# ChristophReich1996/Multi-StyleGAN

Hardware: AMD Instinct MI355X
Metric: training images/sec (G+D step, 256^2, seq=3x2ch) (higher is better)
Workload: dtype bf16

## Files before the change

include/msg_hip.h:

```cpp
#ifndef MSG_HIP_H
#define MSG_HIP_H

#ifdef __cplusplus
extern "C" {
#endif

enum { MSG_OK = 0, MSG_EINVAL = -1, MSG_EUNSUPPORTED = -2, MSG_ELAUNCH = -3 };
enum { MSG_F32 = 0, MSG_BF16 = 1, MSG_F16 = 2, MSG_F64 = 3, MSG_F32_SPLIT = 4 };

#define MSG_ABI_VERSION 5
int msg_abi_version(void);
const char* msg_build_arch(void);
const char* msg_strerror(int code);

int msg_upfirdn2d(const void* x, const float* fir, void* y, int dtype,
                  int major, int in_h, int in_w, int minor, int kh, int kw,
                  int up_x, int up_y, int down_x, int down_y,
                  int pad_x0, int pad_x1, int pad_y0, int pad_y1, void* stream);

int msg_upfirdn2d_pitched(const void* x, const float* fir, void* y, int dtype,
                          int major, int in_h, int in_w, int minor, int in_pitch, int kh, int kw,
                          int up_x, int up_y, int down_x, int down_y,
                          int pad_x0, int pad_x1, int pad_y0, int pad_y1, void* stream);

int msg_upfirdn2d_pitched2(const void* x, const float* fir, void* y, int dtype,
                           int major, int in_h, int in_w, int minor, int in_pitch, int out_pitch, int kh, int kw,
                           int up_x, int up_y, int down_x, int down_y,
                           int pad_x0, int pad_x1, int pad_y0, int pad_y1, void* stream);

int msg_upfirdn2d_separable(const void* x, const float* fir_y, const float* fir_x, void* y, int dtype,
                            int major, int in_h, int in_w, int minor, int kh, int kw,
                            int pad_x0, int pad_x1, int pad_y0, int pad_y1, void* stream);

int msg_upfirdn2d_separable_act(const void* x, const float* fir_y, const float* fir_x, void* y, int dtype,
                                int major, int in_h, int in_w, int minor, int kh, int kw,
                                int pad_x0, int pad_x1, int pad_y0, int pad_y1,
                                const float* act_bias, const float* noise, const float* noise_weight,
                                int noise_batch, float alpha, float scale, void* stream);
int msg_upfirdn2d_separable_act_mask(const void* x, const float* fir_y, const float* fir_x, void* y, int dtype,
                                     int major, int in_h, int in_w, int minor, int kh, int kw,
                                     int pad_x0, int pad_x1, int pad_y0, int pad_y1,
                                     const float* act_bias, const float* noise, const float* noise_weight,
                                     int noise_batch, float alpha, float scale, unsigned char* mask, void* stream);

int msg_fused_bias_act(const void* x, const float* bias, const void* ref, void* y, int dtype,
                       long long size_x, int step_b, int size_b,
                       const float* noise, const float* noise_weight, int noise_batch, int pix,
                       int act, int grad, float alpha, float scale, void* stream);

long long msg_bias_act_backward_workspace(long long size_x, int step_b, int size_b, int has_noise);
int msg_bias_act_backward(const void* gy, const void* out, void* gx, int dtype,
                          long long size_x, int step_b, int size_b,
                          float* grad_bias, const float* noise, float* grad_noise_weight,
                          int noise_batch, int pix, float alpha, float scale,
                          float* ws, long long ws_floats, void* stream);
int msg_channel_sums(const void* x, float* sums, int dtype, long long size_x, int C, float* ws, long long ws_floats,
                     void* stream);
int msg_bias_act_backward_mask(const void* gy, const unsigned char* mask, int tile_m, int tile_n, void* gx, int dtype,
                               long long size_x, int size_b,
                               float* grad_bias, const float* noise, float* grad_noise_weight,
                               int noise_batch, int pix, float alpha, float scale,
                               float* ws, long long ws_floats, void* stream);
int msg_sum_rows(const float* part, float* out, long long rows, int cols, void* stream);
int msg_bias_act_backward_mask_head(const void* gy, const void* ghead, const float* whead, const float* style,
                                    float wscale, int n_head, const unsigned char* mask, int tile_m, int tile_n,
                                    void* gx, int dtype, long long size_x, int size_b,
                                    float* grad_bias, const float* noise, float* grad_noise_weight,
                                    int noise_batch, int pix, float alpha, float scale,
                                    float* ws, long long ws_floats, void* stream);

int msg_conv2d_fprop(const void* x, const void* w, const float* bias, void* y, int dtype,
                     int B, int IH, int IW, int Cx, int Ck, int OH, int OW, int N, int ldy,
                     int kh, int kw, int stride, int pad, int in_up, int pixel_shuffle,
                     long long w_batch_stride, void* stream);
enum { MSG_WGRAD_K_AUTO = -1 };
int msg_conv2d_wgrad(const void* gy, const void* x, float* gw, int dtype,
                     int B, int IH, int IW, int Cx, int I, int OH, int OW, int ldgy, int O, int ldgw,
                     int kh, int kw, int stride, int pad, int pixel_shuffle,
                     int per_sample, int k_chunks, int oi_major, float gain,
                     float* ws, long long ws_floats, void* stream);
long long msg_conv2d_wgrad_workspace(int dtype, int B, int IH, int IW, int Cx, int I, int OH, int OW, int ldgy,
                                     int O, int ldgw, int kh, int kw, int stride, int pad, int pixel_shuffle,
                                     int per_sample, int k_chunks);

int msg_demod_coeff(const float* W, const float* s, float* d, int B, int O, int I, int taps,
                    float scale, float eps, void* stream);
int msg_scale_rows_cols(const float* base, const float* rowscale, const float* colscale, void* out,
                        int dtype, int B, int R, int T, int C, int Ck, float gain, void* stream);
int msg_modulate_weights(const float* base, const float* wsq, const float* style, void* out, float* d_out,
                         int dtype, int B, int R, int O, int T, int C, int Ck, float scale, float eps, void* stream);
int msg_modulate_backward(const float* gwk, const float* W, const float* s, const float* d, float* gW,
                          float* gs_part, int B, int O, int I, int taps, int ldg, int o_group,
                          float scale, void* stream);
int msg_scale_rows_cols2(const float* base, const float* row1, const float* col1, const float* row2, const float* col2,
                         void* out, int dtype, int B, int R, int T, int C, int Ck, float gain, void* stream);
int msg_modulate_backward2(const float* gwk, const float* W, const float* s, const float* d, const float* v,
                           float* gW, float* gs_part, int B, int O, int I, int taps, int ldg, int o_group,
                           float scale, void* stream);

int msg_relayout_weight(const float* w, void* fwd, void* dgrad, float* wsq, int dtype,
                        int O, int I, int T, int Ck, int Ok, int flip, int t_major, float gain, void* stream);

int msg_gather_taps(const void* x, void* y, int dtype, int B, int H, int W, int Cx, int C, int kh, int kw,
                    int pad, int Ko, void* stream);
int msg_fold_taps(const void* g, const void* add, void* gx, int dtype, int B, int H, int W, int Ko, int C, int kh, int kw,
                  int pad, int ldx, int ld_add, void* stream);

int msg_scaled_add(const void* a, const void* b, void* y, int dtype, long long n, float beta, float gain, void* stream);
int msg_rgb_skip_merge(const void* conv, int dtype, int ld, const float* bias, const float* skip, const float* fir,
                       float* out, int B, int C, int H, int W, void* stream);
int msg_rgb_skip_merge_backward(const float* g, void* g_conv, int dtype, int ld, float* g_skip, const float* fir,
                                int B, int C, int H, int W, void* stream);
int msg_gamma_merge(const void* a, const void* b, const float* gamma, void* y, int dtype, long long n, float gain, void* stream);
long long msg_gamma_merge_backward_workspace(void);
int msg_gamma_merge_backward(const void* gy, const void* a, const float* gamma, void* ga, void* gb, float* g_gamma, int dtype,
                             long long n, float gain, float* ws, void* stream);
int msg_scaled_add_rows(const void* a, const void* b, void* y, int dtype, long long rows, int cols,
                        long long lda, long long ldb, long long ldy, float beta, float gain, void* stream);

int msg_softmax_rows(const void* x, void* y, int dtype, long long rows, int cols, void* stream);
int msg_softmax_rows_backward(const void* y, const void* gy, void* gx, int dtype, long long rows, int cols,
                              void* stream);
int msg_softmax_rows_backward2(const void* y, const void* gy, const void* v, void* d_y, void* d_gy, int dtype,
                               long long rows, int cols, void* stream);

int msg_nonlocal_attention_supported(int B, int Nq, int Nk, int dk, int dv);
int msg_nonlocal_attention_fwd(const void* q, const void* k, const void* vt, void* o, float* lse, int dtype,
                               int B, int Nq, int Nk, int dk, int dv, void* stream);
int msg_maxpool2x2_fwd(const void* x, void* y, unsigned short* idx, int dtype, int B, int H, int W, int C, long long ldx,
                       void* stream);
int msg_maxpool2x2_bwd(const void* gy, const unsigned short* idx, void* gx, int dtype, int B, int H, int W, int C,
                       void* stream);
int msg_maxpool2x2_gather(const void* v, const unsigned short* idx, void* out, int dtype, int B, int H, int W, int C,
                          long long ldv, void* stream);

int msg_nonlocal_attention_bwd_splits(int B, int Nq, int Nk);
int msg_nonlocal_attention_bwd(const void* q, const void* qt, const void* k, const void* kt, const void* v,
                               const void* dO, const void* dOt, const void* o, const float* lse, float* delta,
                               void* dq, void* dk_out, void* dv_out, float* workspace, int dtype,
                               int B, int Nq, int Nk, int dk, int dv, void* stream);

int msg_affine_warp(const float* x, float* y, const float* angle_deg, float angle_const, const float* scale_xy,
                    const float* select_u, const float* p, int rot_prob, float cx, float cy, int padding,
                    int align_corners, int B, int C, int H, int W, int backward, void* workspace, void* stream);

long long msg_minibatch_stddev_workspace(int C, int H, int W, int groups, int dtype);
int msg_minibatch_stddev(const void* x, void* y, float* stat, float* workspace, int dtype,
                         int B, int C, int H, int W, int ldx, int ldy, int groups, float alpha, void* stream);
int msg_minibatch_stddev_backward(const void* x, const void* gy, const float* gstat, void* gx, int dtype,
                                  int B, int C, int H, int W, int ldx, int ldgy, int ldgx, int groups,
                                  float alpha, void* stream);

int msg_conv2d_fprop_act(const void* x, const void* w, void* y, int dtype,
                         int B, int IH, int IW, int Cx, int Ck, int OH, int OW, int N, int ldy,
                         int kh, int kw, int stride, int pad, long long w_batch_stride,
                         const float* act_bias, const float* noise, const float* noise_weight,
                         int noise_batch, float alpha, float scale, void* stream);
int msg_conv2d_fprop_act_mask(const void* x, const void* w, void* y, int dtype,
                              int B, int IH, int IW, int Cx, int Ck, int OH, int OW, int N, int ldy,
                              int kh, int kw, int stride, int pad, long long w_batch_stride,
                              const float* act_bias, const float* noise, const float* noise_weight,
                              int noise_batch, float alpha, float scale, unsigned char* mask, void* stream);

int msg_conv2d_fprop_residual(const void* x, const void* w, void* y, int dtype,
                              int B, int IH, int IW, int Cx, int Ck, int OH, int OW, int N, int ldy,
                              int kh, int kw, int stride, int pad, long long w_batch_stride,
                              const void* residual, int res_ld, float gain, void* stream);

int msg_conv2d_fprop_act_backward(const void* x, const void* w, void* y, int dtype,
                                  int B, int IH, int IW, int Cx, int Ck, int OH, int OW, int N, int ldy,
                                  int kh, int kw, int stride, int pad, long long w_batch_stride,
                                  const void* residual, int res_ld,
                                  const unsigned char* sign_mask, int mask_tile_m, int mask_tile_n,
                                  const void* sign_map, int sign_ld, float alpha, float scale,
                                  float* grad_bias, const float* noise, int noise_batch, float* grad_noise_weight,
                                  float* ws, long long ws_floats, void* stream);

int msg_act_pointwise_head(const void* x, const float* bias, const float* w, float* y, int dtype,
                           long long npix, int C, float wscale, float alpha, float scale, void* stream);
long long msg_act_pointwise_head_backward_workspace(long long npix, int C);
int msg_act_pointwise_head_backward(const void* x, const float* bias, const float* w, const float* gy, void* gx,
                                    float* grad_bias_and_w, int dtype, long long npix, int C, float wscale,
                                    float alpha, float scale, float* ws, long long ws_floats, void* stream);

int msg_linear_fprop(const float* x, const float* w, const float* bias, float* y, int M, int N, int K,
                     float gain, float bias_gain, void* stream);
int msg_linear_dgrad(const float* gy, const float* w, float* gx, int M, int N, int K, float gain, void* stream);
int msg_linear_wgrad(const float* gy, const float* x, float* gw, float* gb, int M, int N, int K,
                     float gain, float bias_gain, void* stream);

int msg_linear_grouped_fprop(const float* x, const int* slot, const float* const* w, const float* const* bias, float* y,
                             int G, int M, int N, int K, int L, float gain, float bias_gain, void* stream);
int msg_linear_grouped_dgrad(const float* gy, const float* const* w, float* gx, int G, int M, int N, int K, float gain,
                             void* stream);
int msg_linear_grouped_wgrad(const float* gy, const float* x, const int* slot, float* gw, float* gb, int G, int M, int N,
                             int K, int L, float gain, float bias_gain, void* stream);
int msg_linear_grouped_wgrad_ptrs(const float* gy, const float* x, const int* slot, float* const* gw, float* const* gb, int G,
                                  int M, int N, int K, int L, float gain, float bias_gain, void* stream);

enum {
    MSG_PLAN_REG = 0,
    MSG_PLAN_DMA = 1,
    MSG_PLAN_PP = 2,
    MSG_PLAN_ROW3 = 3,
    MSG_PLAN_ROW3N = 4,
    MSG_PLAN_THIN = 5,
    MSG_PLAN_UPCONV = 6,
    MSG_FPLAN_FIELDS = 5
};
int msg_conv2d_fprop_launch_plan(int dtype, int B, int IH, int IW, int Cx, int Ck, int OH, int OW, int N, int ldy,
                                 int kh, int kw, int stride, int pad, int in_up, int pixel_shuffle,
                                 long long w_batch_stride, int has_bias, int epilogue, long long* out, int n_out_fields);
enum {
    MSG_WPLAN_GENERIC = 0,
    MSG_WPLAN_DMA = 1,
    MSG_WPLAN_UNI = 2,
    MSG_WPLAN_ROW3 = 3,
    MSG_WPLAN_ROW3_W32 = 4,
    MSG_WPLAN_FIELDS = 11
};
int msg_conv2d_wgrad_plan(int dtype, int B, int IH, int IW, int Cx, int I, int OH, int OW, int ldgy,
                          int O, int ldgw, int kh, int kw, int stride, int pad, int pixel_shuffle,
                          int per_sample, int k_chunks, long long* out, int n_out_fields);
int msg_conv2d_fprop_plan(int dtype, int B, int IH, int IW, int Cx, int Ck, int OH, int OW, int N,
                          int kh, int kw, long long w_batch_stride);
long long msg_conv2d_fprop_act_backward_workspace(int dtype, int B, int IH, int IW, int Cx, int Ck, int OH, int OW,
                                                  int N, int kh, int kw, long long w_batch_stride, int has_noise);
int msg_conv2d_fprop_upconv_eligible(int B, int IH, int IW, int Cx, int Ck, int OH, int OW, int N, int kh, int kw,
                                     int stride, int pad, int in_up, int pixel_shuffle, long long w_batch_stride);
int msg_conv2d_fprop_thin_eligible(int B, int IH, int IW, int Cx, int Ck, int OH, int OW, int N, int ldy, int kh, int kw,
                                   int stride, int pad, int in_up, int pixel_shuffle, int act_mode);

int msg_flat_adam(float* param, const float* grad, float* exp_avg, float* exp_avg_sq, float* ema, long long n,
                  const float* coef, float lr, float beta1, float beta2, float eps, int step, float ema_decay,
                  void* stream);
int msg_flat_ema(float* ema, const float* param, long long n, float decay, void* stream);

long long msg_tlfm_prepare_workspace(int B, int T);
int msg_tlfm_prepare(const unsigned short* raw, const unsigned char* hflip, void* out, int dtype,
                     int B, int C, int T, int H, int W, int vflip,
                     float lo1, float div1, float lo2, float div2,
                     unsigned int* ws, void* stream);

int msg_tlfm_frame_range(const unsigned short* frames, long long N, int H, int W,
                         unsigned int* range, void* stream);
int msg_tlfm_gather(const unsigned short* frames, const unsigned int* range, long long N,
                    const int* index, const unsigned char* hflip, void* out, int dtype,
                    int B, int C, int T, int H, int W, int vflip,
                    float lo1, float div1, float lo2, float div2, void* stream);

int msg_sample_sheet(const void* seq, unsigned char* out, int dtype,
                     int B, int C, int T, int H, int W, int tints, void* stream);

enum { MSG_GAN_LOGISTIC = 0, MSG_GAN_WASSERSTEIN = 1, MSG_GAN_HINGE = 2 };
enum { MSG_GAN_AUX_NONE = 0, MSG_GAN_AUX_WEIGHT = 1, MSG_GAN_AUX_LABEL = 2 };
long long msg_gan_loss_workspace(long long n_real, long long n_fake);
int msg_gan_loss(const void* pred_real, const void* pred_fake, const float* aux, float* out, int dtype, int kind,
                 int aux_mode, long long n_real, long long n_fake, long long P, float* ws, long long ws_floats,
                 void* stream);
int msg_gan_loss_backward(const void* pred_real, const void* pred_fake, const float* aux, const float* grad_out,
                          void* grad_real, void* grad_fake, int dtype, int kind, int aux_mode,
                          long long n_real, long long n_fake, long long P, void* stream);

#define MSG_ELASTIC_MAX_SIGMA 32
long long msg_elastic_workspace(int B, int H, int W);
int msg_elastic_deform(const void* in, const float* noise, float* field, void* out, int dtype,
                       int B, int F, int H, int W, int sigma, float alpha, void* ws, void* stream);

#define MSG_JPEG_MAX_WIDTH 16384
long long msg_jpeg_workspace(int N, int H, int W);
int msg_jpeg_scan_capacity(int N, int H, int W, long long* bytes);
int msg_jpeg_encode(const unsigned char* rgb, const unsigned short* qtables, short* coef, unsigned char* scan,
                    long long* offsets, int N, int H, int W, void* ws, void* stream);

#ifdef __cplusplus
}
#endif
#endif
```

multi_stylegan_amd/conv_ops.py:

```python
import ctypes
import functools
import math
import os
from typing import Optional, Tuple

import torch
from torch.autograd import Function

from . import _lib
from ._autograd import _derive


def _vec(dtype) -> int:
    return 8 if dtype == torch.bfloat16 else 4


def _round_up(n: int, m: int) -> int:
    return (n + m - 1) // m * m


def _padded_nhwc(b, c, h, w, dtype, device):
    cx = _round_up(c, _vec(dtype))
    buf = torch.empty((b, h, w, cx), dtype=dtype, device=device)
    if cx != c:
        buf[..., c:].zero_()
    return buf.permute(0, 3, 1, 2)[:, :c]


class _CatChannels(Function):

    @staticmethod
    def forward(ctx, *tensors):
        t0 = tensors[0]
        ctx.splits = [t.shape[1] for t in tensors]
        out = _padded_nhwc(t0.shape[0], sum(ctx.splits), t0.shape[2], t0.shape[3], t0.dtype, t0.device)
        off = 0
        for t in tensors:
            out[:, off:off + t.shape[1]].copy_(t)
            off += t.shape[1]
        return out

    @staticmethod
    def backward(ctx, g):
        if torch.is_grad_enabled():
            pieces = _SplitChannels.apply(g, *ctx.splits)
            return tuple(p if need else None for p, need in zip(pieces, ctx.needs_input_grad))
        outs, off = [], 0
        for i, c in enumerate(ctx.splits):
            outs.append(g[:, off:off + c] if ctx.needs_input_grad[i] else None)
            off += c
        return tuple(outs)


class _SplitChannels(Function):

    @staticmethod
    def forward(ctx, g, *splits):
        ctx.splits = splits
        ctx.meta = (g.shape[0], g.shape[2], g.shape[3], g.dtype, g.device)
        outs, off = [], 0
        for c in splits:
            outs.append(g[:, off:off + c])
            off += c
        return tuple(outs)

    @staticmethod
    def backward(ctx, *gg):
        b, h, w, dtype, dev = ctx.meta
        pieces = [x if x is not None else torch.zeros((b, c, h, w), dtype=dtype, device=dev)
                  for x, c in zip(gg, ctx.splits)]
        return (_CatChannels.apply(*pieces),) + (None,) * len(ctx.splits)


def to_compute_layout(x: torch.Tensor, dtype=None) -> torch.Tensor:
    if dtype is not None and x.dtype != dtype:
        x = x.to(dtype)
    if x.ndim == 4 and x.shape[1] > 1:
        if x.is_cuda and x.shape[1] % _vec(x.dtype):
            return _CatChannels.apply(x)
        return x.contiguous(memory_format=torch.channels_last)
    return x.contiguous()


class _CatAliased(Function):

    @staticmethod
    def forward(ctx, buffer, *pieces):
        ctx.splits = [t.shape[1] for t in pieces]
        off = 0
        for t in pieces:
            want = buffer[:, off:off + t.shape[1]]
            if t.shape != want.shape or t.dtype != buffer.dtype:
                raise _lib.MsgHipError(f"cat_in_place: piece {tuple(t.shape)} for slice {tuple(want.shape)}")
            same = t.data_ptr() == want.data_ptr() and \
                all(a == b for a, b, n in zip(t.stride(), want.stride(), t.shape) if n != 1)
            if not same:
                if t.untyped_storage().data_ptr() == buffer.untyped_storage().data_ptr():
                    raise _lib.MsgHipError("cat_in_place: a piece lives in the destination buffer, but not in its slice")
                want.copy_(t)
            off += t.shape[1]
        if off != buffer.shape[1]:
            raise _lib.MsgHipError("cat_in_place: the pieces do not fill the destination buffer")
        return buffer.view_as(buffer)

    @staticmethod
    def backward(ctx, g):
        needs = ctx.needs_input_grad[1:]
        if torch.is_grad_enabled():
            pieces = _SplitChannels.apply(g, *ctx.splits)
            return (None, *(p if need else None for p, need in zip(pieces, needs)))
        out, off = [], 0
        for c, need in zip(ctx.splits, needs):
            out.append(g[:, off:off + c] if need else None)
            off += c
        return (None, *out)


def cat_destination(b: int, channels, h: int, w: int, dtype, device):
    if any(c % _vec(dtype) for c in channels) or not torch.device(device).type == "cuda":
        return None
    buf = _padded_nhwc(b, sum(channels), h, w, dtype, device)
    if any(c % (128 // buf.element_size()) for c in channels):
        buf.zero_()
    views, off = [], 0
    for c in channels:
        views.append(buf[:, off:off + c])
        off += c
    return buf, views


def cat_in_place(buffer, pieces) -> torch.Tensor:
    return _CatAliased.apply(buffer, *pieces)


def cat_channels(tensors) -> torch.Tensor:
    tensors = list(tensors)
    if tensors[0].is_cuda and all(t.dtype == tensors[0].dtype for t in tensors):
        return _CatChannels.apply(*tensors)
    return to_compute_layout(torch.cat(tensors, dim=1))


def _nhwc_view(x: torch.Tensor) -> Tuple[torch.Tensor, int]:
    b, c, h, w = x.shape
    vec = _vec(x.dtype)
    sb, sc, sh, sw = x.stride()
    cx = sw
    if (sc == 1 or c == 1) and cx >= c and cx % vec == 0 and sh == w * cx and (sb == h * w * cx or b == 1) \
            and x.data_ptr() % 16 == 0:
        return x, cx
    cx = _round_up(c, vec)
    buf = torch.empty((b, h, w, cx), dtype=x.dtype, device=x.device).permute(0, 3, 1, 2)
    if cx == c:
        buf.copy_(x)
        return buf, cx
    buf[:, :c].copy_(x)
    buf[:, c:].zero_()
    return buf[:, :c], cx


def _alloc_out(b: int, n: int, h: int, w: int, dtype, device) -> Tuple[torch.Tensor, int]:
    ld = _round_up(n, _vec(dtype))
    if ld == n:
        return torch.empty((b, n, h, w), dtype=dtype, device=device, memory_format=torch.channels_last), ld
    buf = torch.empty((b, h, w, ld), dtype=dtype, device=device)
    return buf.permute(0, 3, 1, 2)[:, :n], ld


def _relayout_kernel_ok(w, dtype, taps) -> bool:
    return w.is_cuda and w.dtype == torch.float32 and dtype in (torch.bfloat16, torch.float32) and \
        taps <= 16 and w.ndim >= 4


def _relay_fwd(w: torch.Tensor, dtype) -> Tuple[torch.Tensor, int]:
    if w.ndim == 2:
        w = w[:, :, None, None]
    *lead, o, i, kh, kw = w.shape
    ck = _round_up(i, 128 // (2 if dtype == torch.bfloat16 else 4))
    if _relayout_kernel_ok(w, dtype, kh * kw):
        rows = w.numel() // (i * kh * kw)
        out = torch.empty((*lead, o, kh * kw, ck), dtype=dtype, device=w.device)
        with _lib.on_device(w.device):
            code = _lib.lib().msg_relayout_weight(w.detach().contiguous().data_ptr(), out.data_ptr(), None, None,
                                                  _lib.dtype_code(out), rows, i, kh * kw, ck, ck, 0, 0, 1.0,
                                                  _lib.stream_of(w.device))
        _lib.check(code, "msg_relayout_weight")
        return out, ck
    out = torch.zeros((*lead, o, kh * kw, ck), dtype=dtype, device=w.device)
    out[..., :i] = w.reshape(*lead, o, i, kh * kw).transpose(-1, -2)
    return out, ck


def _relay_dgrad(w: torch.Tensor, dtype, flip: bool) -> Tuple[torch.Tensor, int]:
    if w.ndim == 2:
        w = w[:, :, None, None]
    *lead, o, i, kh, kw = w.shape
    ok = _round_up(o, 128 // (2 if dtype == torch.bfloat16 else 4))
    if _relayout_kernel_ok(w, dtype, kh * kw) and len(lead) <= 1:
        n = lead[0] if lead else 1
        out = torch.empty((*lead, i, kh * kw, ok), dtype=dtype, device=w.device)
        w3 = w.detach().contiguous().view(n, o, i, kh * kw)
        ov = out.view(n, i, kh * kw, ok)
        with _lib.on_device(w.device):
            for k in range(n):
                code = _lib.lib().msg_relayout_weight(w3[k].data_ptr(), None, ov[k].data_ptr(), None, _lib.dtype_code(out),
                                                      o, i, kh * kw, ok, ok, int(flip), 0, 1.0, _lib.stream_of(w.device))
                _lib.check(code, "msg_relayout_weight")
        return out, ok
    src = w.reshape(*lead, o, i, kh * kw)
    if flip:
        src = src.flip(-1)
    out = torch.zeros((*lead, i, kh * kw, ok), dtype=dtype, device=w.device)
    out[..., :o] = src.permute(*range(len(lead)), len(lead) + 1, len(lead) + 2, len(lead))
    return out, ok


def _s2_plan(k: int, pad: int):
    offs = {}
    for ph in (0, 1):
        t0 = (ph + pad) % 2
        e = (ph + pad - t0) // 2
        for u in range((k - t0 + 1) // 2):
            offs[(ph, e - u)] = t0 + 2 * u
    dmin = min(d for _, d in offs)
    dmax = max(d for _, d in offs)
    taps = dmax - dmin + 1
    table = [[offs.get((ph, tau + dmin), -1) for tau in range(taps)] for ph in (0, 1)]
    return taps, -dmin, table


def _relay_dgrad_s2(w: torch.Tensor, dtype, pad: int) -> Tuple[torch.Tensor, int, int, int]:
    *lead, o, i, kh, kw = w.shape
    assert kh == kw
    taps, pad2, table = _s2_plan(kh, pad)
    ok = _round_up(o, 128 // (2 if dtype == torch.bfloat16 else 4))
    src = [[(table[ph][th] * kw + table[pw][tw]) if table[ph][th] >= 0 and table[pw][tw] >= 0 else kh * kw
            for th in range(taps) for tw in range(taps)] for ph in (0, 1) for pw in (0, 1)]
    idx = torch.tensor(src, dtype=torch.long, device=w.device)
    wt = w.transpose(-4, -3).reshape(*lead, i, o, kh * kw)
    wz = torch.cat([wt, wt.new_zeros((*lead, i, o, 1))], dim=-1)
    picked = wz[..., idx]
    n = len(lead)
    picked = picked.permute(*range(n), n + 2, n, n + 3, n + 1)
    out = torch.zeros((*lead, 4, i, taps * taps, ok), dtype=dtype, device=w.device)
    out[..., :o] = picked
    return out.reshape(*lead, 4 * i, taps * taps, ok), ok, taps, pad2


_WEIGHT_GENERATION = [0]


def invalidate_weight_cache(params=None) -> None:
    if params is None:
        _WEIGHT_GENERATION[0] += 1
        return
    for p in params:
        p.__dict__["_msg_gen"] = p.__dict__.get("_msg_gen", 0) + 1


def _after_optimizer_step(optimizer, *_args, **_kwargs) -> None:
    for group in optimizer.param_groups:
        invalidate_weight_cache(group["params"])


def _stamp(w):
    return (w._version, _WEIGHT_GENERATION[0], w.__dict__.get("_msg_gen", 0), w.data_ptr())


from torch.optim.optimizer import register_optimizer_step_post_hook as _register_step_hook

_register_step_hook(_after_optimizer_step)


def _cached(w, tag, dtype, wscale, build):
    if not isinstance(w, torch.nn.Parameter):
        out = build()
        return (out[0] * wscale, *out[1:]) if wscale != 1.0 else out
    store = w.__dict__.setdefault("_msg_relay", {})
    key = (tag, dtype, wscale)
    stamp = _stamp(w)
    hit = store.get(key)
    if hit is not None and hit[0] == stamp:
        return hit[1]
    with torch.no_grad():
        out = build()
        if wscale != 1.0:
            out = (out[0] * wscale, *out[1:])
    store[key] = (stamp, out)
    return out


def _param_images(w, dtype, gain, kind, modulation=False):
    key = ("img", dtype, gain, kind, modulation)
    store = w.__dict__.get("_msg_relay")
    if store is not None:
        hit = store.get(key)
        if hit is not None and hit[0] == (w._version, _WEIGHT_GENERATION[0], w.__dict__.get("_msg_gen", 0), w.data_ptr()):
            return hit[1]
    if not (isinstance(w, torch.nn.Parameter) and w.is_cuda and w.dtype == torch.float32):
        return None
    o, i = _oi(w)
    t = w.numel() // (o * i)
    if t > 16 or w.numel() != o * i * t:
        return None
    store = w.__dict__.setdefault("_msg_relay", {})
    stamp = _stamp(w)
    dev = w.device
    unit = 1 if modulation else 128 // (2 if dtype == torch.bfloat16 else 4)
    ck, ok = _round_up(i, unit), _round_up(o, unit)
    up2 = kind == "up2"
    with torch.no_grad():
        w3 = w.detach().reshape(o, i, t).contiguous()
        fwd = torch.empty((t * o, 1, ck) if up2 else (o, t, ck), dtype=dtype, device=dev)
        dgr = torch.empty((i, t, ok), dtype=dtype, device=dev)
        wsq = torch.empty((o, i), dtype=torch.float32, device=dev) if modulation else None
        with _lib.on_device(dev):
            code = _lib.lib().msg_relayout_weight(w3.data_ptr(), fwd.data_ptr(), dgr.data_ptr(), _lib.ptr(wsq),
                                                  _lib.dtype_code(fwd), o, i, t, ck, ok, int(not up2), int(up2),
                                                  float(gain), _lib.stream_of(dev))
        _lib.check(code, "msg_relayout_weight")
    out = {"f": (fwd, ck), "d": (dgr, ok), "wsq": wsq}
    store[key] = (stamp, out)
    return out


_CLOCK_SHAPES = bool(int(os.environ.get("MSG_CLOCK_SHAPES", "0")))

FP32_CONTRACTION = "exact"
MSG_F32_SPLIT = _lib.MSG_F32_SPLIT
_SPLIT_CODES = {"split_bf16x3": MSG_F32_SPLIT}


class fp32_contraction:

    def __init__(self, mode: str):
        if mode not in ("exact", "split_bf16x3"):
            raise ValueError(f"fp32 contraction mode {mode!r}: 'exact' or 'split_bf16x3'")
        self.mode, self.prev = mode, None

    def __enter__(self):
        global FP32_CONTRACTION
        self.prev, FP32_CONTRACTION = FP32_CONTRACTION, self.mode
        return self

    def __exit__(self, *exc):
        global FP32_CONTRACTION
        FP32_CONTRACTION = self.prev
        return False

    @staticmethod
    def set(mode: str) -> None:
        fp32_contraction(mode).__enter__()


def _contraction_code(t: torch.Tensor, mode: Optional[str] = None) -> int:
    code = _lib.dtype_code(t)
    mode = FP32_CONTRACTION if mode is None else mode
    return _SPLIT_CODES[mode] if (code == _lib.MSG_F32 and mode != "exact") else code


_PLANS = {_lib.MSG_PLAN_REG: ("conv_fprop_reg", None), _lib.MSG_PLAN_DMA: ("conv_fprop_dma", None),
          _lib.MSG_PLAN_PP: ("conv_fprop_pp", None), _lib.MSG_PLAN_ROW3: ("conv_fprop_row3", 256),
          _lib.MSG_PLAN_ROW3N: ("conv_fprop_row3n", 128), _lib.MSG_PLAN_THIN: ("conv_fprop_thin", None),
          _lib.MSG_PLAN_UPCONV: ("conv_fprop_upconv", None)}


@functools.lru_cache(maxsize=None)
def _fprop_plan(*args):
    out = (ctypes.c_longlong * _lib.MSG_FPLAN_FIELDS)()
    ok = _lib.lib().msg_conv2d_fprop_launch_plan(*args, ctypes.addressof(out), len(out)) == _lib.MSG_OK
    kernel = out[0] if ok else None
    return (kernel,) + _PLANS.get(kernel, ("conv_fprop", None)) + (out[3] * args[8], out[4])


@functools.lru_cache(maxsize=None)
def _wgrad_plan(*geom):
    out = (ctypes.c_longlong * _lib.MSG_WPLAN_FIELDS)()
    _lib.check(_lib.lib().msg_conv2d_wgrad_plan(*geom, _lib.MSG_WGRAD_K_AUTO, ctypes.addressof(out), len(out)),
               "msg_conv2d_wgrad_plan")
    return out[10], out[1]


def _launch_fprop(x, wk, ck, bias, n, out_hw, kh, kw, stride, pad, in_up, pixel_shuffle, per_sample, c_real,
                  flops=None, act=None, residual=None, out=None, mode=None):
    dev = _lib.require_gpu(x, wk, bias)
    xv, cx = _nhwc_view(x)
    b, _, ih, iw = xv.shape
    oh, ow = out_hw
    if out is not None:
        y, ldy = _nhwc_view(out)
        if y is not out or pixel_shuffle or out.shape != (b, n, oh, ow) or out.dtype != x.dtype or n % _vec(x.dtype):
            raise _lib.MsgHipError(f"conv fprop: destination {tuple(out.shape)} / {out.stride()} for a {(b, n, oh, ow)} result")
    elif pixel_shuffle:
        y, ldy = _alloc_out(b, n // 4, 2 * oh, 2 * ow, x.dtype, dev)
    else:
        y, ldy = _alloc_out(b, n, oh, ow, x.dtype, dev)
    rows_needed = n * (1 if pixel_shuffle else kh * kw) * ck
    if per_sample:
        ws_ = wk.stride() if wk.ndim == 4 else None
        if ws_ is None or wk.shape[0] != b or ws_[0] < rows_needed or ws_[3] != 1 or \
                (wk.shape[2] > 1 and ws_[2] != wk.shape[3]) or (wk.shape[1] > 1 and ws_[1] != wk.shape[2] * wk.shape[3]):
            raise _lib.MsgHipError(f"conv fprop: per-sample weight image {tuple(wk.shape)} for batch {b}, {n} x {kh * kw} x {ck}")
    elif wk.numel() < rows_needed or not wk.is_contiguous():
        raise _lib.MsgHipError(f"conv fprop: weight image {tuple(wk.shape)} smaller than {n} x {kh * kw} x {ck}")
    wstride = wk.stride(0) if per_sample else 0
    if flops is None:
        flops = 2.0 * b * oh * ow * n * kh * kw * c_real / (in_up * in_up)
    key, sign_tile = "conv_fprop", None
    sign_holder = act[5] if act is not None and len(act) > 5 else None
    if _lib.kernel_clock.enabled or sign_holder is not None:
        _, key, sign_tile, _, _ = _fprop_plan(_lib.dtype_code(x), b, ih, iw, cx, ck, oh, ow, n, ldy, kh, kw, stride, pad, in_up,
                                              int(pixel_shuffle), wstride, int(bias is not None),
                                              2 if residual is not None else int(act is not None))
    if _lib.kernel_clock.enabled and _CLOCK_SHAPES:
        key += f"|B{b} {ih}x{iw}->{oh}x{ow} {c_real}->{n} {kh}x{kw} s{stride} up{in_up}" \
               f"{' ps' if pixel_shuffle else ''}{' per-sample' if per_sample else ''}|"
    with _lib.on_device(dev), _lib.kernel_clock.span((key, 'bf16' if x.dtype == torch.bfloat16 else 'f32'), flops):
        if residual is not None:
            assert bias is None and act is None and in_up == 1 and not pixel_shuffle
            rv, res_ld = _nhwc_view(residual[0])
            assert rv.shape == (b, n, oh, ow) and rv.dtype == x.dtype
            code = _lib.lib().msg_conv2d_fprop_residual(
                xv.data_ptr(), wk.data_ptr(), y.data_ptr(), _contraction_code(x, mode), b, ih, iw, cx, ck, oh, ow, n, ldy, kh, kw,
                stride, pad, wstride, rv.data_ptr(), res_ld, float(residual[1]), _lib.stream_of(dev))
        elif act is None:
            code = _lib.lib().msg_conv2d_fprop(
                xv.data_ptr(), wk.data_ptr(), _lib.ptr(bias), y.data_ptr(), _contraction_code(x, mode), b, ih, iw, cx, ck, oh,
                ow, n, ldy, kh, kw, stride, pad, in_up, int(pixel_shuffle), wstride, _lib.stream_of(dev))
        else:
            assert bias is None and in_up == 1 and not pixel_shuffle
            act_bias, noise, noise_w, alpha, scale = act[:5]
            _lib.require_gpu(x, act_bias, noise, noise_w)
            mask = None
            if sign_holder is not None and sign_tile:
                from .op_static.fused_act import sign_mask_for
                mask = sign_mask_for(b, n, oh, ow, x.dtype, dev)
                if mask is not None:
                    sign_holder.append((mask, sign_tile, sign_tile))
            code = _lib.lib().msg_conv2d_fprop_act_mask(
                xv.data_ptr(), wk.data_ptr(), y.data_ptr(), _contraction_code(x, mode), b, ih, iw, cx, ck, oh, ow, n, ldy, kh, kw,
                stride, pad, wstride, _lib.ptr(act_bias), _lib.ptr(noise), _lib.ptr(noise_w),
                1 if noise is None else noise.shape[0], float(alpha), float(scale), _lib.ptr(mask), _lib.stream_of(dev))
    _lib.check(code, "msg_conv2d_fprop")
    return y


def _grad_dest(param):
    if param is None or "_msg_grad_slot" not in getattr(param, "__dict__", ()):
        return None
    from .dist import grad_destination
    return grad_destination(param)


def _launch_wgrad(gy, x, o, i, kh, kw, stride, pad, pixel_shuffle, per_sample, low_hw, raw=False, gain=1.0, out=None,
                  mode=None):
    dev = _lib.require_gpu(gy, x)
    gv, ldgy = _nhwc_view(gy)
    xv, cx = _nhwc_view(x)
    b, _, ih, iw = xv.shape
    oh, ow = low_hw if pixel_shuffle else gv.shape[2:]
    taps = kh * kw
    ldgw = _round_up(i, 4)
    geom = (_contraction_code(x, mode), b, ih, iw, cx, i, oh, ow, ldgy, o, ldgw, kh, kw, stride, pad, int(pixel_shuffle),
            int(per_sample))
    need, nz = _wgrad_plan(*geom)
    ws = _lib.scratch_ptr(need, dev) if need else None
    if per_sample or raw:
        out = None
    oi_major = (bool(need) or out is not None) and not per_sample and not raw
    if oi_major:
        gw = out.view(o, i, kh, kw) if out is not None else torch.empty((o, i, kh, kw), dtype=torch.float32, device=dev)
    elif per_sample:
        gw = torch.empty((b, o, taps, ldgw), dtype=torch.float32, device=dev)
    else:
        gw = torch.empty((o, taps, ldgw), dtype=torch.float32, device=dev)
    flops = 2.0 * b * oh * ow * o * i * taps
    key = "conv_wgrad"
    if _CLOCK_SHAPES and _lib.kernel_clock.enabled:
        key += f"|B{b} {ih}x{iw}->{oh}x{ow} {i}->{o} {kh}x{kw} s{stride}{' ps' if pixel_shuffle else ''}" \
               f"{' per-sample' if per_sample else ' shared'}{f' slabs{nz}' if need else ''}|"
    with _lib.on_device(dev), _lib.kernel_clock.span((key, 'bf16' if x.dtype == torch.bfloat16 else 'f32'), flops):
        code = _lib.lib().msg_conv2d_wgrad(
            gv.data_ptr(), xv.data_ptr(), gw.data_ptr(), *geom, _lib.MSG_WGRAD_K_AUTO, int(oi_major), float(gain), ws, need,
            _lib.stream_of(dev))
    _lib.check(code, "msg_conv2d_wgrad")
    if raw:
        return gw, ldgw
    if oi_major:
        return gw
    lead = gw.shape[:-2]
    return gw.view(*lead, kh, kw, ldgw)[..., :i].permute(*range(len(lead)), len(lead) + 2, len(lead), len(lead) + 1)


class Geometry:
    __slots__ = ("kind", "kh", "kw", "stride", "pad", "x_hw", "y_hw", "per_sample", "wscale", "mode")

    def __init__(self, kind, kh, kw, stride, pad, x_hw, per_sample, wscale=1.0, mode=None):
        self.kind, self.kh, self.kw, self.stride, self.pad = kind, kh, kw, stride, pad
        self.x_hw, self.per_sample, self.wscale = tuple(x_hw), per_sample, float(wscale)
        self.mode = FP32_CONTRACTION if mode is None else mode
        if kind == "up2":
            self.y_hw = (2 * x_hw[0], 2 * x_hw[1])
        else:
            self.y_hw = ((x_hw[0] + 2 * pad - kh) // stride + 1, (x_hw[1] + 2 * pad - kw) // stride + 1)


def _oi(w):
    return (w.shape[0], w.shape[1]) if w.ndim == 2 else (w.shape[-4], w.shape[-3])


def _relay_fwd_kind(w, dtype, kind):
    wk, ck = _relay_fwd(w, dtype)
    if kind == "up2":
        o = _oi(w)[0]
        wk = wk.transpose(-3, -2).reshape(*wk.shape[:-3], 4 * o, 1, ck).contiguous()
    return wk, ck


def _thin_ok(dtype, i, g: Geometry) -> bool:
    taps = g.kh * g.kw
    return g.kind == "conv" and g.stride == 1 and not g.per_sample and taps > 1 and \
        2 * g.pad + 1 == g.kh and g.kh == g.kw and i * taps <= 128 // (2 if dtype == torch.bfloat16 else 4)


def _gather_taps(x, i, g: Geometry):
    dev = _lib.require_gpu(x)
    xv, cx = _nhwc_view(x)
    b, _, h, w = xv.shape
    ko = 128 // x.element_size()
    out = torch.empty((b, h, w, ko), dtype=x.dtype, device=dev)
    with _lib.on_device(dev):
        code = _lib.lib().msg_gather_taps(xv.data_ptr(), out.data_ptr(), _lib.dtype_code(x), b, h, w, cx, i, g.kh, g.kw,
                                          g.pad, ko, _lib.stream_of(dev))
    _lib.check(code, "msg_gather_taps")
    return out.permute(0, 3, 1, 2), ko


def _relay_thin(w, dtype):
    o, i, kh, kw = w.shape
    ko = 128 // (2 if dtype == torch.bfloat16 else 4)
    out = torch.zeros((o, 1, ko), dtype=dtype, device=w.device)
    out[:, 0, :kh * kw * i] = w.permute(0, 2, 3, 1).reshape(o, kh * kw * i)
    return out, ko


def _f_raw(x, w, bias, g: Geometry, act=None, residual=None, out=None):
    if w.ndim == 4 and _thin_ok(x.dtype, w.shape[1], g):
        xc, ko = _gather_taps(x, w.shape[1], g)
        wk, _ = _cached(w, "thin", x.dtype, g.wscale, lambda: _relay_thin(w, x.dtype))
        return _launch_fprop(xc, wk, ko, bias, w.shape[0], g.y_hw, 1, 1, 1, 0, 1, False, False,
                             w.shape[1] * g.kh * g.kw, act=act, residual=residual, out=out, mode=g.mode)
    if g.kind == "up2" and _oi(w)[0] % _vec(x.dtype):
        o_real = _oi(w)[0]
        wp = torch.zeros((*w.shape[:-4], _round_up(o_real, _vec(x.dtype)), *w.shape[-3:]), dtype=w.dtype, device=w.device)
        wp[..., :o_real, :, :, :] = w.detach()
        assert out is None
        return _f_raw(x, wp, bias, g, act=act, residual=residual)[:, :o_real]
    img = _param_images(w, x.dtype, g.wscale, g.kind) if not g.per_sample else None
    wk, ck = img["f"] if img is not None else \
        _cached(w, "f" + g.kind, x.dtype, g.wscale, lambda: _relay_fwd_kind(w, x.dtype, g.kind))
    o, _ = _oi(w)
    if g.kind == "up2":
        assert out is None
        return _launch_fprop(x, wk, ck, None, 4 * o, g.x_hw, 1, 1, 1, 0, 1, True, g.per_sample, _oi(w)[1], mode=g.mode)
    return _launch_fprop(x, wk, ck, bias, o, g.y_hw, g.kh, g.kw, g.stride, g.pad, 1, False, g.per_sample, _oi(w)[1],
                         act=act, residual=residual, out=out, mode=g.mode)


def _act_operands(bias, noise, noise_w, y_shape):
    b32 = None if bias is None else bias.detach().to(torch.float32).contiguous()
    nz = nw = None
    if noise is not None:
        if noise.shape[0] not in (1, y_shape[0]) or noise.shape[1] != 1 or tuple(noise.shape[2:]) != tuple(y_shape[2:]):
            raise _lib.MsgHipError(f"noise shape {tuple(noise.shape)} does not match output {tuple(y_shape)}")
        nz = noise.detach().to(torch.float32).contiguous()
        nw = noise_w.detach().to(torch.float32).contiguous()
    return b32, nz, nw


ACT_BACKWARD_IN_DGRAD = bool(int(os.environ.get("MSG_ACT_BACKWARD_IN_DGRAD", "1")))


class ActHandle:
    __slots__ = ("armed", "sign", "alpha", "scale", "bias_param", "has_bias", "noise", "done")

    def __init__(self):
        self.armed, self.sign, self.done = False, None, None
        self.alpha = self.scale = 0.0
        self.bias_param, self.has_bias, self.noise = None, False, None

    def arm(self, y, mask, alpha, scale, bias_param, has_bias, noise):
        if not ACT_BACKWARD_IN_DGRAD or y.dtype != torch.bfloat16 or not y.is_cuda:
            return
        self.sign = ("mask",) + tuple(mask) if mask is not None else ("map",)
        self.alpha, self.scale = float(alpha), float(scale)
        self.bias_param, self.has_bias, self.noise = bias_param, bool(has_bias), noise
        self.armed, self.done = True, None


def _launch_dgrad_act_backward(gy, wk, ck, n, kh, kw, per_sample, c_real, handle: ActHandle, residual=None, mode=None,
                               sign_map=None):
    if torch.is_grad_enabled() or gy.dtype != torch.bfloat16:
        return None
    if mode is not None and _contraction_code(gy, mode) != _lib.MSG_BF16:
        return None
    dev = gy.device
    xv, cx = _nhwc_view(gy)
    b, _, h, w_ = xv.shape
    wstride = wk.stride(0) if per_sample else 0
    noise = handle.noise
    ldy = _round_up(n, _vec(gy.dtype))
    _, label, _, bias_floats, noise_floats = _fprop_plan(_lib.MSG_BF16, b, h, w_, cx, ck, h, w_, n, ldy, kh, kw, 1, 1, 1, 0, wstride, 0, 3)
    if not bias_floats:
        return None
    need = bias_floats + (noise_floats if noise is not None else 0)
    sign = handle.sign
    smask = smap = None
    tm = tn = sld = 0
    if sign[0] == "mask":
        smask, tm, tn = sign[1], int(sign[2]), int(sign[3])
        if smask.numel() * 8 != b * n * h * w_ or (tm != 1 and tm % 64):
            return None
    else:
        if sign_map is None or sign_map.dtype != torch.bfloat16:
            return None
        smap, sld = _nhwc_view(sign_map)
        if smap is not sign_map or tuple(smap.shape) != (b, n, h, w_):
            return None
    rv, res_ld = (None, 0)
    if residual is not None:
        assert residual[1] == 1.0
        rv, res_ld = _nhwc_view(residual[0])
        if rv.shape != (b, n, h, w_) or rv.dtype != gy.dtype:
            return None
    y, ldy = _alloc_out(b, n, h, w_, gy.dtype, dev)
    gb = None
    if handle.has_bias:
        bp = handle.bias_param
        if bp is not None and bp.dtype == torch.float32 and bp.shape == (n,):
            gb = _grad_dest(bp)
        if gb is None:
            gb = torch.empty(n, dtype=torch.float32, device=dev)
    nz = gnw = None
    nb = 1
    if noise is not None:
        if noise.shape[0] not in (1, b) or tuple(noise.shape[1:]) != (1, h, w_):
            return None
        nz, nb = noise.detach().to(torch.float32).contiguous(), noise.shape[0]
        gnw = torch.empty(1, dtype=torch.float32, device=dev)
    ws = _lib.scratch_ptr(need, dev)
    flops = 2.0 * b * h * w_ * n * kh * kw * c_real
    key = label + "_actbwd"
    if _lib.kernel_clock.enabled and _CLOCK_SHAPES:
        key += f"|B{b} {h}x{w_}->{h}x{w_} {c_real}->{n} 3x3 s1 up1{' per-sample' if per_sample else ''}|"
    with _lib.on_device(dev), _lib.kernel_clock.span((key, 'bf16'), flops):
        code = _lib.lib().msg_conv2d_fprop_act_backward(
            xv.data_ptr(), wk.data_ptr(), y.data_ptr(), _lib.MSG_BF16, b, h, w_, cx, ck, h, w_, n, ldy, kh, kw, 1, 1, wstride,
            _lib.ptr(rv), res_ld, _lib.ptr(smask), tm, tn, _lib.ptr(smap), sld, handle.alpha, handle.scale,
            _lib.ptr(gb), _lib.ptr(nz), nb, _lib.ptr(gnw), ws, need, _lib.stream_of(dev))
    _lib.check(code, "msg_conv2d_fprop_act_backward")
    handle.done = (gb, gnw)
    return y


def _d_raw(gy, w, g: Geometry, residual=None, act_bwd: Optional["ActHandle"] = None, sign_map=None):
    if act_bwd is not None and act_bwd.armed and not g.per_sample and g.kind == "conv" and g.stride == 1 and g.kh == 3 and \
            g.kw == 3 and g.pad == 1 and w.ndim == 4:
        i = _oi(w)[1]
        img = _param_images(w, gy.dtype, g.wscale, g.kind)
        wk, ok = img["d"] if img is not None else \
            _cached(w, "d" + g.kind, gy.dtype, g.wscale, lambda: _relay_dgrad(w, gy.dtype, flip=True))
        out = _launch_dgrad_act_backward(gy, wk, ok, i, 3, 3, False, _oi(w)[0], act_bwd, residual=residual, mode=g.mode,
                                         sign_map=sign_map)
        if out is not None:
            return out
    return _d_raw_plain(gy, w, g, residual)


def _d_raw_plain(gy, w, g: Geometry, residual=None):
    assert residual is None or (g.kind == "conv" and g.stride == 1)
    if g.kind == "conv" and g.stride == 2 and _oi(w)[1] % _vec(gy.dtype) == 0:
        return _d_raw_s2(gy, w, g)
    i = _oi(w)[1]
    if w.ndim == 4 and _thin_ok(gy.dtype, i, g) and i <= 8 and gy.shape[1] >= 64:
        return _d_raw_thin(gy, w, g, residual)
    img = _param_images(w, gy.dtype, g.wscale, g.kind) if not g.per_sample else None
    wk, ok = img["d"] if img is not None else \
        _cached(w, "d" + g.kind, gy.dtype, g.wscale, lambda: _relay_dgrad(w, gy.dtype, flip=g.kind != "up2"))
    if g.kind == "up2":
        return _launch_fprop(gy, wk, ok, None, i, g.x_hw, 2, 2, 2, 0, 1, False, g.per_sample, _oi(w)[0], mode=g.mode)
    pad = g.kh - 1 - g.pad
    assert g.kh == g.kw
    return _launch_fprop(gy, wk, ok, None, i, g.x_hw, g.kh, g.kw, 1, pad, g.stride, False, g.per_sample, _oi(w)[0],
                         residual=residual, mode=g.mode)


def _relay_thin_dgrad(w, dtype):
    o, i, kh, kw = w.shape
    esz = 2 if dtype == torch.bfloat16 else 4
    ko, ok = 128 // esz, _round_up(o, 128 // esz)
    out = torch.zeros((ko, 1, ok), dtype=dtype, device=w.device)
    out[:kh * kw * i, 0, :o] = w.permute(2, 3, 1, 0).reshape(kh * kw * i, o)
    return out, ok


def _d_raw_thin(gy, w, g: Geometry, residual=None):
    o, i = w.shape[0], w.shape[1]
    dev = gy.device
    wd, ok = _cached(w, "dthin", gy.dtype, g.wscale, lambda: _relay_thin_dgrad(w, gy.dtype))
    ko = 128 // gy.element_size()
    flops = 2.0 * gy.shape[0] * g.x_hw[0] * g.x_hw[1] * o * i * g.kh * g.kw
    gk = _launch_fprop(gy, wd, ok, None, ko, g.x_hw, 1, 1, 1, 0, 1, False, False, o, flops=flops, mode=g.mode)
    gkv, ldk = _nhwc_view(gk)
    b, _, h, w_ = gkv.shape
    gx, ldx = _alloc_out(b, i, h, w_, gy.dtype, dev)
    add = ld_add = None
    if residual is not None:
        assert residual[1] == 1.0
        add, ld_add = _nhwc_view(residual[0])
        assert add.shape == gx.shape and add.dtype == gx.dtype
    with _lib.on_device(dev), _lib.kernel_clock.span(("fold_taps", gy.dtype), (gkv.numel() + b * h * w_ * ldx) * gy.element_size()):
        code = _lib.lib().msg_fold_taps(gkv.data_ptr(), _lib.ptr(add), gx.data_ptr(), _lib.dtype_code(gy), b, h, w_, ldk, i,
                                        g.kh, g.kw, g.pad, ldx, ld_add or 0, _lib.stream_of(dev))
    _lib.check(code, "msg_fold_taps")
    return gx


def _d_raw_s2(gy, w, g: Geometry):
    o, i = _oi(w)
    wk, ok, taps, pad2 = _cached(w, "ds2", gy.dtype, g.wscale, lambda: _relay_dgrad_s2(w, gy.dtype, g.pad))
    hc, wc = (g.x_hw[0] + 1) // 2, (g.x_hw[1] + 1) // 2
    flops = 2.0 * gy.shape[0] * gy.shape[2] * gy.shape[3] * o * i * g.kh * g.kw
    gx = _launch_fprop(gy, wk, ok, None, 4 * i, (hc, wc), taps, taps, 1, pad2, 1, True, g.per_sample, o, flops=flops, mode=g.mode)
    return gx[:, :, :g.x_hw[0], :g.x_hw[1]]


def _g_raw(gy, x, o, i, g: Geometry, out=None):
    if _thin_ok(x.dtype, i, g):
        xc, ko = _gather_taps(x, i, g)
        gwp = _launch_wgrad(gy, xc, o, ko, 1, 1, 1, 0, False, False, None, gain=g.wscale, mode=g.mode)
        taps = g.kh * g.kw
        return gwp[:, :taps * i, 0, 0].reshape(o, taps, i).permute(0, 2, 1).reshape(o, i, g.kh, g.kw)
    if g.kind == "up2":
        return _launch_wgrad(gy, x, o, i, 2, 2, 1, 0, True, g.per_sample, g.x_hw, gain=g.wscale, out=out, mode=g.mode)
    return _launch_wgrad(gy, x, o, i, g.kh, g.kw, g.stride, g.pad, False, g.per_sample, None, gain=g.wscale, out=out, mode=g.mode)


def _consumed(ctx, arg_index: int, tensor_ordinal: int) -> bool:
    if not ctx.needs_input_grad[arg_index]:
        return False
    try:
        node = ctx.next_functions[tensor_ordinal][0]
        return node is None or bool(torch._C._will_engine_execute_node(node))
    except Exception:
        return True


class _ConvF(Function):
    @staticmethod
    def forward(ctx, x, w, bias, g):
        ctx.g = g
        ctx.has_bias = bias is not None
        ctx.save_for_backward(x, w)
        return _f_raw(x, w, bias, g)

    @staticmethod
    def backward(ctx, gy):
        x, w = ctx.saved_tensors
        g = ctx.g
        gx = _derive(_ConvD, gy, w, g) if ctx.needs_input_grad[0] else None
        gw = _derive(_ConvG, gy, x, _oi(w), w.ndim, g, w) if _consumed(ctx, 1, 1) else None
        gb = _channel_sums(gy) if ctx.has_bias and _consumed(ctx, 2, 2) else None
        return gx, gw, gb, None


def _channel_sums(gy):
    c = gy.shape[1]
    vec = _vec(gy.dtype)
    if torch.is_grad_enabled() or not gy.is_cuda or gy.dtype not in (torch.float32, torch.bfloat16) or c % vec or \
            not gy.is_contiguous(memory_format=torch.channels_last) or gy.data_ptr() % 16 or gy.numel() == 0:
        return gy.sum(dim=(0, 2, 3), dtype=torch.float32)
    dev = gy.device
    need = _lib.lib().msg_bias_act_backward_workspace(gy.numel(), 1, c, 0)
    ws = torch.empty(max(need, 1), dtype=torch.float32, device=dev)
    out = torch.empty(c, dtype=torch.float32, device=dev)
    with _lib.on_device(dev):
        code = _lib.lib().msg_channel_sums(gy.data_ptr(), out.data_ptr(), _lib.dtype_code(gy), gy.numel(), c, ws.data_ptr(),
                                           need, _lib.stream_of(dev))
    _lib.check(code, "msg_channel_sums")
    return out


def _dgrad_add_ok(add, x_shape, dtype, g) -> bool:
    return add is not None and g.kind == "conv" and g.stride == 1 and tuple(add.shape) == tuple(x_shape) and add.dtype == dtype


class _ConvD(Function):

    @staticmethod
    def forward(ctx, gy, w, g, add=None):
        ctx.g = g
        ctx.save_for_backward(gy, w)
        return _d_raw(gy, w, g, residual=None if add is None else (add, 1.0))

    @staticmethod
    def backward(ctx, v):
        gy, w = ctx.saved_tensors
        g = ctx.g
        ggy = _derive(_ConvF, v, w, None, g) if ctx.needs_input_grad[0] else None
        gw = _derive(_ConvG, gy, v, _oi(w), w.ndim, g) if ctx.needs_input_grad[1] else None
        return ggy, gw, None, (v if len(ctx.needs_input_grad) > 3 and ctx.needs_input_grad[3] else None)


RESIDUAL_FORK_NODE = True


class _ConvDFork(Function):

    @staticmethod
    def forward(ctx, gy, w, g):
        ctx.g = g
        ctx.save_for_backward(gy, w)
        return _d_raw(gy, w, g), gy.view_as(gy)

    @staticmethod
    @torch.autograd.function.once_differentiable
    def backward(ctx, v, c):
        gy, w = ctx.saved_tensors
        g = ctx.g
        ggy = gw = None
        if v is None:
            return c, None, None
        if ctx.needs_input_grad[0]:
            if c is not None and g.kind == "conv" and g.stride == 1 and c.shape == gy.shape and c.dtype == v.dtype:
                ggy = _f_raw(v, w, None, g, residual=(c, 1.0))
            else:
                ggy = _f_raw(v, w, None, g)
                ggy = ggy if c is None else ggy + c
        if ctx.needs_input_grad[1]:
            gw = _derive(_ConvG, gy, v, _oi(w), w.ndim, g)
        return ggy, gw, None


class _ConvG(Function):
    @staticmethod
    def forward(ctx, gy, x, oi, w_ndim, g, dest=None):
        ctx.g = g
        ctx.save_for_backward(gy, x)
        out = None if (g.per_sample or _thin_ok(x.dtype, oi[1], g)) else _grad_dest(dest)
        gw = _g_raw(gy, x, oi[0], oi[1], g, out=out)
        if out is not None:
            return out
        if w_ndim == 5 and not g.per_sample:
            return gw.unsqueeze(0)
        return gw.reshape(oi) if w_ndim == 2 else gw

    @staticmethod
    def backward(ctx, u):
        gy, x = ctx.saved_tensors
        g = ctx.g
        ggy = _derive(_ConvF, x, u, None, g) if ctx.needs_input_grad[0] else None
        gx = _derive(_ConvD, gy, u, g) if ctx.needs_input_grad[1] else None
        return ggy, gx, None, None, None, None


class _ConvActF(Function):

    @staticmethod
    def forward(ctx, x, w, act_bias, noise, noise_w, g, alpha, scale, slot=None, out_scale=None, act_handle=None,
                input_act=None):
        o = _oi(w)[0]
        b32, nz, nw = _act_operands(act_bias, noise, noise_w, (x.shape[0], o, *g.y_hw))
        holder = [] if any(ctx.needs_input_grad) else None
        y = _f_raw(x, w, None, g, act=(b32, nz, nw, alpha, scale, holder))
        ctx.mask = holder[0] if holder else None
        ctx.slot, ctx.out_scale = slot, out_scale
        ctx.act_handle = ctx.input_act = None
        if act_handle is not None and out_scale is None and noise is None and holder is not None:
            act_handle.arm(y, ctx.mask, alpha, scale, act_bias, act_bias is not None, None)
            ctx.act_handle = act_handle if act_handle.armed else None
        if input_act is not None and input_act.armed:
            ctx.input_act = input_act
        ctx.bias_param = act_bias
        ctx.g, ctx.cfg = g, (alpha, scale, act_bias is not None, noise is not None)
        ctx.nw_shape = None if noise_w is None else noise_w.shape
        ctx.save_for_backward(x, w, y, noise)
        return y

    @staticmethod
    def backward(ctx, gy):
        from .op_static.fused_act import FusedLeakyReLUFunctionBackward
        x, w, y, noise = ctx.saved_tensors
        alpha, scale, has_bias, has_noise = ctx.cfg
        g = ctx.g
        owed = 1.0
        if ctx.out_scale is not None and ctx.out_scale.pending is not None:
            owed, ctx.out_scale.pending = ctx.out_scale.pending, None
        handed = ctx.act_handle.done if ctx.act_handle is not None else None
        if handed is not None:
            ctx.act_handle.done = None
            gpre, (gb, gnw) = gy, handed
        else:
            gpre, gb, gnw = _derive(FusedLeakyReLUFunctionBackward, gy, y, noise if has_noise else None,
                                    ctx.bias_param if has_bias else False, alpha, scale * owed, ctx.mask)
        gx = None
        if ctx.needs_input_grad[0]:
            other = ctx.slot.g if ctx.slot is not None else None
            pre = ctx.input_act if not torch.is_grad_enabled() else None
            if _dgrad_add_ok(other, x.shape, gpre.dtype, g):
                gx = _derive(_ConvD, gpre, w, g, other) if torch.is_grad_enabled() else \
                    _d_raw(gpre, w, g, residual=(other, 1.0), act_bwd=pre, sign_map=x)
                ctx.slot.merged = True
            elif pre is not None:
                gx = _d_raw(gpre, w, g, act_bwd=pre, sign_map=x)
            else:
                gx = _derive(_ConvD, gpre, w, g)
        gw = _derive(_ConvG, gpre, x, _oi(w), w.ndim, g, w) if _consumed(ctx, 1, 1) else None
        return gx, gw, (gb if has_bias and ctx.needs_input_grad[2] else None), None, \
            (gnw.reshape(ctx.nw_shape) if has_noise and ctx.needs_input_grad[4] else None), None, None, None, None, None, None, None


class _ConvResidualF(Function):

    @staticmethod
    def forward(ctx, x, w, main, g, gain, fork, slot=None, main_scale=None, out=None):
        y = _f_raw(x, w, None, g, residual=(main, gain), out=out)
        if out is not None:
            y = out.view_as(out)
        ctx.slot, ctx.main_scale = slot, main_scale
        ctx.g, ctx.gain, ctx.fork = g, float(gain), fork
        ctx.save_for_backward(x, w)
        return (y, y.view_as(y)) if fork else y

    @staticmethod
    def backward(ctx, *grads):
        from .op_static.fused_act import _ScaledAddRows, _rows_ok
        x, w = ctx.saved_tensors
        g1 = grads[0]
        g2 = grads[1] if ctx.fork else None
        if (g1 is None or g2 is None) and ctx.main_scale is not None and ctx.needs_input_grad[2]:
            gs = g1 if g1 is not None else g2
            ctx.main_scale.pending = ctx.gain
            gg = Geometry(ctx.g.kind, ctx.g.kh, ctx.g.kw, ctx.g.stride, ctx.g.pad, ctx.g.x_hw, ctx.g.per_sample,
                          ctx.g.wscale * ctx.gain, mode=ctx.g.mode)
            gs_main = gs
            if torch.is_grad_enabled() and ctx.needs_input_grad[0] and RESIDUAL_FORK_NODE:
                gx, gs_main = _ConvDFork.apply(gs, w, gg)
            else:
                gx = _derive(_ConvD, gs, w, gg) if ctx.needs_input_grad[0] else None
            if ctx.slot is not None and gx is not None:
                ctx.slot.g = gx
            gw = _derive(_ConvG, gs, x, _oi(w), w.ndim, gg, w) if _consumed(ctx, 1, 1) else None
            return gx, gw, gs_main, None, None, None, None, None, None
        if g1 is None or g2 is None:
            gs = (g1 if g1 is not None else g2) * ctx.gain
        elif _rows_ok(g1, g2):
            gs = _derive(_ScaledAddRows, g1, g2, ctx.gain)
        else:
            gs = (g1 + g2) * ctx.gain
        gx = _derive(_ConvD, gs, w, ctx.g) if ctx.needs_input_grad[0] else None
        if ctx.slot is not None and gx is not None:
            ctx.slot.g = gx
        gw = _derive(_ConvG, gs, x, _oi(w), w.ndim, ctx.g, w) if _consumed(ctx, 1, 1) else None
        return gx, gw, (gs if ctx.needs_input_grad[2] else None), None, None, None, None, None, None


class _MultiConvF(Function):

    @staticmethod
    def forward(ctx, x, geoms, *weights):
        ctx.geoms = geoms
        ctx.save_for_backward(x, *weights)
        return tuple(_f_raw(x, w, None, g) for w, g in zip(weights, geoms))

    @staticmethod
    def backward(ctx, *grads):
        x, *weights = ctx.saved_tensors
        second_order = torch.is_grad_enabled()
        gx, gws = None, []
        for k, (gy, w, g) in enumerate(zip(grads, weights, ctx.geoms)):
            if gy is None:
                gws.append(None)
                continue
            if ctx.needs_input_grad[0]:
                if gx is None or not _dgrad_add_ok(gx, x.shape, gy.dtype, g):
                    part = _derive(_ConvD, gy, w, g)
                    gx = part if gx is None else gx + part
                elif second_order:
                    gx = _derive(_ConvD, gy, w, g, gx)
                else:
                    gx = _d_raw(gy, w, g, residual=(gx, 1.0))
            gws.append(_derive(_ConvG, gy, x, _oi(w), w.ndim, g, w) if _consumed(ctx, 2 + k, 1 + k) else None)
        return (gx, None, *gws)


def conv2d_shared_input(x, weights_and_scales, padding=0):
    p = _square(padding, "padding")
    geoms = tuple(Geometry("conv", w.shape[2], w.shape[3], 1, p, x.shape[2:], False, ws) for w, ws in weights_and_scales)
    return _MultiConvF.apply(x, geoms, *[w for w, _ in weights_and_scales])


class GradScale:
    __slots__ = ("pending",)

    def __init__(self):
        self.pending = None


class GradSlot:
    __slots__ = ("g", "merged")

    def __init__(self):
        self.g, self.merged = None, False


class HeadGradSlot:
    __slots__ = ("head", "dgrad", "armed")

    def __init__(self):
        self.head = None
        self.dgrad = None
        self.armed = False

    def take(self):
        head, dgrad, self.head, self.dgrad = self.head, self.dgrad, None, None
        return head, dgrad


class _ForkInput(Function):

    @staticmethod
    def forward(ctx, x, slot):
        ctx.slot = slot
        return x.view_as(x), x.view_as(x)

    @staticmethod
    def backward(ctx, g_main, g_res):
        slot = ctx.slot
        merged, slot.g, slot.merged = slot.merged, None, False
        if merged or g_res is None:
            return g_main, None
        if g_main is None:
            return g_res, None
        return g_main + g_res, None


def _square(value, what: str) -> int:
    if isinstance(value, int):
        return value
    value = tuple(value)
    if len(value) != 2 or value[0] != value[1]:
        raise _lib.MsgHipError(f"conv2d: only square {what} is implemented, got {value}")
    return int(value[0])


def fork_input(x, slot: GradSlot):
    return _ForkInput.apply(x, slot)


def conv2d_add_residual(x, weight, main, gain, stride=1, padding=0, wscale=1.0, fork=False, grad_slot=None,
                        main_grad_scale=None, out=None):
    s, p = _square(stride, "stride"), _square(padding, "padding")
    g = Geometry("conv", weight.shape[2], weight.shape[3], s, p, x.shape[2:], False, wscale)
    return _ConvResidualF.apply(x, weight, main, g, float(gain), bool(fork), grad_slot, main_grad_scale, out)


def conv2d_bias_act(x, weight, act_bias, stride=1, padding=0, wscale=1.0, negative_slope=0.2, scale=1.0,
                    grad_slot=None, out_grad_scale=None, act_handle=None, input_act=None):
    s, p = _square(stride, "stride"), _square(padding, "padding")
    g = Geometry("conv", weight.shape[2], weight.shape[3], s, p, x.shape[2:], False, wscale)
    return _ConvActF.apply(x, weight, act_bias, None, None, g, float(negative_slope), float(scale), grad_slot,
                           out_grad_scale, act_handle, input_act)


def conv2d(x, weight, bias=None, stride=1, padding=0, wscale=1.0):
    s, p = _square(stride, "stride"), _square(padding, "padding")
    g = Geometry("conv", weight.shape[2], weight.shape[3], s, p, x.shape[2:], False, wscale)
    return _ConvF.apply(x, weight, None if bias is None else bias.float(), g)


def conv_transpose2d_2x2(x, weight, bias=None, wscale=1.0):
    if tuple(weight.shape[2:]) != (2, 2):
        raise _lib.MsgHipError("conv_transpose2d_2x2: 2x2 kernel, stride 2, padding 0 only")
    g = Geometry("up2", 2, 2, 1, 1, x.shape[2:], False, wscale)
    y = _ConvF.apply(x, weight.transpose(0, 1), None, g)
    return y if bias is None else y + bias.view(1, -1, 1, 1).to(y.dtype)


_LINEAR_MAX_ROWS = 256


def _lin_call(name, flops, *args):
    dev = args[0].device
    with _lib.on_device(dev), _lib.kernel_clock.span((name, "f32"), flops):
        code = getattr(_lib.lib(), f"msg_{name}")(*[a.data_ptr() if isinstance(a, torch.Tensor) else
                                                   (0 if a is None else a) for a in args], _lib.stream_of(dev))
    _lib.check(code, f"msg_{name}")


def _dense32(*ts):
    for t in ts:
        if t is not None and t.dtype != torch.float32:
            raise _lib.MsgHipError("the few-row linear kernels are fp32 (mapping network / style affines / heads)")
    return [None if t is None else t.contiguous() for t in ts]


class _LinF(Function):

    @staticmethod
    def forward(ctx, x, w, bias, gain, bias_gain=1.0):
        _lib.require_gpu(x, w, bias)
        x, w, bias = _dense32(x, w, bias)
        (m, k), n = x.shape, w.shape[0]
        y = torch.empty((m, n), dtype=torch.float32, device=x.device)
        _lin_call("linear_fprop", 2.0 * m * n * k, x, w, bias, y, m, n, k, float(gain), float(bias_gain))
        ctx.save_for_backward(x, w)
        ctx.gain, ctx.has_bias, ctx.bias_gain = float(gain), bias is not None, float(bias_gain)
        ctx.bias_param = bias
        return y

    @staticmethod
    def backward(ctx, gy):
        x, w = ctx.saved_tensors
        need_x, need_w, need_b = ctx.needs_input_grad[:3]
        gx = _derive(_LinD, gy, w, ctx.gain) if need_x else None
        gw = gb = None
        if need_w and need_b and ctx.has_bias and not torch.is_grad_enabled():
            (gy_,) = _dense32(gy)
            (m, n), k = gy_.shape, x.shape[1]
            gw, gb = _grad_dest(w), _grad_dest(ctx.bias_param)
            gw = gw if gw is not None else torch.empty((n, k), dtype=torch.float32, device=x.device)
            gb = gb if gb is not None else torch.empty((n,), dtype=torch.float32, device=x.device)
            _lin_call("linear_wgrad", 2.0 * m * n * k, gy_, x, gw, gb, m, n, k, ctx.gain, ctx.bias_gain)
        else:
            if need_w:
                gw = _derive(_LinG, gy, x, ctx.gain)
            if need_b and ctx.has_bias:
                gb = gy.sum(dim=0) if ctx.bias_gain == 1.0 else gy.sum(dim=0) * ctx.bias_gain
        return gx, gw, gb, None, None


class _LinD(Function):

    @staticmethod
    def forward(ctx, gy, w, gain):
        _lib.require_gpu(gy, w)
        gy, w = _dense32(gy, w)
        (m, n), k = gy.shape, w.shape[1]
        gx = torch.empty((m, k), dtype=torch.float32, device=gy.device)
        _lin_call("linear_dgrad", 2.0 * m * n * k, gy, w, gx, m, n, k, float(gain))
        ctx.save_for_backward(gy, w)
        ctx.gain = float(gain)
        return gx

    @staticmethod
    def backward(ctx, g):
        gy, w = ctx.saved_tensors
        d_gy = _derive(_LinF, g, w, None, ctx.gain) if ctx.needs_input_grad[0] else None
        d_w = _derive(_LinG, gy, g, ctx.gain) if ctx.needs_input_grad[1] else None
        return d_gy, d_w, None


class _LinG(Function):

    @staticmethod
    def forward(ctx, gy, x, gain):
        _lib.require_gpu(gy, x)
        gy, x = _dense32(gy, x)
        (m, n), k = gy.shape, x.shape[1]
        gw = torch.empty((n, k), dtype=torch.float32, device=gy.device)
        _lin_call("linear_wgrad", 2.0 * m * n * k, gy, x, gw, None, m, n, k, float(gain), 1.0)
        ctx.save_for_backward(gy, x)
        ctx.gain = float(gain)
        return gw

    @staticmethod
    def backward(ctx, g):
        gy, x = ctx.saved_tensors
        d_gy = _derive(_LinF, x, g, None, ctx.gain) if ctx.needs_input_grad[0] else None
        d_x = _derive(_LinD, gy, g, ctx.gain) if ctx.needs_input_grad[1] else None
        return d_gy, d_x, None


def linear(x, weight, bias=None, wscale=1.0, bias_scale=1.0):
    b, i = x.shape
    o = weight.shape[0]
    if x.dtype == torch.float32 and weight.dtype == torch.float32 and b <= _LINEAR_MAX_ROWS:
        return _LinF.apply(x, weight, None if bias is None else bias.float(), float(wscale), float(bias_scale))
    if bias is not None and bias_scale != 1.0:
        bias = bias * bias_scale
    g = Geometry("conv", 1, 1, 1, 0, (b, 1), False, wscale)
    y = _ConvF.apply(x.reshape(1, b, 1, i).permute(0, 3, 1, 2), weight, None if bias is None else bias.float(), g)
    return y.permute(0, 2, 3, 1).reshape(b, o)


_PTR_TABLES: dict = {}


def _ptr_table(tensors, dev):
    key = (dev.index, tuple(t.data_ptr() for t in tensors))
    hit = _PTR_TABLES.get(key)
    if hit is None:
        if len(_PTR_TABLES) > 64:
            _PTR_TABLES.clear()
        hit = _PTR_TABLES[key] = torch.tensor(key[1], dtype=torch.int64, device=dev)
    return hit


class _GroupedLinear(Function):

    @staticmethod
    def forward(ctx, latent, slot, wscale, bias_scale, *wb):
        g = len(slot)
        ws, bs = wb[:g], wb[g:]
        dev = _lib.require_gpu(latent, *ws, *bs)
        (lat,) = _dense32(latent)
        b, l, k = lat.shape
        n = ws[0].shape[0]
        for w, bb in zip(ws, bs):
            if w.shape != (n, k) or bb.shape != (n,) or w.dtype != torch.float32 or bb.dtype != torch.float32 \
                    or not w.is_contiguous():
                raise _lib.MsgHipError("grouped linear: layers must be fp32, contiguous and of one shape")
        slot_t = _ptr_table_ints(slot, dev)
        y = torch.empty((g, b, n), dtype=torch.float32, device=dev)
        with _lib.on_device(dev), _lib.kernel_clock.span("linear_grouped_fprop/f32", 2.0 * g * b * n * k):
            code = _lib.lib().msg_linear_grouped_fprop(lat.data_ptr(), slot_t.data_ptr(), _ptr_table(ws, dev).data_ptr(),
                                                       _ptr_table(bs, dev).data_ptr(), y.data_ptr(), g, b, n, k, l,
                                                       float(wscale), float(bias_scale), _lib.stream_of(dev))
        _lib.check(code, "msg_linear_grouped_fprop")
        ctx.save_for_backward(latent, *ws, *bs)
        ctx.cfg = (tuple(slot), float(wscale), float(bias_scale))
        return y

    @staticmethod
    def backward(ctx, gy):
        slot, wscale, bias_scale = ctx.cfg
        g = len(slot)
        lat, ws, bs = ctx.saved_tensors[0], ctx.saved_tensors[1:1 + g], ctx.saved_tensors[1 + g:]
        need = ctx.needs_input_grad
        if torch.is_grad_enabled() and need[0] and not any(_consumed(ctx, 4 + j, 1 + j) for j in range(2 * g) if need[4 + j]):
            glat = _GroupedLinD.apply(gy, slot, wscale, lat.shape[1], *ws)
            return (glat, None, None, None, *([None] * (2 * g)))
        if torch.is_grad_enabled():
            with torch.enable_grad():
                ins = [t for t, nd in zip((lat, *ws, *bs), (need[0], *need[4:])) if nd]
                out = torch.stack([linear(lat[:, slot[j]], ws[j], bs[j], wscale, bias_scale) for j in range(g)])
                grads = list(torch.autograd.grad(out, ins, gy, create_graph=True, allow_unused=True))
            res = [grads.pop(0) if nd else None for nd in (need[0], *need[4:])]
            return (res[0], None, None, None, *res[1:])
        dev = lat.device
        gy, lat = _dense32(gy, lat)
        b, l, k = lat.shape
        n = ws[0].shape[0]
        slot_t = _ptr_table_ints(slot, dev)
        glat = _grouped_dgrad(gy, ws, slot, wscale, l) if need[0] else None
        grads_w, grads_b = [None] * g, [None] * g
        if any(need[4:]):
            gw = gb = None
            dw, db, direct = [], [], 0
            for j in range(g):
                tw = _grad_dest(ws[j]) if need[4 + j] else None
                tb = _grad_dest(bs[j]) if need[4 + g + j] else None
                direct += (tw is not None) + (tb is not None)
                if tw is None:
                    if gw is None:
                        gw = torch.empty((g, n, k), dtype=torch.float32, device=dev)
                    tw = gw[j]
                if tb is None:
                    if gb is None:
                        gb = torch.empty((g, n), dtype=torch.float32, device=dev)
                    tb = gb[j]
                dw.append(tw)
                db.append(tb)
            if direct == 0:
                with _lib.on_device(dev):
                    code = _lib.lib().msg_linear_grouped_wgrad(gy.data_ptr(), lat.data_ptr(), slot_t.data_ptr(), gw.data_ptr(),
                                                               gb.data_ptr(), g, b, n, k, l, wscale, bias_scale,
                                                               _lib.stream_of(dev))
                _lib.check(code, "msg_linear_grouped_wgrad")
            else:
                if gw is None and gb is None:
                    tbl = _ptr_table(dw + db, dev).view(2, g)
                else:
                    tbl = torch.tensor([[t.data_ptr() for t in dw], [t.data_ptr() for t in db]], dtype=torch.int64).to(dev)
                with _lib.on_device(dev):
                    code = _lib.lib().msg_linear_grouped_wgrad_ptrs(gy.data_ptr(), lat.data_ptr(), slot_t.data_ptr(),
                                                                    tbl[0].data_ptr(), tbl[1].data_ptr(), g, b, n, k, l,
                                                                    wscale, bias_scale, _lib.stream_of(dev))
                _lib.check(code, "msg_linear_grouped_wgrad_ptrs")
            grads_w = [dw[j] if need[4 + j] else None for j in range(g)]
            grads_b = [db[j] if need[4 + g + j] else None for j in range(g)]
        return (glat, None, None, None, *grads_w, *grads_b)


def _grouped_dgrad(gy, ws, slot, wscale, n_slots):
    dev = gy.device
    g = len(slot)
    (gy,) = _dense32(gy)
    b, n, k = gy.shape[1], ws[0].shape[0], ws[0].shape[1]
    gx = torch.empty((g + 1, b, k), dtype=torch.float32, device=dev)
    gx[g].zero_()
    with _lib.on_device(dev):
        code = _lib.lib().msg_linear_grouped_dgrad(gy.data_ptr(), _ptr_table(ws, dev).data_ptr(), gx.data_ptr(),
                                                   g, b, n, k, wscale, _lib.stream_of(dev))
    _lib.check(code, "msg_linear_grouped_dgrad")
    return gx[_slot_gather_table(slot, n_slots, dev)].sum(dim=1).transpose(0, 1)


class _GroupedLinD(Function):

    @staticmethod
    def forward(ctx, gy, slot, wscale, n_slots, *ws):
        _lib.require_gpu(gy, *ws)
        ctx.save_for_backward(gy, *ws)
        ctx.cfg = (tuple(slot), float(wscale), int(n_slots))
        return _grouped_dgrad(gy, ws, slot, wscale, n_slots)

    @staticmethod
    @torch.autograd.function.once_differentiable
    def backward(ctx, v):
        gy, *ws = ctx.saved_tensors
        slot, wscale, l = ctx.cfg
        g, dev = len(slot), gy.device
        gy, v = _dense32(gy, v)
        b, n, k = gy.shape[1], ws[0].shape[0], ws[0].shape[1]
        slot_t = _ptr_table_ints(slot, dev)
        d_gy, d_ws = None, [None] * g
        with _lib.on_device(dev):
            if ctx.needs_input_grad[0]:
                d_gy = torch.empty((g, b, n), dtype=torch.float32, device=dev)
                code = _lib.lib().msg_linear_grouped_fprop(v.data_ptr(), slot_t.data_ptr(), _ptr_table(ws, dev).data_ptr(), None,
                                                           d_gy.data_ptr(), g, b, n, k, l, wscale, 1.0, _lib.stream_of(dev))
                _lib.check(code, "msg_linear_grouped_fprop")
            if any(ctx.needs_input_grad[4:]):
                gw = torch.empty((g, n, k), dtype=torch.float32, device=dev)
                code = _lib.lib().msg_linear_grouped_wgrad(gy.data_ptr(), v.data_ptr(), slot_t.data_ptr(), gw.data_ptr(), None, g, b,
                                                           n, k, l, wscale, 1.0, _lib.stream_of(dev))
                _lib.check(code, "msg_linear_grouped_wgrad")
                d_ws = [gw[j] if ctx.needs_input_grad[4 + j] else None for j in range(g)]
        return (d_gy, None, None, None, *d_ws)


_INT_TABLES: dict = {}
_GATHER_TABLES: dict = {}


def _slot_gather_table(slot, n_slots, dev):
    key = (dev.index, tuple(int(v) for v in slot), n_slots)
    hit = _GATHER_TABLES.get(key)
    if hit is None:
        if len(_GATHER_TABLES) > 64:
            _GATHER_TABLES.clear()
        rows = [[j for j, v in enumerate(key[1]) if v == l] for l in range(n_slots)]
        width = max(1, max(len(r) for r in rows))
        hit = _GATHER_TABLES[key] = torch.tensor([r + [len(slot)] * (width - len(r)) for r in rows], dtype=torch.int64,
                                                 device=dev)
    return hit


def _ptr_table_ints(values, dev):
    key = (dev.index, tuple(int(v) for v in values))
    hit = _INT_TABLES.get(key)
    if hit is None:
        if len(_INT_TABLES) > 64:
            _INT_TABLES.clear()
        hit = _INT_TABLES[key] = torch.tensor(key[1], dtype=torch.int32, device=dev)
    return hit


def grouped_linear(latent, slots, weights, biases, wscale, bias_scale):
    return _GroupedLinear.apply(latent, tuple(int(v) for v in slots), float(wscale), float(bias_scale), *weights, *biases)


def demod_coefficients(weight, style, scale):
    wsq = weight[0].square().sum(dim=(2, 3))
    return torch.rsqrt((scale * scale) * (style.square() @ wsq.t()) + 1e-8)


def _modulated_composite(x, weight, style, demodulate, upsample):
    _, out_c, in_c, kh, kw = weight.shape
    scale = math.sqrt(2.0) / math.sqrt(in_c * kh * kw)
    coef = style[:, None, :] * scale
    if demodulate:
        coef = coef * demod_coefficients(weight, style, scale)[:, :, None]
    wmod = weight * coef[:, :, :, None, None]
    g = Geometry("up2" if upsample else "conv", kh, kw, 1, kh // 2, x.shape[2:], True)
    return _ConvF.apply(x, wmod, None, g)


def _scale_rows_cols(base, rowscale, colscale, out, gain):
    b, r, t, ck = out.shape
    c = base.shape[-1]
    dev = base.device
    with _lib.on_device(dev):
        code = _lib.lib().msg_scale_rows_cols(base.data_ptr(), _lib.ptr(rowscale), _lib.ptr(colscale), out.data_ptr(),
                                              _lib.dtype_code(out), b, r, t, c, ck, float(gain), _lib.stream_of(dev))
    _lib.check(code, "msg_scale_rows_cols")
    return out


_MODCONV_BWD_BATCH = 16


def _dgrad_image_base(weight, w3, upsample, kind):
    img = _param_images(weight, torch.float32, 1.0, kind, modulation=True)
    return img["d"][0] if img is not None else _cached(weight, "md" + kind, torch.float32, 1.0, lambda: (
        (w3 if upsample else w3.flip(-1)).permute(1, 2, 0).contiguous(), 0))[0]


def _fwd_image_base(weight, w3, upsample, kind):
    o, i, t = w3.shape
    img = _param_images(weight, torch.float32, 1.0, kind, modulation=True)
    return img["f"][0] if img is not None else _cached(weight, "mb" + kind, torch.float32, 1.0, lambda: (
        (w3.permute(2, 0, 1).reshape(t * o, 1, i) if upsample else w3.transpose(1, 2)).contiguous(), 0))[0]


def _tap_square_sums(weight, w3, kind):
    img = _param_images(weight, torch.float32, 1.0, kind, modulation=True)
    return img["wsq"] if img is not None else \
        _cached(weight, "wsq", torch.float32, 1.0, lambda: (w3.square().sum(dim=2).contiguous(), 0))[0]


def _dgrad_modconv(gy, wd, okp, o, i, kh, kw, upsample, g, act_bwd=None, sign_map=None):
    if act_bwd is not None and act_bwd.armed and not upsample and kh == 3 and kw == 3:
        out = _launch_dgrad_act_backward(gy, wd, okp, i, kh, kw, True, o, act_bwd, mode=g.mode, sign_map=sign_map)
        if out is not None:
            return out
    if upsample:
        return _launch_fprop(gy, wd, okp, None, i, g.x_hw, 2, 2, 2, 0, 1, False, True, o, mode=g.mode)
    return _launch_fprop(gy, wd, okp, None, i, g.x_hw, kh, kw, 1, kh - 1 - kh // 2, 1, False, True, o, mode=g.mode)


def _fprop_modconv(x, wk, ck, o, i, kh, kw, upsample, g, add_to=None):
    if upsample:
        y = _launch_fprop(x, wk, ck, None, 4 * o, g.x_hw, 1, 1, 1, 0, 1, True, True, i, mode=g.mode)
        return y if add_to is None else y + add_to
    return _launch_fprop(x, wk, ck, None, o, g.y_hw, kh, kw, 1, kh // 2, 1, False, True, i,
                         residual=None if add_to is None else (add_to, 1.0), mode=g.mode)


def _wgrad_modconv(gy, x, o, i, kh, kw, upsample, g):
    if upsample:
        return _launch_wgrad(gy, x, o, i, 2, 2, 1, 0, True, True, g.x_hw, raw=True, mode=g.mode)
    return _launch_wgrad(gy, x, o, i, kh, kw, 1, kh // 2, False, True, None, raw=True, mode=g.mode)


def _fold_weight_gradient(gwk, ldg, w3, s, dd, scale, style_dtype, cotangent=None, dest=None):
    b = gwk.shape[0]
    o, i, t = w3.shape
    dev = gwk.device
    og = 2 if o >= 512 or o < 256 else 1
    groups = (o + og - 1) // og
    out = _grad_dest(dest) if cotangent is None else None
    gw3 = out.view(o, i, t) if out is not None else torch.empty((o, i, t), dtype=torch.float32, device=dev)
    gs_part = _lib.scratch_ptr(groups * b * i, dev)
    gs = torch.empty((b, i), dtype=torch.float32, device=dev)
    with _lib.on_device(dev):
        st = _lib.stream_of(dev)
        if cotangent is None:
            code = _lib.lib().msg_modulate_backward(gwk.data_ptr(), w3.data_ptr(), s.data_ptr(), _lib.ptr(dd),
                                                    gw3.data_ptr(), gs_part, b, o, i, t, ldg, og, scale, st)
        else:
            code = _lib.lib().msg_modulate_backward2(gwk.data_ptr(), w3.data_ptr(), s.data_ptr(), _lib.ptr(dd),
                                                     cotangent.data_ptr(), gw3.data_ptr(), gs_part, b, o, i, t,
                                                     ldg, og, scale, st)
        _lib.check(code, "msg_modulate_backward" + ("2" if cotangent is not None else ""))
        code = _lib.lib().msg_sum_rows(gs_part, gs.data_ptr(), groups, b * i, st)
    _lib.check(code, "msg_sum_rows")
    return (out if out is not None else gw3), (gs if style_dtype == torch.float32 else gs.to(style_dtype))


def _modconv_backward(x, weight, style, d, gy, demodulate, upsample, g, scale, need, keep_gwk=False, direct=False,
                      act_bwd=None):
    _, o, i, kh, kw = weight.shape
    b, t = x.shape[0], kh * kw
    dev = x.device
    w3 = weight.detach().reshape(o, i, t)
    s = style.detach().float().contiguous()
    dd = d if demodulate else None
    esz = 2 if gy.dtype == torch.bfloat16 else 4
    gx = None
    if need[0]:
        okp = _round_up(o, 128 // esz)
        wd = torch.empty((b, i, t, okp), dtype=gy.dtype, device=dev)
        _scale_rows_cols(_dgrad_image_base(weight, w3, upsample, g.kind), s, dd, wd, scale)
        gx = _dgrad_modconv(gy, wd, okp, o, i, kh, kw, upsample, g, act_bwd=act_bwd, sign_map=x)
    gw = gs = gwk = None
    if need[1] or need[2]:
        gwk, ldg = _wgrad_modconv(gy, x, o, i, kh, kw, upsample, g)
        gw3, gs = _fold_weight_gradient(gwk, ldg, w3, s, dd, scale, style.dtype, dest=weight if direct else None)
        gw = gw3.reshape(1, o, i, kh, kw)
    return (gx, gw, gs, gwk) if keep_gwk else (gx, gw, gs)


_NATIVE_SECOND_ORDER = True


def _modconv_second_order_composite(gy, x, weight, style, demodulate, upsample, a, cot_w, cot_s, want):
    with torch.enable_grad():
        leaves = [t.detach().requires_grad_(True) for t in (gy, x, weight, style)]
        y2 = _modulated_composite(leaves[1], leaves[2], leaves[3], demodulate, upsample)
        first = torch.autograd.grad(y2, leaves[1:], leaves[0], create_graph=True, allow_unused=True)
        terms = [(c.to(f.dtype) * f).sum() for c, f in zip((a, cot_w, cot_s), first) if c is not None and f is not None]
        if not terms:
            return (None, None, None, None)
        grads = torch.autograd.grad(sum(terms), leaves, allow_unused=True)
    return tuple(gr if w else None for gr, w in zip(grads, want))


class _ModConvGrad(Function):

    @staticmethod
    def forward(ctx, gy, x, weight, style, d, demodulate, upsample, g, scale, need):
        gx, gw, gs, gwk = _modconv_backward(x, weight, style, d, gy, demodulate, upsample, g, scale, need, keep_gwk=True)
        ctx.set_materialize_grads(False)
        ctx.save_for_backward(gy, x, weight, style, d, gwk)
        ctx.cfg = (demodulate, upsample, g, scale)
        return gx, gw, gs

    @staticmethod
    @torch.autograd.function.once_differentiable
    def backward(ctx, a, cot_w, cot_s):
        gy, x, weight, style, d, gwk = ctx.saved_tensors
        demodulate, upsample, g, scale = ctx.cfg
        want = ctx.needs_input_grad[:4]
        _, o, i, kh, kw = weight.shape
        b, t = x.shape[0], kh * kw
        tail = (None,) * 6
        if a is None and cot_w is None and cot_s is None:
            return (None, None, None, None) + tail
        if cot_w is not None or i % 4 or i > 512 or t not in (1, 4, 9) or b > _MODCONV_BWD_BATCH or \
                (cot_s is not None and gwk is None):
            return _modconv_second_order_composite(gy, x, weight, style, demodulate, upsample, a, cot_w, cot_s, want) + tail
        dev = x.device
        w3 = weight.detach().reshape(o, i, t)
        s = style.detach().float().contiguous()
        dd = d if demodulate else None
        esz = 2 if gy.dtype == torch.bfloat16 else 4
        ck, okp = _round_up(i, 128 // esz), _round_up(o, 128 // esz)
        rows = t * o if upsample else o
        ggy = gx2 = gw3 = gs2 = None
        if a is not None:
            a = a.to(x.dtype)
            if want[0]:
                wk = torch.empty((b, rows, 1 if upsample else t, ck), dtype=x.dtype, device=dev)
                base = _fwd_image_base(weight, w3, upsample, g.kind)
                if demodulate:
                    _scale_rows_cols(base, d.repeat(1, t) if upsample else d, s, wk, scale)
                else:
                    _scale_rows_cols(base, None, s, wk, scale)
                ggy = _fprop_modconv(a, wk, ck, o, i, kh, kw, upsample, g)
            if want[2] or want[3]:
                gwk_a, ldg = _wgrad_modconv(gy, a, o, i, kh, kw, upsample, g)
                gw3, gs2 = _fold_weight_gradient(gwk_a, ldg, w3, s, dd, scale, style.dtype)
        if cot_s is not None:
            v = cot_s.detach().float().contiguous()
            if want[0] or want[1]:
                hf = torch.empty((b, rows, 1 if upsample else t, ck), dtype=x.dtype, device=dev)
                hd = torch.empty((b, i, t, okp), dtype=gy.dtype, device=dev)
                base_f = _fwd_image_base(weight, w3, upsample, g.kind)
                base_d = _dgrad_image_base(weight, w3, upsample, g.kind)
                if demodulate:
                    wsq = _tap_square_sums(weight, w3, g.kind)
                    ddir = -(scale * scale) * d.pow(3) * linear(s * v, wsq)
                    rows_d, rows_dd = (d.repeat(1, t), ddir.repeat(1, t)) if upsample else (d, ddir)
                    with _lib.on_device(dev):
                        lib, st = _lib.lib(), _lib.stream_of(dev)
                        code = lib.msg_scale_rows_cols2(base_f.data_ptr(), rows_d.contiguous().data_ptr(), v.data_ptr(),
                                                        rows_dd.contiguous().data_ptr(), s.data_ptr(), hf.data_ptr(),
                                                        _lib.dtype_code(hf), b, rows, 1 if upsample else t, i, ck, scale, st)
                        _lib.check(code, "msg_scale_rows_cols2")
                        code = lib.msg_scale_rows_cols2(base_d.data_ptr(), v.data_ptr(), d.data_ptr(), s.data_ptr(),
                                                        ddir.contiguous().data_ptr(), hd.data_ptr(), _lib.dtype_code(hd), b, i, t,
                                                        o, okp, scale, st)
                        _lib.check(code, "msg_scale_rows_cols2")
                else:
                    _scale_rows_cols(base_f, None, v, hf, scale)
                    _scale_rows_cols(base_d, v, None, hd, scale)
                if want[0]:
                    ggy = _fprop_modconv(x, hf, ck, o, i, kh, kw, upsample, g, add_to=ggy)
                if want[1]:
                    gx2 = _dgrad_modconv(gy, hd, okp, o, i, kh, kw, upsample, g)
            if want[2] or want[3]:
                gw3b, gs2b = _fold_weight_gradient(gwk, gwk.shape[-1], w3, s, dd, scale, style.dtype, cotangent=v)
                gw3 = gw3b if gw3 is None else gw3 + gw3b
                gs2 = gs2b if gs2 is None else gs2 + gs2b
        gw = gw3.reshape(1, o, i, kh, kw) if (gw3 is not None and want[2]) else None
        return (ggy, gx2, gw, gs2 if want[3] else None) + tail


class _ModulatedConv(Function):

    @staticmethod
    def forward(ctx, x, weight, style, demodulate, upsample, act_bias=None, noise=None, noise_w=None, alpha=0.2,
                act_scale=1.0, fuse_act=False, head_slot=None, input_act=None):
        dev = _lib.require_gpu(x, weight, style)
        ctx.input_act = input_act if input_act is not None and input_act.armed else None
        ctx.head_slot = head_slot
        if head_slot is not None and fuse_act:
            ctx.set_materialize_grads(False)
            head_slot.armed = True
        _, o, i, kh, kw = weight.shape
        b, t = x.shape[0], kh * kw
        scale = math.sqrt(2.0) / math.sqrt(i * t)
        w3 = weight.detach().reshape(o, i, t)
        s = style.detach().float().contiguous()
        d = None
        esz = 2 if x.dtype == torch.bfloat16 else 4
        ck = _round_up(i, 128 // esz)
        kind = "up2" if upsample else "conv"
        img = _param_images(weight, torch.float32, 1.0, kind, modulation=True)
        base = img["f"][0] if img is not None else _cached(weight, "mb" + kind, torch.float32, 1.0, lambda: (
            (w3.permute(2, 0, 1).reshape(t * o, 1, i) if upsample else w3.transpose(1, 2)).contiguous(), 0))[0]
        rows = t * o if upsample else o
        wk = torch.empty((b, rows, 1 if upsample else t, ck), dtype=x.dtype, device=dev)
        if demodulate:
            wsq = img["wsq"] if img is not None else \
                _cached(weight, "wsq", torch.float32, 1.0, lambda: (w3.square().sum(dim=2).contiguous(), 0))[0]
            d = torch.empty((b, o), dtype=torch.float32, device=dev)
            with _lib.on_device(dev):
                code = _lib.lib().msg_modulate_weights(base.data_ptr(), wsq.data_ptr(), s.data_ptr(), wk.data_ptr(),
                                                       d.data_ptr(), _lib.dtype_code(wk), b, rows, o,
                                                       1 if upsample else t, i, ck, scale, 1e-8, _lib.stream_of(dev))
            _lib.check(code, "msg_modulate_weights")
        else:
            _scale_rows_cols(base, None, s, wk, scale)
        g = Geometry(kind, kh, kw, 1, kh // 2, x.shape[2:], True)
        act = None
        holder = [] if any(ctx.needs_input_grad) else None
        if fuse_act:
            assert not upsample, "the upsampling layers blur before their activation"
            act = (*_act_operands(act_bias, noise, noise_w, (b, o, *g.y_hw)), alpha, act_scale, holder)
        if upsample:
            y = _launch_fprop(x, wk, ck, None, 4 * o, g.x_hw, 1, 1, 1, 0, 1, True, True, i, mode=g.mode)
        else:
            y = _launch_fprop(x, wk, ck, None, o, g.y_hw, kh, kw, 1, kh // 2, 1, False, True, i, act=act, mode=g.mode)
        ctx.save_for_backward(x, weight, style, d if d is not None else torch.empty(0, device=dev),
                              y if fuse_act else None, noise if fuse_act else None)
        ctx.cfg = (demodulate, upsample, g, scale)
        ctx.act = (alpha, act_scale, act_bias is not None, noise is not None,
                   None if noise_w is None else noise_w.shape) if fuse_act else None
        ctx.bias_param = act_bias
        ctx.mask = holder[0] if holder else None
        return y

    @staticmethod
    def backward(ctx, gy):
        x, weight, style, d, y_act, noise = ctx.saved_tensors
        demodulate, upsample, g, scale = ctx.cfg
        _, o, i, kh, kw = weight.shape
        b, t = x.shape[0], kh * kw
        need = list(ctx.needs_input_grad)
        need[1], need[2] = _consumed(ctx, 1, 1), _consumed(ctx, 2, 2)
        gb = gnw = None
        slot = ctx.head_slot
        if ctx.act is not None:
            from .op_static.fused_act import FusedLeakyReLUFunctionBackward, act_backward_with_head
            alpha, act_scale, has_bias, has_noise, nw_shape = ctx.act
            head, head_dgrad = slot.take() if slot is not None else (None, None)
            fused = None
            if head is not None:
                fused = act_backward_with_head(gy, head, y_act.shape, noise if has_noise else None,
                                               ctx.bias_param if has_bias else None, has_bias, alpha, act_scale, ctx.mask)
                if fused is None:
                    gh = head_dgrad()
                    gy = gh if gy is None else gy + gh
            if fused is not None:
                gy, gb, gnw = fused
            elif gy is None:
                return (None,) * 13
            else:
                gy, gb, gnw = _derive(FusedLeakyReLUFunctionBackward, gy, y_act, noise if has_noise else None,
                                      ctx.bias_param if has_bias else False, alpha, act_scale, ctx.mask)
            gb = gb if has_bias and need[5] else None
            gnw = gnw.reshape(nw_shape) if has_noise and need[7] else None
        tail = (None, None, gb, None, gnw, None, None, None, None, None)
        if ctx.act is None and slot is not None and slot.armed and need[0] and not torch.is_grad_enabled() and \
                fused_head_ok(gy, weight, b, demodulate, upsample):
            gyc, wt, st = gy, weight, style
            slot.head = (gyc, weight.detach().reshape(o, i).float().contiguous(), style.detach().float().contiguous(), scale)
            slot.dgrad = lambda: _modconv_backward(x, wt, st, d, gyc, demodulate, upsample, g, scale,
                                                   [True, False, False])[0]
            need[0] = False
        fused_ok = i <= 512 and t <= 9
        if torch.is_grad_enabled() and fused_ok and _NATIVE_SECOND_ORDER and b <= _MODCONV_BWD_BATCH and x.is_cuda:
            gx, gw, gs = _derive(_ModConvGrad, gy, x, weight, style, d if demodulate else None, demodulate, upsample, g, scale,
                                            tuple(need[:3]))
            return (gx, gw, gs) + tail
        if torch.is_grad_enabled() or not fused_ok:
            with torch.enable_grad():
                ins = [v for v, n in zip((x, weight, style), need[:3]) if n]
                y2 = _modulated_composite(x, weight, style, demodulate, upsample)
                grads = list(torch.autograd.grad(y2, ins, gy, create_graph=torch.is_grad_enabled(), allow_unused=True))
            out = [grads.pop(0) if n else None for n in need[:3]]
            return (out[0], out[1], out[2]) + tail
        if b > _MODCONV_BWD_BATCH:
            gxs, gws, gss = [], [], []
            for lo in range(0, b, _MODCONV_BWD_BATCH):
                hi = min(b, lo + _MODCONV_BWD_BATCH)
                cgx, cgw, cgs = _modconv_backward(x[lo:hi], weight, style[lo:hi], d[lo:hi] if demodulate else d,
                                                  gy[lo:hi], demodulate, upsample, g, scale, need)
                gxs.append(cgx); gws.append(cgw); gss.append(cgs)
            gx = torch.cat(gxs) if need[0] else None
            gw = torch.stack(gws).sum(dim=0) if gws[0] is not None else None
            gs = torch.cat(gss) if gss[0] is not None else None
            return (gx, gw, gs) + tail
        gx, gw, gs = _modconv_backward(x, weight, style, d, gy, demodulate, upsample, g, scale, need, direct=True,
                                       act_bwd=ctx.input_act)
        return (gx, gw, gs) + tail


def fused_head_ok(gy, weight, b, demodulate, upsample) -> bool:
    _, o, _, kh, kw = weight.shape
    return gy is not None and gy.is_cuda and gy.dtype == torch.bfloat16 and kh == 1 and kw == 1 and o <= 8 and \
        not demodulate and not upsample and b <= _MODCONV_BWD_BATCH and HEAD_GRAD_FUSION


HEAD_GRAD_FUSION = bool(int(os.environ.get("MSG_HEAD_GRAD_FUSION", "1")))


def modulated_conv2d_bias_act(x, weight, style, demodulate, act_bias, noise, noise_weight, negative_slope=0.2,
                              scale=1.0, head_slot=None, input_act=None):
    return _ModulatedConv.apply(x, weight, style, bool(demodulate), False, act_bias, noise, noise_weight,
                                float(negative_slope), float(scale), True, head_slot, input_act)


def modulated_conv2d(x, weight, style, demodulate, upsample, head_slot=None):
    if head_slot is None:
        return _ModulatedConv.apply(x, weight, style, bool(demodulate), bool(upsample))
    return _ModulatedConv.apply(x, weight, style, bool(demodulate), bool(upsample), None, None, None, 0.2, 1.0, False,
                                head_slot)
```

multi_stylegan_amd/csrc/conv_fprop.hip:

```cpp
#include "conv_dispatch.h"
#include <stdlib.h>

typedef __bf16 bf16v8 __attribute__((ext_vector_type(8)));
typedef const __attribute__((address_space(1))) char* gptr_t;
typedef const __attribute__((address_space(1))) u32x4* gvec_t;
typedef __attribute__((address_space(3))) char* lds_t;

struct ConvParams {
    int B, IH, IW, Cx, Ck, OH, OW, N, ldy;
    int kh, kw, stride, pad, in_up, pixel_shuffle, per_sample;
    long long x_bstride, w_bstride, y_bstride;
    int Mtot, n_chunks, n_iters, m_tiles, n_tiles;
    ActEpilogue act;
};

constexpr int BM = 128, BN = 128, ROWB = 128;
constexpr int STAGE_BYTES = (BM + BN) * ROWB;
__device__ __attribute__((aligned(256))) unsigned int g_zero_page[16384];

__device__ __forceinline__ int swz(int row, int slot) { return row * ROWB + ((slot ^ ((row >> 1) & 7)) << 4); }

template <int SPLIT>
__device__ __forceinline__ void split_park(const u32x4& raw, char* dst) {
    uint2 pl[3];
#pragma unroll
    for (int h = 0; h < 2; ++h) {
        const float x0 = __uint_as_float(raw[2 * h]), x1 = __uint_as_float(raw[2 * h + 1]);
        const unsigned hp = (unsigned)f2bf(x0) | ((unsigned)f2bf(x1) << 16);
        const float r0 = x0 - __uint_as_float(hp << 16), r1 = x1 - __uint_as_float(hp & 0xffff0000u);
        const unsigned mp = (unsigned)f2bf(r0) | ((unsigned)f2bf(r1) << 16);
        (h ? pl[0].y : pl[0].x) = hp;
        (h ? pl[1].y : pl[1].x) = mp;
        if constexpr (SPLIT == 3) {
            const float q0 = r0 - __uint_as_float(mp << 16), q1 = r1 - __uint_as_float(mp & 0xffff0000u);
            (h ? pl[2].y : pl[2].x) = (unsigned)f2bf(q0) | ((unsigned)f2bf(q1) << 16);
        }
    }
#pragma unroll
    for (int p = 0; p < SPLIT; ++p) *reinterpret_cast<uint2*>(dst + p * 64) = pl[p];
}

template <typename T, bool DMA, int LEAN = 0, int SPLIT = 0>
__global__ __launch_bounds__(256, LEAN ? LEAN : 2) void conv_fprop_kernel(const T* __restrict__ x, const T* __restrict__ w,
                                                            T* __restrict__ y, const float* __restrict__ bias,
                                                            ConvParams p) {
    constexpr int VEC = 16 / sizeof(T);
    constexpr int BKE = ROWB / sizeof(T);
    static_assert(!LEAN || (!DMA && sizeof(T) == 2), "lean variant: bf16, register staging");
    static_assert(SPLIT == 0 || sizeof(T) == 4, "split-bf16 products are a mode of the fp32-storage kernel");
    static_assert(SPLIT == 0 || !DMA, "the split planes are written from the staging registers");
    constexpr int SROW = SPLIT ? SPLIT * 64 + 16 : ROWB;
    constexpr int STAGE = SPLIT ? (BM + BN) * SROW : STAGE_BYTES;
    constexpr bool ONE_STAGE = LEAN != 0 || SPLIT == 3;
    constexpr int SMEM_BYTES = ONE_STAGE ? (STAGE > 65536 || sizeof(T) == 2 ? STAGE : 65536) : 2 * STAGE;
    __shared__ __attribute__((aligned(16))) char smem[SMEM_BYTES];

    const int tid = threadIdx.x, lane = tid & 63, wid = tid >> 6;
    const int wm = wid >> 1, wn = wid & 1;
    const int lr = lane & 31, lh = lane >> 5;
    const unsigned L = xcd_remap(blockIdx.x, gridDim.x);
    const int n0 = (int)(L % p.n_tiles) * BN;
    const int m0 = (int)(L / p.n_tiles) * BM;
    const int bz = blockIdx.z;

    const int wid_u = __builtin_amdgcn_readfirstlane(wid);
    const int slot_phys = tid & 7;
    int row_of[4];
#pragma unroll
    for (int j = 0; j < 4; ++j) row_of[j] = DMA ? (wid * 32 + 8 * j + (lane >> 3)) : ((tid >> 3) + 32 * j);
    const int slot = DMA ? 0 : slot_phys;
    int a_ih0[4], a_iw0[4];
    long long a_boff[4];
    int a_slot[4];
    bool a_ok[4];
    const int ohw = p.OH * p.OW;
#pragma unroll
    for (int j = 0; j < 4; ++j) {
        const int m = m0 + row_of[j];
        const int slot_j = DMA ? (slot_phys ^ ((row_of[j] >> 1) & 7)) : slot_phys;
        a_ok[j] = m < p.Mtot;
        const int mm = a_ok[j] ? m : 0;
        const int b = p.per_sample ? bz : mm / ohw;
        const int pix = p.per_sample ? mm : mm - b * ohw;
        const int oh = pix / p.OW, ow = pix - oh * p.OW;
        a_ih0[j] = oh * p.stride - p.pad;
        a_iw0[j] = ow * p.stride - p.pad;
        a_boff[j] = ((long long)((DMA && p.per_sample) ? 0 : b) * p.x_bstride + slot_j * VEC +
                     ((long long)a_ih0[j] * p.IW + a_iw0[j]) * p.Cx) * (long long)sizeof(T);
        a_slot[j] = slot_j;
    }
    const int taps = p.kh * p.kw;
    const gptr_t xbase = (gptr_t)x;
    const gptr_t zbase = (gptr_t)g_zero_page;
    const long long zoff = slot_phys * 16;
    gptr_t pa[4];
    gptr_t pb[4];
    {
        const gptr_t wb = (gptr_t)w + (p.per_sample ? (long long)bz * p.w_bstride : 0) * (long long)sizeof(T);
#pragma unroll
        for (int j = 0; j < 4; ++j) {
            const int n = n0 + row_of[j];
            const bool ok = n < p.N;
            pb[j] = (ok ? wb : zbase) + (ok ? ((long long)n * taps * p.Ck + a_slot[j] * VEC) * (long long)sizeof(T) : zoff);
            pa[j] = zbase;
        }
    }
    msg_desc_t d_x = {0, 0, 0, 0}, d_w = {0, 0, 0, 0};
    unsigned lds0 = 0;
    int va[4] = {MSG_DMA_OOB, MSG_DMA_OOB, MSG_DMA_OOB, MSG_DMA_OOB}, vb[4] = {MSG_DMA_OOB, MSG_DMA_OOB, MSG_DMA_OOB, MSG_DMA_OOB};
    if constexpr (DMA) {
        d_x = msg_make_desc((const char*)x + (p.per_sample ? (long long)bz * p.x_bstride * (long long)sizeof(T) : 0));
        d_w = msg_make_desc((const char*)w + (p.per_sample ? (long long)bz * p.w_bstride * (long long)sizeof(T) : 0));
        lds0 = (unsigned)(unsigned long long)(lds_t)smem;
#pragma unroll
        for (int j = 0; j < 4; ++j) {
            const int n = n0 + row_of[j];
            vb[j] = n < p.N ? (int)(((long long)n * taps * p.Ck + a_slot[j] * VEC) * (long long)sizeof(T)) : MSG_DMA_OOB;
        }
    }
    const bool ragged = (p.Cx % BKE) != 0;
    int ld_tap = -1, ld_chunk = p.n_chunks - 1;
    int kh_ = 0, kw_ = -1;
    int st_off[4];
#pragma unroll
    for (int j = 0; j < 4; ++j) st_off[j] = swz(row_of[j], a_slot[j]);

    f32x16 acc[2][2];
#pragma unroll
    for (int i = 0; i < 2; ++i)
#pragma unroll
        for (int j = 0; j < 2; ++j)
#pragma unroll
            for (int e = 0; e < 16; ++e) acc[i][j][e] = 0.f;

    u32x4 ra[4], rb[4];
    int dma_stage = 0;
    auto load_next = [&]() __attribute__((always_inline)) {
        if (++ld_chunk == p.n_chunks) {
            ld_chunk = 0;
            ++ld_tap;
            if (++kw_ == p.kw) { kw_ = 0; ++kh_; }
            if (p.in_up == 1) {
                const long long tap_off = ((long long)kh_ * p.IW + kw_) * p.Cx * (long long)sizeof(T);
#pragma unroll
                for (int j = 0; j < 4; ++j) {
                    const bool ok = a_ok[j] & ((unsigned)(a_ih0[j] + kh_) < (unsigned)p.IH) &
                                    ((unsigned)(a_iw0[j] + kw_) < (unsigned)p.IW);
                    pa[j] = (ok ? xbase : zbase) + (ok ? a_boff[j] + tap_off : zoff);
                    if constexpr (DMA) va[j] = ok ? (int)(a_boff[j] + tap_off) : MSG_DMA_OOB;
                }
            } else {
#pragma unroll
                for (int j = 0; j < 4; ++j) {
                    const int ih = a_ih0[j] + kh_, iw = a_iw0[j] + kw_;
                    bool ok = a_ok[j] & (ih >= 0) & (iw >= 0) & (ih % p.in_up == 0) & (iw % p.in_up == 0);
                    const int ihs = ih / p.in_up, iws = iw / p.in_up;
                    ok = ok & (ihs < p.IH) & (iws < p.IW);
                    const long long off = a_boff[j] + ((long long)(ihs - a_ih0[j]) * p.IW + (iws - a_iw0[j])) * p.Cx * (long long)sizeof(T);
                    pa[j] = (ok ? xbase : zbase) + (ok ? off : zoff);
                    if constexpr (DMA) va[j] = ok ? (int)off : MSG_DMA_OOB;
                }
            }
        }
#pragma unroll
        for (int j = 0; j < 4; ++j) {
            const bool c_bad = ragged && (ld_chunk * BKE + a_slot[j] * VEC + VEC > p.Cx);
            gptr_t a_addr = pa[j];
            if (c_bad) a_addr = zbase + zoff;
            if constexpr (DMA) {
                const unsigned la = lds0 + dma_stage * STAGE + (wid_u * 32 + 8 * j) * ROWB;
                msg_dma16(d_x, la, c_bad ? MSG_DMA_OOB : va[j], ld_chunk * ROWB);
                msg_dma16(d_w, la + BM * ROWB, vb[j], (ld_tap * p.n_chunks + ld_chunk) * ROWB);
            } else {
                ra[j] = *(gvec_t)a_addr;
                rb[j] = *(gvec_t)pb[j];
            }
            pa[j] += ROWB;
            pb[j] += ROWB;
        }
    };
    auto park = [&](int stage) __attribute__((always_inline)) {
        char* sa = smem + stage * STAGE;
        if constexpr (SPLIT != 0) {
            char* sb = sa + BM * SROW;
#pragma unroll
            for (int j = 0; j < 4; ++j) {
                split_park<SPLIT>(ra[j], sa + row_of[j] * SROW + slot_phys * 8);
                split_park<SPLIT>(rb[j], sb + row_of[j] * SROW + slot_phys * 8);
            }
            return;
        }
        char* sb = sa + BM * ROWB;
#pragma unroll
        for (int j = 0; j < 4; ++j) {
            *reinterpret_cast<u32x4*>(sa + st_off[j]) = ra[j];
            *reinterpret_cast<u32x4*>(sb + st_off[j]) = rb[j];
        }
    };
    auto mma_step = [&](const char* sa) __attribute__((always_inline)) {
        const char* sb = sa + BM * ROWB;
        if constexpr (sizeof(T) == 2) {
            bf16v8 fa[2][2], fb[2][2];
#pragma unroll
            for (int t = 0; t < 2; ++t) {
                fa[0][t] = *reinterpret_cast<const bf16v8*>(sa + swz(wm * 64 + t * 32 + lr, lh));
                fb[0][t] = *reinterpret_cast<const bf16v8*>(sb + swz(wn * 64 + t * 32 + lr, lh));
            }
#pragma unroll
            for (int kk = 0; kk < 4; ++kk) {
                if (kk + 1 < 4) {
#pragma unroll
                    for (int t = 0; t < 2; ++t) {
                        fa[(kk + 1) & 1][t] = *reinterpret_cast<const bf16v8*>(sa + swz(wm * 64 + t * 32 + lr, 2 * (kk + 1) + lh));
                        fb[(kk + 1) & 1][t] = *reinterpret_cast<const bf16v8*>(sb + swz(wn * 64 + t * 32 + lr, 2 * (kk + 1) + lh));
                    }
                }
#pragma unroll
                for (int i = 0; i < 2; ++i)
#pragma unroll
                    for (int j = 0; j < 2; ++j)
                        acc[i][j] = __builtin_amdgcn_mfma_f32_32x32x16_bf16(fb[kk & 1][j], fa[kk & 1][i], acc[i][j], 0, 0, 0);
            }
            __builtin_amdgcn_sched_group_barrier(0x100, 8, 0);
            __builtin_amdgcn_sched_group_barrier(0x008, 4, 0);
            __builtin_amdgcn_sched_group_barrier(0x100, 4, 0);
            __builtin_amdgcn_sched_group_barrier(0x008, 4, 0);
            __builtin_amdgcn_sched_group_barrier(0x100, 4, 0);
            __builtin_amdgcn_sched_group_barrier(0x008, 8, 0);
        } else if constexpr (SPLIT != 0) {
            const char* sbs = sa + BM * SROW;
#pragma unroll
            for (int sstep = 0; sstep < 2; ++sstep) {
                bf16v8 af[SPLIT][2], bf[SPLIT][2];
#pragma unroll
                for (int t = 0; t < 2; ++t)
#pragma unroll
                    for (int pl = 0; pl < SPLIT; ++pl) {
                        af[pl][t] = *reinterpret_cast<const bf16v8*>(sa + (wm * 64 + t * 32 + lr) * SROW + pl * 64 + (2 * sstep + lh) * 16);
                        bf[pl][t] = *reinterpret_cast<const bf16v8*>(sbs + (wn * 64 + t * 32 + lr) * SROW + pl * 64 + (2 * sstep + lh) * 16);
                    }
#pragma unroll
                for (int i = 0; i < 2; ++i)
#pragma unroll
                    for (int j = 0; j < 2; ++j) {
#pragma unroll
                        for (int order = SPLIT - 1; order >= 0; --order)
#pragma unroll
                            for (int pa = 0; pa <= order; ++pa)
                                acc[i][j] = __builtin_amdgcn_mfma_f32_32x32x16_bf16(bf[order - pa][j], af[pa][i], acc[i][j], 0, 0, 0);
                    }
            }
        } else {
#pragma unroll
            for (int q = 0; q < 4; ++q) {
                f32x4 fa[2], fb[2];
#pragma unroll
                for (int t = 0; t < 2; ++t) {
                    fa[t] = *reinterpret_cast<const f32x4*>(sa + swz(wm * 64 + t * 32 + lr, 4 * lh + q));
                    fb[t] = *reinterpret_cast<const f32x4*>(sb + swz(wn * 64 + t * 32 + lr, 4 * lh + q));
                }
#pragma unroll
                for (int e = 0; e < 4; ++e)
#pragma unroll
                    for (int i = 0; i < 2; ++i)
#pragma unroll
                        for (int j = 0; j < 2; ++j)
                            acc[i][j] = __builtin_amdgcn_mfma_f32_32x32x2f32(fb[j][e], fa[i][e], acc[i][j], 0, 0, 0);
            }
        }
    };
    if constexpr (ONE_STAGE) {
        load_next();
        for (int it = 0; it < p.n_iters; ++it) {
            if (it) __syncthreads();
            park(0);
            if (it + 1 < p.n_iters) load_next();
            __syncthreads();
            mma_step(smem);
        }
    } else {
        if constexpr (DMA) {
            dma_stage = 0;
            load_next();
        } else {
            load_next();
            park(0);
            if (p.n_iters > 1) load_next();
        }
        for (int it = 0; it < p.n_iters; ++it) {
            if constexpr (DMA) asm volatile("s_waitcnt vmcnt(0)" ::: "memory");
            __syncthreads();
            if constexpr (DMA) {
                if (it + 1 < p.n_iters) { dma_stage = (it + 1) & 1; load_next(); }
            } else {
                if (it + 1 < p.n_iters) park((it + 1) & 1);
                if (it + 2 < p.n_iters) load_next();
            }
            mma_step(smem + (it & 1) * STAGE);
        }
    }
    if constexpr (DMA) asm volatile("s_waitcnt vmcnt(0)" ::: "memory");
    __syncthreads();

    constexpr int PITCH = 64 * sizeof(T);
    constexpr int UNITB = 4 * sizeof(T);
    char* ep = smem + wid * (64 * PITCH);
#pragma unroll
    for (int j = 0; j < 2; ++j)
#pragma unroll
        for (int g = 0; g < 4; ++g) {
            const int unit = 8 * j + 2 * g + lh;
            float bv[4] = {0.f, 0.f, 0.f, 0.f};
            if (bias) {
                const int nb = n0 + wn * 64 + 4 * unit;
#pragma unroll
                for (int e = 0; e < 4; ++e) bv[e] = nb + e < p.N ? bias[nb + e] : 0.f;
            }
#pragma unroll
            for (int i = 0; i < 2; ++i) {
                const int row = i * 32 + lr;
                char* dstl = ep + row * PITCH + ((unit ^ (row & 15)) * UNITB);
                if constexpr (sizeof(T) == 2) {
                    uint2 pk;
                    pk.x = (unsigned)f2bf(acc[i][j][4 * g + 0] + bv[0]) | ((unsigned)f2bf(acc[i][j][4 * g + 1] + bv[1]) << 16);
                    pk.y = (unsigned)f2bf(acc[i][j][4 * g + 2] + bv[2]) | ((unsigned)f2bf(acc[i][j][4 * g + 3] + bv[3]) << 16);
                    *reinterpret_cast<uint2*>(dstl) = pk;
                } else {
                    *reinterpret_cast<f32x4*>(dstl) = f32x4{acc[i][j][4 * g + 0] + bv[0], acc[i][j][4 * g + 1] + bv[1],
                                                            acc[i][j][4 * g + 2] + bv[2], acc[i][j][4 * g + 3] + bv[3]};
                }
            }
        }
    constexpr int LPR = 64 / VEC;
    constexpr int RPP = 64 / LPR;
    constexpr int NPASS = 64 / RPP;
    const int er = lane / LPR, ec = (lane % LPR) * VEC;
    const int n = n0 + wn * 64 + ec;
    int nn = n, q = 0;
    if (p.pixel_shuffle) { const int oc = p.N >> 2; q = n / oc; nn = n - q * oc; }
    const int lim = p.pixel_shuffle ? (p.N >> 2) - nn : p.N - n;
    const bool n_ok = n < p.N;
    int gp[NPASS];
    float a_bias[VEC], a_noise[NPASS];
    {
        const int m_first = min(m0 + wm * 64 + er, p.Mtot - 1);
        int b = p.per_sample ? bz : m_first / ohw;
        const int pix0 = p.per_sample ? m_first : m_first - b * ohw;
        int oh = pix0 / p.OW, ow = pix0 - oh * p.OW;
        const bool want_noise = p.act.enabled == 1 && p.act.noise;
        const float nw = want_noise ? p.act.noise_w[0] : 0.f;
        if (p.act.enabled == 1) {
#pragma unroll
            for (int e = 0; e < VEC; ++e) a_bias[e] = (p.act.bias && n + e < p.N) ? p.act.bias[n + e] : 0.f;
        }
#pragma unroll
        for (int pass = 0; pass < NPASS; ++pass) {
            const bool ok = m0 + wm * 64 + pass * RPP + er < p.Mtot;
            const int pix = oh * p.OW + ow;
            const int g = p.pixel_shuffle ? ((b * 2 * p.OH + 2 * oh + (q >> 1)) * (2 * p.OW) + 2 * ow + (q & 1))
                                          : b * ohw + pix;
            gp[pass] = ok ? g : -1;
            a_noise[pass] = (want_noise && ok) ? nw * p.act.noise[(long long)(p.act.noise_batch == 1 ? 0 : b) * ohw + pix] : 0.f;
            ow += RPP;
            while (ow >= p.OW) { ow -= p.OW; ++oh; }
            if (!p.per_sample) while (oh >= p.OH) { oh -= p.OH; ++b; }
        }
    }
    __syncthreads();
    u32x4 v[NPASS];
#pragma unroll
    for (int pass = 0; pass < NPASS; ++pass) {
        const int row = pass * RPP + er;
        if constexpr (sizeof(T) == 2)
            v[pass] = *reinterpret_cast<const u32x4*>(ep + row * PITCH + (((lane & 7) ^ ((row & 15) >> 1)) << 4));
        else
            v[pass] = *reinterpret_cast<const u32x4*>(ep + row * PITCH + (((lane & 15) ^ (row & 15)) << 4));
    }
    if constexpr (sizeof(T) == 2) {
        if (er & 1) {
#pragma unroll
            for (int pass = 0; pass < NPASS; ++pass) v[pass] = u32x4{v[pass][2], v[pass][3], v[pass][0], v[pass][1]};
        }
    }
    if (p.act.enabled == 1) {
#pragma unroll
        for (int pass = 0; pass < NPASS; ++pass) v[pass] = act_epilogue_apply<T>(v[pass], a_bias, a_noise[pass], p.act.alpha, p.act.scale);
    } else if (p.act.enabled == 2) {
        const T* rbase = reinterpret_cast<const T*>(p.act.residual) + (n_ok ? n : 0);
        u32x4 r[NPASS];
#pragma unroll
        for (int pass = 0; pass < NPASS; ++pass)
            r[pass] = *reinterpret_cast<const u32x4*>(rbase + (long long)max(gp[pass], 0) * p.act.res_ld);
#pragma unroll
        for (int pass = 0; pass < NPASS; ++pass) v[pass] = residual_epilogue_apply<T>(v[pass], r[pass], p.act.res_gain);
    }
    T* ybase = y + (p.pixel_shuffle ? nn : n);
    if (n_ok && lim >= VEC) {
#pragma unroll
        for (int pass = 0; pass < NPASS; ++pass)
            if (gp[pass] >= 0) *reinterpret_cast<u32x4*>(ybase + (long long)gp[pass] * p.ldy) = v[pass];
    } else if (n_ok) {
#pragma unroll
        for (int pass = 0; pass < NPASS; ++pass) {
            if (gp[pass] < 0) continue;
            T tmp[VEC];
            *reinterpret_cast<u32x4*>(tmp) = v[pass];
            T* dst = ybase + (long long)gp[pass] * p.ldy;
            for (int e = 0; e < lim; ++e) dst[e] = tmp[e];
        }
    }
}

static ConvPlan conv_generic_select(const ConvProblem& q) {
    const int n_iters = q.kh * q.kw * (q.Ck / (ROWB / q.esz()));
    static const int variant = msg_tunable("MSG_CONV_VARIANT", 0);
    const bool dma = q.fits31() && (variant == 1 || (variant == 0 && n_iters >= 8));
    static const int lean_max = msg_tunable("MSG_CONV_LEAN", 4);
    ConvPlan plan{CONV_REG, BM, BN, true};
    if (q.split) plan.kernel = CONV_REG_SPLIT;
    else if (dma) plan.kernel = CONV_DMA;
    else if (q.dtype == MSG_BF16 && n_iters <= lean_max) plan.kernel = CONV_REG_LEAN;
    const long long mtot = q.mtot(), blocks = ((mtot + BM - 1) / BM) * ((q.N + BN - 1) / BN);
    plan.supported = mtot < (1ll << 31) && blocks < (1ll << 31) &&
                     (long long)(n_iters + 1) * ROWB + 128 <= 65536;
    return plan;
}

static void conv_generic_launch(const ConvProblem& q, const ConvPlan& plan, const void* x, const void* w, const float* bias, void* y,
                                const ActEpilogue* act, void* stream) {
    ConvParams p{};
    conv_fill_common(p, q, act);
    conv_fill_taps(p, q);
    p.n_chunks = q.Ck / (ROWB / q.esz());
    p.n_iters = q.kh * q.kw * p.n_chunks;
    p.m_tiles = (int)((q.mtot() + BM - 1) / BM);
    p.n_tiles = (q.N + BN - 1) / BN;
    dim3 grid((unsigned)((long long)p.m_tiles * p.n_tiles), 1, q.samples());
#define GENERIC(T, ...) hipLaunchKernelGGL((conv_fprop_kernel<T, __VA_ARGS__>), grid, dim3(256), 0, (hipStream_t)stream, \
                                           (const T*)x, (const T*)w, (T*)y, bias, p)
    const bool bf16 = q.dtype == MSG_BF16;
    if (bf16 && plan.kernel == CONV_REG_LEAN) GENERIC(bf16_t, false, 3);
    else if (bf16 && plan.kernel == CONV_DMA) GENERIC(bf16_t, true);
    else if (bf16) GENERIC(bf16_t, false);
    else if (plan.kernel == CONV_REG_SPLIT) GENERIC(float, false, 0, 3);
    else if (plan.kernel == CONV_DMA) GENERIC(float, true);
    else GENERIC(float, false);
#undef GENERIC
}

ConvPlan conv_fprop_select(const ConvProblem& q, const ActEpilogue* act, bool has_bias) {
    ConvPlan plan;
    if (conv_thin_eligible(q, act, &plan)) return plan;
    if (conv_upconv_eligible(q, act, has_bias, &plan)) return plan;
    if (conv_row3_eligible(q, act, has_bias, &plan)) return plan;
    if (conv_pp_eligible(q, &plan)) return plan;
    return conv_generic_select(q);
}

static ConvProblem conv_problem(int dtype, int B, int IH, int IW, int Cx, int Ck, int OH, int OW, int N, int ldy,
                                int kh, int kw, int stride, int pad, int in_up, int pixel_shuffle, long long w_batch_stride) {
    const int split = dtype == MSG_F32_SPLIT ? 3 : 0;
    return ConvProblem{split ? (int)MSG_F32 : dtype, split, B, IH, IW, Cx, Ck, OH, OW, N, ldy, kh, kw, stride, pad, in_up, pixel_shuffle,
                       w_batch_stride};
}

static ConvPlan fprop_select(const ConvProblem& q, int act_mode, bool has_bias) {
    ActEpilogue act{};
    act.enabled = act_mode;
    return conv_fprop_select(q, &act, has_bias);
}

static int fprop_check(const ConvProblem& q, const void* const* io) {
    if (q.B < 0 || q.IH <= 0 || q.IW <= 0 || q.OH <= 0 || q.OW <= 0 || q.N <= 0 || q.kh <= 0 || q.kw <= 0 || q.stride <= 0 ||
        q.in_up <= 0 || q.Cx <= 0 || q.Ck <= 0 || q.ldy <= 0 || (io && (!io[0] || !io[1] || !io[2])))
        return MSG_EINVAL;
    if (q.dtype != MSG_F32 && q.dtype != MSG_BF16) return MSG_EUNSUPPORTED;
    const int vec = 16 / q.esz(), bke = ROWB / q.esz();
    if (q.Ck % bke || q.Cx % vec || (io && (((uintptr_t)io[0] | (uintptr_t)io[1] | (uintptr_t)io[2]) & 15u))) return MSG_EUNSUPPORTED;
    if (q.ldy % vec || (q.pixel_shuffle && (q.N % 4 || (q.N / 4) % vec))) return MSG_EUNSUPPORTED;
    if (q.in_up > 1 && q.stride != 1) return MSG_EUNSUPPORTED;
    return MSG_OK;
}

static int fprop_plan_for(const ConvProblem& q, int act_mode, bool has_bias, const void* const* io, ConvPlan* plan) {
    if (q.B == 0) return MSG_OK;
    const int rc = fprop_check(q, io);
    if (rc != MSG_OK) return rc;
    *plan = fprop_select(q, act_mode, has_bias);
    return plan->supported ? MSG_OK : MSG_EUNSUPPORTED;
}

static bool is_row3(const ConvPlan& plan) { return plan.kernel == CONV_ROW3 || plan.kernel == CONV_ROW3N; }

static void act_backward_partials(const ConvProblem& q, const ConvPlan& plan, long long* rows, long long* entries) {
    *rows = *entries = 0;
    if (!is_row3(plan) || q.ldy != q.N) return;
    const long long tiles = (q.mtot() / plan.tile_m) * q.samples();
    *rows = tiles * 2;
    *entries = tiles * (q.N / plan.tile_n) * 4;
}

static int plan_code(ConvKernel kernel) {
    switch (kernel) {
        case CONV_THIN_N: case CONV_THIN_K: return MSG_PLAN_THIN;
        case CONV_UPCONV: return MSG_PLAN_UPCONV;
        case CONV_ROW3: return MSG_PLAN_ROW3;
        case CONV_ROW3N: return MSG_PLAN_ROW3N;
        case CONV_PP: return MSG_PLAN_PP;
        case CONV_DMA: return MSG_PLAN_DMA;
        default: return MSG_PLAN_REG;
    }
}

extern "C" int msg_conv2d_fprop_launch_plan(int dtype, int B, int IH, int IW, int Cx, int Ck, int OH, int OW, int N, int ldy,
                                            int kh, int kw, int stride, int pad, int in_up, int pixel_shuffle,
                                            long long w_batch_stride, int has_bias, int epilogue, long long* out, int n_out_fields) {
    if (epilogue < 0 || epilogue > 3 || (epilogue && (has_bias || in_up != 1 || pixel_shuffle))) return MSG_EINVAL;
    const ConvProblem q = conv_problem(dtype, B, IH, IW, Cx, Ck, OH, OW, N, ldy, kh, kw, stride, pad, in_up, pixel_shuffle, w_batch_stride);
    ConvPlan plan;
    const int rc = fprop_plan_for(q, epilogue, has_bias != 0, nullptr, &plan);
    if (rc != MSG_OK) return rc;
    long long fields[MSG_FPLAN_FIELDS] = {};
    if (q.B) {
        fields[0] = plan_code(plan.kernel); fields[1] = plan.tile_m; fields[2] = plan.tile_n;
        if (epilogue == 3) act_backward_partials(q, plan, &fields[3], &fields[4]);
    }
    for (int k = 0; k < MSG_FPLAN_FIELDS && k < n_out_fields; ++k) out[k] = fields[k];
    return MSG_OK;
}

static ConvProblem conv_query_problem(int dtype, int B, int IH, int IW, int Cx, int Ck, int OH, int OW, int N, int kh, int kw,
                                      long long w_batch_stride) {
    return conv_problem(dtype, B, IH, IW, Cx, Ck, OH, OW, N, N <= 8 ? 8 : (N + 7) / 8 * 8, kh, kw, 1, kh / 2, 1, 0, w_batch_stride);
}
extern "C" int msg_conv2d_fprop_plan(int dtype, int B, int IH, int IW, int Cx, int Ck, int OH, int OW, int N,
                                     int kh, int kw, long long w_batch_stride) {
    return plan_code(fprop_select(conv_query_problem(dtype, B, IH, IW, Cx, Ck, OH, OW, N, kh, kw, w_batch_stride), 0, false).kernel);
}
extern "C" long long msg_conv2d_fprop_act_backward_workspace(int dtype, int B, int IH, int IW, int Cx, int Ck, int OH, int OW,
                                                             int N, int kh, int kw, long long w_batch_stride, int has_noise) {
    const ConvProblem q = conv_query_problem(dtype, B, IH, IW, Cx, Ck, OH, OW, N, kh, kw, w_batch_stride);
    long long rows, entries;
    act_backward_partials(q, fprop_select(q, 3, false), &rows, &entries);
    return rows ? rows * N + (has_noise ? entries : 0) : 0;
}
extern "C" int msg_conv2d_fprop_upconv_eligible(int B, int IH, int IW, int Cx, int Ck, int OH, int OW, int N, int kh, int kw,
                                                int stride, int pad, int in_up, int pixel_shuffle, long long w_batch_stride) {
    return fprop_select(conv_problem(MSG_BF16, B, IH, IW, Cx, Ck, OH, OW, N, N / 4, kh, kw, stride, pad, in_up, pixel_shuffle,
                                     w_batch_stride), 0, false).kernel == CONV_UPCONV;
}
extern "C" int msg_conv2d_fprop_thin_eligible(int B, int IH, int IW, int Cx, int Ck, int OH, int OW, int N, int ldy,
                                              int kh, int kw, int stride, int pad, int in_up, int pixel_shuffle,
                                              int act_mode) {
    const ConvKernel kernel = fprop_select(conv_problem(MSG_BF16, B, IH, IW, Cx, Ck, OH, OW, N, ldy, kh, kw, stride, pad, in_up,
                                                        pixel_shuffle, 0), act_mode, false).kernel;
    return kernel == CONV_THIN_N ? 1 : kernel == CONV_THIN_K ? 2 : 0;
}

static int conv2d_fprop_impl(const void* x, const void* w, const float* bias, void* y, const ConvProblem& q,
                             const ActEpilogue& act, void* stream) {
    const void* const io[3] = {x, w, y};
    ConvPlan plan;
    const int rc = fprop_plan_for(q, act.enabled, bias != nullptr, io, &plan);
    if (rc != MSG_OK || q.B == 0) return rc;
    if (act.mask && !is_row3(plan)) return MSG_EUNSUPPORTED;
    switch (plan.kernel) {
        case CONV_THIN_N: case CONV_THIN_K: conv_thin_launch(q, plan, x, w, bias, y, &act, stream); break;
        case CONV_UPCONV: conv_upconv_launch(q, plan, x, w, y, stream); break;
        case CONV_ROW3: case CONV_ROW3N: conv_row3_launch(q, plan, x, w, bias, y, &act, stream); break;
        case CONV_PP: conv_pp_launch(q, plan, x, w, bias, y, &act, stream); break;
        case CONV_DMA: case CONV_REG: case CONV_REG_LEAN: case CONV_REG_SPLIT:
            conv_generic_launch(q, plan, x, w, bias, y, &act, stream); break;
    }
    return MSG_CHECK_LAUNCH();
}

extern "C" int msg_conv2d_fprop(const void* x, const void* w, const float* bias, void* y, int dtype,
                                int B, int IH, int IW, int Cx, int Ck, int OH, int OW, int N, int ldy,
                                int kh, int kw, int stride, int pad, int in_up, int pixel_shuffle,
                                long long w_batch_stride, void* stream) {
    ActEpilogue act{};
    return conv2d_fprop_impl(x, w, bias, y, conv_problem(dtype, B, IH, IW, Cx, Ck, OH, OW, N, ldy, kh, kw, stride, pad, in_up,
                                                         pixel_shuffle, w_batch_stride), act, stream);
}

extern "C" int msg_conv2d_fprop_act_mask(const void* x, const void* w, void* y, int dtype,
                                         int B, int IH, int IW, int Cx, int Ck, int OH, int OW, int N, int ldy,
                                         int kh, int kw, int stride, int pad, long long w_batch_stride,
                                         const float* act_bias, const float* noise, const float* noise_weight,
                                         int noise_batch, float alpha, float scale, unsigned char* mask, void* stream) {
    if (noise && (!noise_weight || (noise_batch != 1 && noise_batch != B))) return MSG_EINVAL;
    ActEpilogue act{act_bias, noise, noise_weight, noise_batch, 1, alpha, scale, nullptr, 0, 0.f, mask};
    return conv2d_fprop_impl(x, w, nullptr, y, conv_problem(dtype, B, IH, IW, Cx, Ck, OH, OW, N, ldy, kh, kw, stride, pad, 1, 0,
                                                            w_batch_stride), act, stream);
}

extern "C" int msg_conv2d_fprop_act(const void* x, const void* w, void* y, int dtype,
                                    int B, int IH, int IW, int Cx, int Ck, int OH, int OW, int N, int ldy,
                                    int kh, int kw, int stride, int pad, long long w_batch_stride,
                                    const float* act_bias, const float* noise, const float* noise_weight,
                                    int noise_batch, float alpha, float scale, void* stream) {
    return msg_conv2d_fprop_act_mask(x, w, y, dtype, B, IH, IW, Cx, Ck, OH, OW, N, ldy, kh, kw, stride, pad, w_batch_stride,
                                     act_bias, noise, noise_weight, noise_batch, alpha, scale, nullptr, stream);
}

extern "C" int msg_conv2d_fprop_residual(const void* x, const void* w, void* y, int dtype,
                                         int B, int IH, int IW, int Cx, int Ck, int OH, int OW, int N, int ldy,
                                         int kh, int kw, int stride, int pad, long long w_batch_stride,
                                         const void* residual, int res_ld, float gain, void* stream) {
    if (!residual || res_ld < N || (((uintptr_t)residual) & 15u) || res_ld % (dtype == MSG_BF16 ? 8 : 4)) return MSG_EINVAL;
    ActEpilogue act{};
    act.enabled = 2; act.residual = residual; act.res_ld = res_ld; act.res_gain = gain;
    return conv2d_fprop_impl(x, w, nullptr, y, conv_problem(dtype, B, IH, IW, Cx, Ck, OH, OW, N, ldy, kh, kw, stride, pad, 1, 0,
                                                            w_batch_stride), act, stream);
}

extern "C" int msg_conv2d_fprop_act_backward(const void* x, const void* w, void* y, int dtype,
                                             int B, int IH, int IW, int Cx, int Ck, int OH, int OW, int N, int ldy,
                                             int kh, int kw, int stride, int pad, long long w_batch_stride,
                                             const void* residual, int res_ld,
                                             const unsigned char* sign_mask, int mask_tile_m, int mask_tile_n,
                                             const void* sign_map, int sign_ld, float alpha, float scale,
                                             float* grad_bias, const float* noise, int noise_batch, float* grad_noise_weight,
                                             float* ws, long long ws_floats, void* stream) {
    if (B == 0) return MSG_OK;
    if (!sign_mask == !sign_map) return MSG_EINVAL;
    const ConvProblem q = conv_problem(dtype, B, IH, IW, Cx, Ck, OH, OW, N, ldy, kh, kw, stride, pad, 1, 0, w_batch_stride);
    const void* const io[3] = {x, w, y};
    ConvPlan plan;
    const int rc = fprop_plan_for(q, 3, false, io, &plan);
    if (rc != MSG_OK) return rc;
    long long rows, entries;
    act_backward_partials(q, plan, &rows, &entries);
    if (!rows) return MSG_EUNSUPPORTED;
    if (sign_mask && (mask_tile_m <= 0 || mask_tile_n <= 0 || mask_tile_n % 128 || N % mask_tile_n || (((uintptr_t)sign_mask) & 15u) ||
                      (mask_tile_m != 1 && mask_tile_m % 64) || ((long long)B * OH * OW) % mask_tile_m))
        return MSG_EINVAL;
    if (sign_map && (sign_ld < N || sign_ld % 8 || (((uintptr_t)sign_map) & 15u))) return MSG_EINVAL;
    if (residual && (res_ld < N || res_ld % 8 || (((uintptr_t)residual) & 15u))) return MSG_EINVAL;
    const bool has_noise = noise && grad_noise_weight;
    if (has_noise && noise_batch != 1 && noise_batch != B) return MSG_EINVAL;
    const long long need_b = grad_bias ? rows * N : 0, need_n = has_noise ? entries : 0;
    if (need_b + need_n > 0 && (!ws || ws_floats < need_b + need_n)) return MSG_EINVAL;
    ActEpilogue act{};
    act.enabled = 3; act.alpha = alpha; act.scale = scale;
    act.residual = residual; act.res_ld = res_ld; act.res_gain = 1.f;
    act.mask = const_cast<unsigned char*>(sign_mask); act.mask_tile_m = mask_tile_m; act.mask_tile_n = mask_tile_n;
    act.sign_src = sign_map; act.sign_ld = sign_ld;
    act.noise = has_noise ? noise : nullptr; act.noise_batch = noise_batch;
    act.part_b = grad_bias ? ws : nullptr;
    act.part_n = has_noise ? ws + need_b : nullptr;
    conv_row3_launch(q, plan, x, w, nullptr, y, &act, stream);
    if (MSG_CHECK_LAUNCH() != MSG_OK) return MSG_ELAUNCH;
    return msg_bias_act_reduce_launch(act.part_b, grad_bias, N, rows, act.part_n, grad_noise_weight, entries, stream);
}
```

Before: 156.5.

## Add split-K path for generic conv fprop with fp32 workspace and finish pass

Adds a k-split mode to the generic conv forward kernels. When the grid is too small to fill the GPU, the reduction over taps and channels is divided into slices that write fp32 partials to a scratch workspace. A finish pass then sums the slices and applies the bias, activation or residual epilogue. A cost model picks the slice count automatically, and the Python wrapper allocates scratch and routes calls to new _ws entry points. This trades extra workspace traffic and a second launch for more parallelism on small-grid layers.

```diff
diff --git a/include/msg_hip.h b/include/msg_hip.h
--- a/include/msg_hip.h
+++ b/include/msg_hip.h
@@ -211,6 +211,33 @@
 int msg_conv2d_fprop_launch_plan(int dtype, int B, int IH, int IW, int Cx, int Ck, int OH, int OW, int N, int ldy,
                                  int kh, int kw, int stride, int pad, int in_up, int pixel_shuffle,
                                  long long w_batch_stride, int has_bias, int epilogue, long long* out, int n_out_fields);
+enum { MSG_FPROP_K_AUTO = 0, MSG_FKSPLIT_FIELDS = 2 };
+int msg_conv2d_fprop_ksplit_plan(int dtype, int B, int IH, int IW, int Cx, int Ck, int OH, int OW, int N, int ldy,
+                                 int kh, int kw, int stride, int pad, int in_up, int pixel_shuffle,
+                                 long long w_batch_stride, int has_bias, int epilogue, int k_slices,
+                                 long long* out, int n_out_fields);
+int msg_conv2d_fprop_ksplit_phases(int phases);
+int msg_conv2d_fprop_ws(const void* x, const void* w, const float* bias, void* y, int dtype,
+                        int B, int IH, int IW, int Cx, int Ck, int OH, int OW, int N, int ldy,
+                        int kh, int kw, int stride, int pad, int in_up, int pixel_shuffle,
+                        long long w_batch_stride, float* ws, long long ws_floats, int k_slices, void* stream);
+int msg_conv2d_fprop_act_ws(const void* x, const void* w, void* y, int dtype,
+                            int B, int IH, int IW, int Cx, int Ck, int OH, int OW, int N, int ldy,
+                            int kh, int kw, int stride, int pad, long long w_batch_stride,
+                            const float* act_bias, const float* noise, const float* noise_weight,
+                            int noise_batch, float alpha, float scale,
+                            float* ws, long long ws_floats, int k_slices, void* stream);
+int msg_conv2d_fprop_act_mask_ws(const void* x, const void* w, void* y, int dtype,
+                                 int B, int IH, int IW, int Cx, int Ck, int OH, int OW, int N, int ldy,
+                                 int kh, int kw, int stride, int pad, long long w_batch_stride,
+                                 const float* act_bias, const float* noise, const float* noise_weight,
+                                 int noise_batch, float alpha, float scale, unsigned char* mask,
+                                 float* ws, long long ws_floats, int k_slices, void* stream);
+int msg_conv2d_fprop_residual_ws(const void* x, const void* w, void* y, int dtype,
+                                 int B, int IH, int IW, int Cx, int Ck, int OH, int OW, int N, int ldy,
+                                 int kh, int kw, int stride, int pad, long long w_batch_stride,
+                                 const void* residual, int res_ld, float gain,
+                                 float* ws, long long ws_floats, int k_slices, void* stream);
 enum {
     MSG_WPLAN_GENERIC = 0,
     MSG_WPLAN_DMA = 1,
diff --git a/multi_stylegan_amd/conv_ops.py b/multi_stylegan_amd/conv_ops.py
--- a/multi_stylegan_amd/conv_ops.py
+++ b/multi_stylegan_amd/conv_ops.py
@@ -373,6 +373,13 @@
 
 
 @functools.lru_cache(maxsize=None)
+def _fprop_ksplit(*args):
+    out = (ctypes.c_longlong * _lib.MSG_FKSPLIT_FIELDS)()
+    ok = _lib.lib().msg_conv2d_fprop_ksplit_plan(*args, _lib.MSG_FPROP_K_AUTO, ctypes.addressof(out), len(out)) == _lib.MSG_OK
+    return (out[0], out[1]) if ok and out[0] > 1 else (1, 0)
+
+
+@functools.lru_cache(maxsize=None)
 def _wgrad_plan(*geom):
     out = (ctypes.c_longlong * _lib.MSG_WPLAN_FIELDS)()
     _lib.check(_lib.lib().msg_conv2d_wgrad_plan(*geom, _lib.MSG_WGRAD_K_AUTO, ctypes.addressof(out), len(out)),
@@ -406,26 +413,29 @@
     if flops is None:
         flops = 2.0 * b * oh * ow * n * kh * kw * c_real / (in_up * in_up)
     key, sign_tile = "conv_fprop", None
+    geom = (b, ih, iw, cx, ck, oh, ow, n, ldy, kh, kw, stride, pad, in_up, int(pixel_shuffle), wstride, int(bias is not None),
+            2 if residual is not None else int(act is not None))
+    code_ = _contraction_code(x, mode)
+    slices, need = _fprop_ksplit(code_, *geom)
+    ws = (_lib.scratch_ptr(need, dev), need, slices) if slices > 1 else None
     sign_holder = act[5] if act is not None and len(act) > 5 else None
     if _lib.kernel_clock.enabled or sign_holder is not None:
-        _, key, sign_tile, _, _ = _fprop_plan(_lib.dtype_code(x), b, ih, iw, cx, ck, oh, ow, n, ldy, kh, kw, stride, pad, in_up,
-                                              int(pixel_shuffle), wstride, int(bias is not None),
-                                              2 if residual is not None else int(act is not None))
+        _, key, sign_tile, _, _ = _fprop_plan(_lib.dtype_code(x), *geom)
     if _lib.kernel_clock.enabled and _CLOCK_SHAPES:
         key += f"|B{b} {ih}x{iw}->{oh}x{ow} {c_real}->{n} {kh}x{kw} s{stride} up{in_up}" \
-               f"{' ps' if pixel_shuffle else ''}{' per-sample' if per_sample else ''}|"
-    with _lib.on_device(dev), _lib.kernel_clock.span((key, 'bf16' if x.dtype == torch.bfloat16 else 'f32'), flops):
+               f"{' ps' if pixel_shuffle else ''}{' per-sample' if per_sample else ''}{f' slices{slices}' if ws else ''}|"
+    with _lib.on_device(dev):
         if residual is not None:
             assert bias is None and act is None and in_up == 1 and not pixel_shuffle
             rv, res_ld = _nhwc_view(residual[0])
             assert rv.shape == (b, n, oh, ow) and rv.dtype == x.dtype
-            code = _lib.lib().msg_conv2d_fprop_residual(
-                xv.data_ptr(), wk.data_ptr(), y.data_ptr(), _contraction_code(x, mode), b, ih, iw, cx, ck, oh, ow, n, ldy, kh, kw,
-                stride, pad, wstride, rv.data_ptr(), res_ld, float(residual[1]), _lib.stream_of(dev))
+            args = (xv.data_ptr(), wk.data_ptr(), y.data_ptr(), code_, b, ih, iw, cx, ck, oh, ow, n, ldy, kh, kw,
+                    stride, pad, wstride, rv.data_ptr(), res_ld, float(residual[1]))
+            fn = _lib.lib().msg_conv2d_fprop_residual_ws if ws else _lib.lib().msg_conv2d_fprop_residual
         elif act is None:
-            code = _lib.lib().msg_conv2d_fprop(
-                xv.data_ptr(), wk.data_ptr(), _lib.ptr(bias), y.data_ptr(), _contraction_code(x, mode), b, ih, iw, cx, ck, oh,
-                ow, n, ldy, kh, kw, stride, pad, in_up, int(pixel_shuffle), wstride, _lib.stream_of(dev))
+            args = (xv.data_ptr(), wk.data_ptr(), _lib.ptr(bias), y.data_ptr(), code_, b, ih, iw, cx, ck, oh,
+                    ow, n, ldy, kh, kw, stride, pad, in_up, int(pixel_shuffle), wstride)
+            fn = _lib.lib().msg_conv2d_fprop_ws if ws else _lib.lib().msg_conv2d_fprop
         else:
             assert bias is None and in_up == 1 and not pixel_shuffle
             act_bias, noise, noise_w, alpha, scale = act[:5]
@@ -436,10 +446,24 @@
                 mask = sign_mask_for(b, n, oh, ow, x.dtype, dev)
                 if mask is not None:
                     sign_holder.append((mask, sign_tile, sign_tile))
-            code = _lib.lib().msg_conv2d_fprop_act_mask(
-                xv.data_ptr(), wk.data_ptr(), y.data_ptr(), _contraction_code(x, mode), b, ih, iw, cx, ck, oh, ow, n, ldy, kh, kw,
-                stride, pad, wstride, _lib.ptr(act_bias), _lib.ptr(noise), _lib.ptr(noise_w),
-                1 if noise is None else noise.shape[0], float(alpha), float(scale), _lib.ptr(mask), _lib.stream_of(dev))
+            args = (xv.data_ptr(), wk.data_ptr(), y.data_ptr(), code_, b, ih, iw, cx, ck, oh, ow, n, ldy, kh, kw,
+                    stride, pad, wstride, _lib.ptr(act_bias), _lib.ptr(noise), _lib.ptr(noise_w),
+                    1 if noise is None else noise.shape[0], float(alpha), float(scale), _lib.ptr(mask))
+            fn = _lib.lib().msg_conv2d_fprop_act_mask_ws if ws else _lib.lib().msg_conv2d_fprop_act_mask
+        args += (*(ws or ()), _lib.stream_of(dev))
+        dt = 'bf16' if x.dtype == torch.bfloat16 else 'f32'
+        if ws and _lib.kernel_clock.enabled:
+            _lib.lib().msg_conv2d_fprop_ksplit_phases(1)
+            with _lib.kernel_clock.span((key, dt), flops):
+                code = fn(*args)
+            _lib.lib().msg_conv2d_fprop_ksplit_phases(2)
+            with _lib.kernel_clock.span(("ksplit_finish" + key[key.find("|"):] if "|" in key else "ksplit_finish", dt),
+                                        4.0 * b * oh * ow * n * slices + b * oh * ow * n * x.element_size()):
+                code = code or fn(*args)
+            _lib.lib().msg_conv2d_fprop_ksplit_phases(3)
+        else:
+            with _lib.kernel_clock.span((key, dt), flops):
+                code = fn(*args)
     _lib.check(code, "msg_conv2d_fprop")
     return y
 
diff --git a/multi_stylegan_amd/csrc/conv_fprop.hip b/multi_stylegan_amd/csrc/conv_fprop.hip
--- a/multi_stylegan_amd/csrc/conv_fprop.hip
+++ b/multi_stylegan_amd/csrc/conv_fprop.hip
@@ -12,10 +12,15 @@
     long long x_bstride, w_bstride, y_bstride;
     int Mtot, n_chunks, n_iters, m_tiles, n_tiles;
     ActEpilogue act;
+    int k_slices;
+    float* ws;
 };
 
 constexpr int BM = 128, BN = 128, ROWB = 128;
 constexpr int STAGE_BYTES = (BM + BN) * ROWB;
+constexpr int KSPLIT_ROUND_WGS = 512, KSPLIT_MIN_STEPS = 4;
+constexpr int FINISH_CHUNK = 4;
+constexpr int KSPLIT_FIXED = 600, KSPLIT_SLAB = 400, KSPLIT_PER_SLICE = 120, KSPLIT_TRAFFIC = 8;
 __device__ __attribute__((aligned(256))) unsigned int g_zero_page[16384];
 
 __device__ __forceinline__ int swz(int row, int slot) { return row * ROWB + ((slot ^ ((row >> 1) & 7)) << 4); }
@@ -40,268 +45,14 @@
     for (int p = 0; p < SPLIT; ++p) *reinterpret_cast<uint2*>(dst + p * 64) = pl[p];
 }
 
-template <typename T, bool DMA, int LEAN = 0, int SPLIT = 0>
-__global__ __launch_bounds__(256, LEAN ? LEAN : 2) void conv_fprop_kernel(const T* __restrict__ x, const T* __restrict__ w,
-                                                            T* __restrict__ y, const float* __restrict__ bias,
-                                                            ConvParams p) {
+template <typename T>
+__device__ __forceinline__ void conv_tile_epilogue(const f32x16 (&acc)[2][2], char* smem, T* __restrict__ y,
+                                                   const float* __restrict__ bias, const ConvParams& p, int m0, int n0, int bz) {
     constexpr int VEC = 16 / sizeof(T);
-    constexpr int BKE = ROWB / sizeof(T);
-    static_assert(!LEAN || (!DMA && sizeof(T) == 2), "lean variant: bf16, register staging");
-    static_assert(SPLIT == 0 || sizeof(T) == 4, "split-bf16 products are a mode of the fp32-storage kernel");
-    static_assert(SPLIT == 0 || !DMA, "the split planes are written from the staging registers");
-    constexpr int SROW = SPLIT ? SPLIT * 64 + 16 : ROWB;
-    constexpr int STAGE = SPLIT ? (BM + BN) * SROW : STAGE_BYTES;
-    constexpr bool ONE_STAGE = LEAN != 0 || SPLIT == 3;
-    constexpr int SMEM_BYTES = ONE_STAGE ? (STAGE > 65536 || sizeof(T) == 2 ? STAGE : 65536) : 2 * STAGE;
-    __shared__ __attribute__((aligned(16))) char smem[SMEM_BYTES];
-
     const int tid = threadIdx.x, lane = tid & 63, wid = tid >> 6;
     const int wm = wid >> 1, wn = wid & 1;
     const int lr = lane & 31, lh = lane >> 5;
-    const unsigned L = xcd_remap(blockIdx.x, gridDim.x);
-    const int n0 = (int)(L % p.n_tiles) * BN;
-    const int m0 = (int)(L / p.n_tiles) * BM;
-    const int bz = blockIdx.z;
-
-    const int wid_u = __builtin_amdgcn_readfirstlane(wid);
-    const int slot_phys = tid & 7;
-    int row_of[4];
-#pragma unroll
-    for (int j = 0; j < 4; ++j) row_of[j] = DMA ? (wid * 32 + 8 * j + (lane >> 3)) : ((tid >> 3) + 32 * j);
-    const int slot = DMA ? 0 : slot_phys;
-    int a_ih0[4], a_iw0[4];
-    long long a_boff[4];
-    int a_slot[4];
-    bool a_ok[4];
     const int ohw = p.OH * p.OW;
-#pragma unroll
-    for (int j = 0; j < 4; ++j) {
-        const int m = m0 + row_of[j];
-        const int slot_j = DMA ? (slot_phys ^ ((row_of[j] >> 1) & 7)) : slot_phys;
-        a_ok[j] = m < p.Mtot;
-        const int mm = a_ok[j] ? m : 0;
-        const int b = p.per_sample ? bz : mm / ohw;
-        const int pix = p.per_sample ? mm : mm - b * ohw;
-        const int oh = pix / p.OW, ow = pix - oh * p.OW;
-        a_ih0[j] = oh * p.stride - p.pad;
-        a_iw0[j] = ow * p.stride - p.pad;
-        a_boff[j] = ((long long)((DMA && p.per_sample) ? 0 : b) * p.x_bstride + slot_j * VEC +
-                     ((long long)a_ih0[j] * p.IW + a_iw0[j]) * p.Cx) * (long long)sizeof(T);
-        a_slot[j] = slot_j;
-    }
-    const int taps = p.kh * p.kw;
-    const gptr_t xbase = (gptr_t)x;
-    const gptr_t zbase = (gptr_t)g_zero_page;
-    const long long zoff = slot_phys * 16;
-    gptr_t pa[4];
-    gptr_t pb[4];
-    {
-        const gptr_t wb = (gptr_t)w + (p.per_sample ? (long long)bz * p.w_bstride : 0) * (long long)sizeof(T);
-#pragma unroll
-        for (int j = 0; j < 4; ++j) {
-            const int n = n0 + row_of[j];
-            const bool ok = n < p.N;
-            pb[j] = (ok ? wb : zbase) + (ok ? ((long long)n * taps * p.Ck + a_slot[j] * VEC) * (long long)sizeof(T) : zoff);
-            pa[j] = zbase;
-        }
-    }
-    msg_desc_t d_x = {0, 0, 0, 0}, d_w = {0, 0, 0, 0};
-    unsigned lds0 = 0;
-    int va[4] = {MSG_DMA_OOB, MSG_DMA_OOB, MSG_DMA_OOB, MSG_DMA_OOB}, vb[4] = {MSG_DMA_OOB, MSG_DMA_OOB, MSG_DMA_OOB, MSG_DMA_OOB};
-    if constexpr (DMA) {
-        d_x = msg_make_desc((const char*)x + (p.per_sample ? (long long)bz * p.x_bstride * (long long)sizeof(T) : 0));
-        d_w = msg_make_desc((const char*)w + (p.per_sample ? (long long)bz * p.w_bstride * (long long)sizeof(T) : 0));
-        lds0 = (unsigned)(unsigned long long)(lds_t)smem;
-#pragma unroll
-        for (int j = 0; j < 4; ++j) {
-            const int n = n0 + row_of[j];
-            vb[j] = n < p.N ? (int)(((long long)n * taps * p.Ck + a_slot[j] * VEC) * (long long)sizeof(T)) : MSG_DMA_OOB;
-        }
-    }
-    const bool ragged = (p.Cx % BKE) != 0;
-    int ld_tap = -1, ld_chunk = p.n_chunks - 1;
-    int kh_ = 0, kw_ = -1;
-    int st_off[4];
-#pragma unroll
-    for (int j = 0; j < 4; ++j) st_off[j] = swz(row_of[j], a_slot[j]);
-
-    f32x16 acc[2][2];
-#pragma unroll
-    for (int i = 0; i < 2; ++i)
-#pragma unroll
-        for (int j = 0; j < 2; ++j)
-#pragma unroll
-            for (int e = 0; e < 16; ++e) acc[i][j][e] = 0.f;
-
-    u32x4 ra[4], rb[4];
-    int dma_stage = 0;
-    auto load_next = [&]() __attribute__((always_inline)) {
-        if (++ld_chunk == p.n_chunks) {
-            ld_chunk = 0;
-            ++ld_tap;
-            if (++kw_ == p.kw) { kw_ = 0; ++kh_; }
-            if (p.in_up == 1) {
-                const long long tap_off = ((long long)kh_ * p.IW + kw_) * p.Cx * (long long)sizeof(T);
-#pragma unroll
-                for (int j = 0; j < 4; ++j) {
-                    const bool ok = a_ok[j] & ((unsigned)(a_ih0[j] + kh_) < (unsigned)p.IH) &
-                                    ((unsigned)(a_iw0[j] + kw_) < (unsigned)p.IW);
-                    pa[j] = (ok ? xbase : zbase) + (ok ? a_boff[j] + tap_off : zoff);
-                    if constexpr (DMA) va[j] = ok ? (int)(a_boff[j] + tap_off) : MSG_DMA_OOB;
-                }
-            } else {
-#pragma unroll
-                for (int j = 0; j < 4; ++j) {
-                    const int ih = a_ih0[j] + kh_, iw = a_iw0[j] + kw_;
-                    bool ok = a_ok[j] & (ih >= 0) & (iw >= 0) & (ih % p.in_up == 0) & (iw % p.in_up == 0);
-                    const int ihs = ih / p.in_up, iws = iw / p.in_up;
-                    ok = ok & (ihs < p.IH) & (iws < p.IW);
-                    const long long off = a_boff[j] + ((long long)(ihs - a_ih0[j]) * p.IW + (iws - a_iw0[j])) * p.Cx * (long long)sizeof(T);
-                    pa[j] = (ok ? xbase : zbase) + (ok ? off : zoff);
-                    if constexpr (DMA) va[j] = ok ? (int)off : MSG_DMA_OOB;
-                }
-            }
-        }
-#pragma unroll
-        for (int j = 0; j < 4; ++j) {
-            const bool c_bad = ragged && (ld_chunk * BKE + a_slot[j] * VEC + VEC > p.Cx);
-            gptr_t a_addr = pa[j];
-            if (c_bad) a_addr = zbase + zoff;
-            if constexpr (DMA) {
-                const unsigned la = lds0 + dma_stage * STAGE + (wid_u * 32 + 8 * j) * ROWB;
-                msg_dma16(d_x, la, c_bad ? MSG_DMA_OOB : va[j], ld_chunk * ROWB);
-                msg_dma16(d_w, la + BM * ROWB, vb[j], (ld_tap * p.n_chunks + ld_chunk) * ROWB);
-            } else {
-                ra[j] = *(gvec_t)a_addr;
-                rb[j] = *(gvec_t)pb[j];
-            }
-            pa[j] += ROWB;
-            pb[j] += ROWB;
-        }
-    };
-    auto park = [&](int stage) __attribute__((always_inline)) {
-        char* sa = smem + stage * STAGE;
-        if constexpr (SPLIT != 0) {
-            char* sb = sa + BM * SROW;
-#pragma unroll
-            for (int j = 0; j < 4; ++j) {
-                split_park<SPLIT>(ra[j], sa + row_of[j] * SROW + slot_phys * 8);
-                split_park<SPLIT>(rb[j], sb + row_of[j] * SROW + slot_phys * 8);
-            }
-            return;
-        }
-        char* sb = sa + BM * ROWB;
-#pragma unroll
-        for (int j = 0; j < 4; ++j) {
-            *reinterpret_cast<u32x4*>(sa + st_off[j]) = ra[j];
-            *reinterpret_cast<u32x4*>(sb + st_off[j]) = rb[j];
-        }
-    };
-    auto mma_step = [&](const char* sa) __attribute__((always_inline)) {
-        const char* sb = sa + BM * ROWB;
-        if constexpr (sizeof(T) == 2) {
-            bf16v8 fa[2][2], fb[2][2];
-#pragma unroll
-            for (int t = 0; t < 2; ++t) {
-                fa[0][t] = *reinterpret_cast<const bf16v8*>(sa + swz(wm * 64 + t * 32 + lr, lh));
-                fb[0][t] = *reinterpret_cast<const bf16v8*>(sb + swz(wn * 64 + t * 32 + lr, lh));
-            }
-#pragma unroll
-            for (int kk = 0; kk < 4; ++kk) {
-                if (kk + 1 < 4) {
-#pragma unroll
-                    for (int t = 0; t < 2; ++t) {
-                        fa[(kk + 1) & 1][t] = *reinterpret_cast<const bf16v8*>(sa + swz(wm * 64 + t * 32 + lr, 2 * (kk + 1) + lh));
-                        fb[(kk + 1) & 1][t] = *reinterpret_cast<const bf16v8*>(sb + swz(wn * 64 + t * 32 + lr, 2 * (kk + 1) + lh));
-                    }
-                }
-#pragma unroll
-                for (int i = 0; i < 2; ++i)
-#pragma unroll
-                    for (int j = 0; j < 2; ++j)
-                        acc[i][j] = __builtin_amdgcn_mfma_f32_32x32x16_bf16(fb[kk & 1][j], fa[kk & 1][i], acc[i][j], 0, 0, 0);
-            }
-            __builtin_amdgcn_sched_group_barrier(0x100, 8, 0);
-            __builtin_amdgcn_sched_group_barrier(0x008, 4, 0);
-            __builtin_amdgcn_sched_group_barrier(0x100, 4, 0);
-            __builtin_amdgcn_sched_group_barrier(0x008, 4, 0);
-            __builtin_amdgcn_sched_group_barrier(0x100, 4, 0);
-            __builtin_amdgcn_sched_group_barrier(0x008, 8, 0);
-        } else if constexpr (SPLIT != 0) {
-            const char* sbs = sa + BM * SROW;
-#pragma unroll
-            for (int sstep = 0; sstep < 2; ++sstep) {
-                bf16v8 af[SPLIT][2], bf[SPLIT][2];
-#pragma unroll
-                for (int t = 0; t < 2; ++t)
-#pragma unroll
-                    for (int pl = 0; pl < SPLIT; ++pl) {
-                        af[pl][t] = *reinterpret_cast<const bf16v8*>(sa + (wm * 64 + t * 32 + lr) * SROW + pl * 64 + (2 * sstep + lh) * 16);
-                        bf[pl][t] = *reinterpret_cast<const bf16v8*>(sbs + (wn * 64 + t * 32 + lr) * SROW + pl * 64 + (2 * sstep + lh) * 16);
-                    }
-#pragma unroll
-                for (int i = 0; i < 2; ++i)
-#pragma unroll
-                    for (int j = 0; j < 2; ++j) {
-#pragma unroll
-                        for (int order = SPLIT - 1; order >= 0; --order)
-#pragma unroll
-                            for (int pa = 0; pa <= order; ++pa)
-                                acc[i][j] = __builtin_amdgcn_mfma_f32_32x32x16_bf16(bf[order - pa][j], af[pa][i], acc[i][j], 0, 0, 0);
-                    }
-            }
-        } else {
-#pragma unroll
-            for (int q = 0; q < 4; ++q) {
-                f32x4 fa[2], fb[2];
-#pragma unroll
-                for (int t = 0; t < 2; ++t) {
-                    fa[t] = *reinterpret_cast<const f32x4*>(sa + swz(wm * 64 + t * 32 + lr, 4 * lh + q));
-                    fb[t] = *reinterpret_cast<const f32x4*>(sb + swz(wn * 64 + t * 32 + lr, 4 * lh + q));
-                }
-#pragma unroll
-                for (int e = 0; e < 4; ++e)
-#pragma unroll
-                    for (int i = 0; i < 2; ++i)
-#pragma unroll
-                        for (int j = 0; j < 2; ++j)
-                            acc[i][j] = __builtin_amdgcn_mfma_f32_32x32x2f32(fb[j][e], fa[i][e], acc[i][j], 0, 0, 0);
-            }
-        }
-    };
-    if constexpr (ONE_STAGE) {
-        load_next();
-        for (int it = 0; it < p.n_iters; ++it) {
-            if (it) __syncthreads();
-            park(0);
-            if (it + 1 < p.n_iters) load_next();
-            __syncthreads();
-            mma_step(smem);
-        }
-    } else {
-        if constexpr (DMA) {
-            dma_stage = 0;
-            load_next();
-        } else {
-            load_next();
-            park(0);
-            if (p.n_iters > 1) load_next();
-        }
-        for (int it = 0; it < p.n_iters; ++it) {
-            if constexpr (DMA) asm volatile("s_waitcnt vmcnt(0)" ::: "memory");
-            __syncthreads();
-            if constexpr (DMA) {
-                if (it + 1 < p.n_iters) { dma_stage = (it + 1) & 1; load_next(); }
-            } else {
-                if (it + 1 < p.n_iters) park((it + 1) & 1);
-                if (it + 2 < p.n_iters) load_next();
-            }
-            mma_step(smem + (it & 1) * STAGE);
-        }
-    }
-    if constexpr (DMA) asm volatile("s_waitcnt vmcnt(0)" ::: "memory");
-    __syncthreads();
-
     constexpr int PITCH = 64 * sizeof(T);
     constexpr int UNITB = 4 * sizeof(T);
     char* ep = smem + wid * (64 * PITCH);
@@ -411,6 +162,352 @@
     }
 }
 
+__device__ __forceinline__ long long ksplit_slab(const ConvParams& p, unsigned tile, int bz, int slice) {
+    return ((((long long)bz * p.m_tiles * p.n_tiles + tile) * p.k_slices + slice) * (long long)(BM * BN / 4));
+}
+__device__ __forceinline__ void ksplit_store(const f32x16 (&acc)[2][2], f32x4* __restrict__ slab, const ConvParams& p, int m0) {
+    const int lane = threadIdx.x & 63, wid = threadIdx.x >> 6;
+#pragma unroll
+    for (int i = 0; i < 2; ++i) {
+        if (m0 + (wid >> 1) * 64 + i * 32 + (lane & 31) >= p.Mtot) continue;
+#pragma unroll
+        for (int j = 0; j < 2; ++j)
+#pragma unroll
+            for (int g = 0; g < 4; ++g)
+                slab[((((wid * 2 + i) * 2 + j) * 4 + g) << 6) + lane] =
+                    f32x4{acc[i][j][4 * g + 0], acc[i][j][4 * g + 1], acc[i][j][4 * g + 2], acc[i][j][4 * g + 3]};
+    }
+}
+
+template <typename T>
+__global__ __launch_bounds__(256) void conv_fprop_finish_kernel(const float* __restrict__ ws, T* __restrict__ y,
+                                                                const float* __restrict__ bias, ConvParams p) {
+    __shared__ __attribute__((aligned(16))) char smem[4 * 64 * 64 * sizeof(T)];
+    const int lane = threadIdx.x & 63, wid = threadIdx.x >> 6;
+    const unsigned L = xcd_remap(blockIdx.x, gridDim.x);
+    const int n0 = (int)(L % p.n_tiles) * BN;
+    const int m0 = (int)(L / p.n_tiles) * BM;
+    const int bz = blockIdx.z;
+    const f32x4* __restrict__ slab = reinterpret_cast<const f32x4*>(ws) + ksplit_slab(p, L, bz, 0);
+    f32x16 acc[2][2];
+#pragma unroll
+    for (int i = 0; i < 2; ++i) {
+        const bool ok = m0 + (wid >> 1) * 64 + i * 32 + (lane & 31) < p.Mtot;
+#pragma unroll
+        for (int j = 0; j < 2; ++j)
+#pragma unroll
+            for (int e = 0; e < 16; ++e) acc[i][j][e] = 0.f;
+        if (!ok) continue;
+        for (int s0 = 0; s0 < p.k_slices; s0 += FINISH_CHUNK) {
+            f32x4 v[FINISH_CHUNK][2][4];
+#pragma unroll
+            for (int c = 0; c < FINISH_CHUNK; ++c) {
+                if (s0 + c >= p.k_slices) break;
+                const f32x4* __restrict__ src = slab + (long long)(s0 + c) * (BM * BN / 4) + lane;
+#pragma unroll
+                for (int j = 0; j < 2; ++j)
+#pragma unroll
+                    for (int g = 0; g < 4; ++g) v[c][j][g] = src[(((wid * 2 + i) * 2 + j) * 4 + g) << 6];
+            }
+#pragma unroll
+            for (int c = 0; c < FINISH_CHUNK; ++c) {
+                if (s0 + c >= p.k_slices) break;
+#pragma unroll
+                for (int j = 0; j < 2; ++j)
+#pragma unroll
+                    for (int g = 0; g < 4; ++g)
+#pragma unroll
+                        for (int e = 0; e < 4; ++e) acc[i][j][4 * g + e] += v[c][j][g][e];
+            }
+        }
+    }
+    conv_tile_epilogue<T>(acc, smem, y, bias, p, m0, n0, bz);
+}
+
+template <typename T, bool DMA, int LEAN = 0, int SPLIT = 0>
+__global__ __launch_bounds__(256, LEAN ? LEAN : 2) void conv_fprop_kernel(const T* __restrict__ x, const T* __restrict__ w,
+                                                            T* __restrict__ y, const float* __restrict__ bias,
+                                                            ConvParams p) {
+    constexpr int VEC = 16 / sizeof(T);
+    constexpr int BKE = ROWB / sizeof(T);
+    static_assert(!LEAN || (!DMA && sizeof(T) == 2), "lean variant: bf16, register staging");
+    static_assert(SPLIT == 0 || sizeof(T) == 4, "split-bf16 products are a mode of the fp32-storage kernel");
+    static_assert(SPLIT == 0 || !DMA, "the split planes are written from the staging registers");
+    constexpr int SROW = SPLIT ? SPLIT * 64 + 16 : ROWB;
+    constexpr int STAGE = SPLIT ? (BM + BN) * SROW : STAGE_BYTES;
+    constexpr bool ONE_STAGE = LEAN != 0 || SPLIT == 3;
+    constexpr int SMEM_BYTES = ONE_STAGE ? (STAGE > 65536 || sizeof(T) == 2 ? STAGE : 65536) : 2 * STAGE;
+    __shared__ __attribute__((aligned(16))) char smem[SMEM_BYTES];
+
+    const int tid = threadIdx.x, lane = tid & 63, wid = tid >> 6;
+    const int wm = wid >> 1, wn = wid & 1;
+    const int lr = lane & 31, lh = lane >> 5;
+    const unsigned L = xcd_remap(blockIdx.x, gridDim.x);
+    const int n0 = (int)(L % p.n_tiles) * BN;
+    const int m0 = (int)(L / p.n_tiles) * BM;
+    const int bz = blockIdx.z;
+
+    const int wid_u = __builtin_amdgcn_readfirstlane(wid);
+    const int slot_phys = tid & 7;
+    int row_of[4];
+#pragma unroll
+    for (int j = 0; j < 4; ++j) row_of[j] = DMA ? (wid * 32 + 8 * j + (lane >> 3)) : ((tid >> 3) + 32 * j);
+    const int slot = DMA ? 0 : slot_phys;
+    int a_ih0[4], a_iw0[4];
+    long long a_boff[4];
+    int a_slot[4];
+    bool a_ok[4];
+    const int ohw = p.OH * p.OW;
+#pragma unroll
+    for (int j = 0; j < 4; ++j) {
+        const int m = m0 + row_of[j];
+        const int slot_j = DMA ? (slot_phys ^ ((row_of[j] >> 1) & 7)) : slot_phys;
+        a_ok[j] = m < p.Mtot;
+        const int mm = a_ok[j] ? m : 0;
+        const int b = p.per_sample ? bz : mm / ohw;
+        const int pix = p.per_sample ? mm : mm - b * ohw;
+        const int oh = pix / p.OW, ow = pix - oh * p.OW;
+        a_ih0[j] = oh * p.stride - p.pad;
+        a_iw0[j] = ow * p.stride - p.pad;
+        a_boff[j] = ((long long)((DMA && p.per_sample) ? 0 : b) * p.x_bstride + slot_j * VEC +
+                     ((long long)a_ih0[j] * p.IW + a_iw0[j]) * p.Cx) * (long long)sizeof(T);
+        a_slot[j] = slot_j;
+    }
+    const int taps = p.kh * p.kw;
+    const gptr_t xbase = (gptr_t)x;
+    const gptr_t zbase = (gptr_t)g_zero_page;
+    const long long zoff = slot_phys * 16;
+    gptr_t pa[4];
+    gptr_t pb[4];
+    {
+        const gptr_t wb = (gptr_t)w + (p.per_sample ? (long long)bz * p.w_bstride : 0) * (long long)sizeof(T);
+#pragma unroll
+        for (int j = 0; j < 4; ++j) {
+            const int n = n0 + row_of[j];
+            const bool ok = n < p.N;
+            pb[j] = (ok ? wb : zbase) + (ok ? ((long long)n * taps * p.Ck + a_slot[j] * VEC) * (long long)sizeof(T) : zoff);
+            pa[j] = zbase;
+        }
+    }
+    msg_desc_t d_x = {0, 0, 0, 0}, d_w = {0, 0, 0, 0};
+    unsigned lds0 = 0;
+    int va[4] = {MSG_DMA_OOB, MSG_DMA_OOB, MSG_DMA_OOB, MSG_DMA_OOB}, vb[4] = {MSG_DMA_OOB, MSG_DMA_OOB, MSG_DMA_OOB, MSG_DMA_OOB};
+    if constexpr (DMA) {
+        d_x = msg_make_desc((const char*)x + (p.per_sample ? (long long)bz * p.x_bstride * (long long)sizeof(T) : 0));
+        d_w = msg_make_desc((const char*)w + (p.per_sample ? (long long)bz * p.w_bstride * (long long)sizeof(T) : 0));
+        lds0 = (unsigned)(unsigned long long)(lds_t)smem;
+#pragma unroll
+        for (int j = 0; j < 4; ++j) {
+            const int n = n0 + row_of[j];
+            vb[j] = n < p.N ? (int)(((long long)n * taps * p.Ck + a_slot[j] * VEC) * (long long)sizeof(T)) : MSG_DMA_OOB;
+        }
+    }
+    const bool ragged = (p.Cx % BKE) != 0;
+    int k_first = 0, k_steps = p.n_iters;
+    if constexpr (DMA) {
+        k_first = (int)blockIdx.y * p.n_iters / p.k_slices;
+        k_steps = ((int)blockIdx.y + 1) * p.n_iters / p.k_slices - k_first;
+    }
+    const bool mid_tap = DMA && (k_first % p.n_chunks) != 0;
+    int ld_tap = k_first / p.n_chunks - (mid_tap ? 0 : 1);
+    int ld_chunk = mid_tap ? k_first % p.n_chunks - 1 : p.n_chunks - 1;
+    int kh_ = ld_tap < 0 ? 0 : ld_tap / p.kw, kw_ = ld_tap - kh_ * p.kw;
+    int st_off[4];
+#pragma unroll
+    for (int j = 0; j < 4; ++j) st_off[j] = swz(row_of[j], a_slot[j]);
+
+    f32x16 acc[2][2];
+#pragma unroll
+    for (int i = 0; i < 2; ++i)
+#pragma unroll
+        for (int j = 0; j < 2; ++j)
+#pragma unroll
+            for (int e = 0; e < 16; ++e) acc[i][j][e] = 0.f;
+
+    u32x4 ra[4], rb[4];
+    int dma_stage = 0;
+    auto enter_tap = [&]() __attribute__((always_inline)) {
+        {
+            if (p.in_up == 1) {
+                const long long tap_off = ((long long)kh_ * p.IW + kw_) * p.Cx * (long long)sizeof(T);
+#pragma unroll
+                for (int j = 0; j < 4; ++j) {
+                    const bool ok = a_ok[j] & ((unsigned)(a_ih0[j] + kh_) < (unsigned)p.IH) &
+                                    ((unsigned)(a_iw0[j] + kw_) < (unsigned)p.IW);
+                    pa[j] = (ok ? xbase : zbase) + (ok ? a_boff[j] + tap_off : zoff);
+                    if constexpr (DMA) va[j] = ok ? (int)(a_boff[j] + tap_off) : MSG_DMA_OOB;
+                }
+            } else {
+#pragma unroll
+                for (int j = 0; j < 4; ++j) {
+                    const int ih = a_ih0[j] + kh_, iw = a_iw0[j] + kw_;
+                    bool ok = a_ok[j] & (ih >= 0) & (iw >= 0) & (ih % p.in_up == 0) & (iw % p.in_up == 0);
+                    const int ihs = ih / p.in_up, iws = iw / p.in_up;
+                    ok = ok & (ihs < p.IH) & (iws < p.IW);
+                    const long long off = a_boff[j] + ((long long)(ihs - a_ih0[j]) * p.IW + (iws - a_iw0[j])) * p.Cx * (long long)sizeof(T);
+                    pa[j] = (ok ? xbase : zbase) + (ok ? off : zoff);
+                    if constexpr (DMA) va[j] = ok ? (int)off : MSG_DMA_OOB;
+                }
+            }
+        }
+    };
+    auto load_next = [&]() __attribute__((always_inline)) {
+        if (++ld_chunk == p.n_chunks) {
+            ld_chunk = 0;
+            ++ld_tap;
+            if (++kw_ == p.kw) { kw_ = 0; ++kh_; }
+            enter_tap();
+        }
+#pragma unroll
+        for (int j = 0; j < 4; ++j) {
+            const bool c_bad = ragged && (ld_chunk * BKE + a_slot[j] * VEC + VEC > p.Cx);
+            gptr_t a_addr = pa[j];
+            if (c_bad) a_addr = zbase + zoff;
+            if constexpr (DMA) {
+                const unsigned la = lds0 + dma_stage * STAGE + (wid_u * 32 + 8 * j) * ROWB;
+                msg_dma16(d_x, la, c_bad ? MSG_DMA_OOB : va[j], ld_chunk * ROWB);
+                msg_dma16(d_w, la + BM * ROWB, vb[j], (ld_tap * p.n_chunks + ld_chunk) * ROWB);
+            } else {
+                ra[j] = *(gvec_t)a_addr;
+                rb[j] = *(gvec_t)pb[j];
+            }
+            pa[j] += ROWB;
+            pb[j] += ROWB;
+        }
+    };
+    auto park = [&](int stage) __attribute__((always_inline)) {
+        char* sa = smem + stage * STAGE;
+        if constexpr (SPLIT != 0) {
+            char* sb = sa + BM * SROW;
+#pragma unroll
+            for (int j = 0; j < 4; ++j) {
+                split_park<SPLIT>(ra[j], sa + row_of[j] * SROW + slot_phys * 8);
+                split_park<SPLIT>(rb[j], sb + row_of[j] * SROW + slot_phys * 8);
+            }
+            return;
+        }
+        char* sb = sa + BM * ROWB;
+#pragma unroll
+        for (int j = 0; j < 4; ++j) {
+            *reinterpret_cast<u32x4*>(sa + st_off[j]) = ra[j];
+            *reinterpret_cast<u32x4*>(sb + st_off[j]) = rb[j];
+        }
+    };
+    auto mma_step = [&](const char* sa) __attribute__((always_inline)) {
+        const char* sb = sa + BM * ROWB;
+        if constexpr (sizeof(T) == 2) {
+            bf16v8 fa[2][2], fb[2][2];
+#pragma unroll
+            for (int t = 0; t < 2; ++t) {
+                fa[0][t] = *reinterpret_cast<const bf16v8*>(sa + swz(wm * 64 + t * 32 + lr, lh));
+                fb[0][t] = *reinterpret_cast<const bf16v8*>(sb + swz(wn * 64 + t * 32 + lr, lh));
+            }
+#pragma unroll
+            for (int kk = 0; kk < 4; ++kk) {
+                if (kk + 1 < 4) {
+#pragma unroll
+                    for (int t = 0; t < 2; ++t) {
+                        fa[(kk + 1) & 1][t] = *reinterpret_cast<const bf16v8*>(sa + swz(wm * 64 + t * 32 + lr, 2 * (kk + 1) + lh));
+                        fb[(kk + 1) & 1][t] = *reinterpret_cast<const bf16v8*>(sb + swz(wn * 64 + t * 32 + lr, 2 * (kk + 1) + lh));
+                    }
+                }
+#pragma unroll
+                for (int i = 0; i < 2; ++i)
+#pragma unroll
+                    for (int j = 0; j < 2; ++j)
+                        acc[i][j] = __builtin_amdgcn_mfma_f32_32x32x16_bf16(fb[kk & 1][j], fa[kk & 1][i], acc[i][j], 0, 0, 0);
+            }
+            __builtin_amdgcn_sched_group_barrier(0x100, 8, 0);
+            __builtin_amdgcn_sched_group_barrier(0x008, 4, 0);
+            __builtin_amdgcn_sched_group_barrier(0x100, 4, 0);
+            __builtin_amdgcn_sched_group_barrier(0x008, 4, 0);
+            __builtin_amdgcn_sched_group_barrier(0x100, 4, 0);
+            __builtin_amdgcn_sched_group_barrier(0x008, 8, 0);
+        } else if constexpr (SPLIT != 0) {
+            const char* sbs = sa + BM * SROW;
+#pragma unroll
+            for (int sstep = 0; sstep < 2; ++sstep) {
+                bf16v8 af[SPLIT][2], bf[SPLIT][2];
+#pragma unroll
+                for (int t = 0; t < 2; ++t)
+#pragma unroll
+                    for (int pl = 0; pl < SPLIT; ++pl) {
+                        af[pl][t] = *reinterpret_cast<const bf16v8*>(sa + (wm * 64 + t * 32 + lr) * SROW + pl * 64 + (2 * sstep + lh) * 16);
+                        bf[pl][t] = *reinterpret_cast<const bf16v8*>(sbs + (wn * 64 + t * 32 + lr) * SROW + pl * 64 + (2 * sstep + lh) * 16);
+                    }
+#pragma unroll
+                for (int i = 0; i < 2; ++i)
+#pragma unroll
+                    for (int j = 0; j < 2; ++j) {
+#pragma unroll
+                        for (int order = SPLIT - 1; order >= 0; --order)
+#pragma unroll
+                            for (int pa = 0; pa <= order; ++pa)
+                                acc[i][j] = __builtin_amdgcn_mfma_f32_32x32x16_bf16(bf[order - pa][j], af[pa][i], acc[i][j], 0, 0, 0);
+                    }
+            }
+        } else {
+#pragma unroll
+            for (int q = 0; q < 4; ++q) {
+                f32x4 fa[2], fb[2];
+#pragma unroll
+                for (int t = 0; t < 2; ++t) {
+                    fa[t] = *reinterpret_cast<const f32x4*>(sa + swz(wm * 64 + t * 32 + lr, 4 * lh + q));
+                    fb[t] = *reinterpret_cast<const f32x4*>(sb + swz(wn * 64 + t * 32 + lr, 4 * lh + q));
+                }
+#pragma unroll
+                for (int e = 0; e < 4; ++e)
+#pragma unroll
+                    for (int i = 0; i < 2; ++i)
+#pragma unroll
+                        for (int j = 0; j < 2; ++j)
+                            acc[i][j] = __builtin_amdgcn_mfma_f32_32x32x2f32(fb[j][e], fa[i][e], acc[i][j], 0, 0, 0);
+            }
+        }
+    };
+    if (mid_tap) enter_tap();
+    if constexpr (ONE_STAGE) {
+        load_next();
+        for (int it = 0; it < p.n_iters; ++it) {
+            if (it) __syncthreads();
+            park(0);
+            if (it + 1 < p.n_iters) load_next();
+            __syncthreads();
+            mma_step(smem);
+        }
+    } else {
+        if constexpr (DMA) {
+            dma_stage = 0;
+            load_next();
+        } else {
+            load_next();
+            park(0);
+            if (p.n_iters > 1) load_next();
+        }
+        for (int it = 0; it < k_steps; ++it) {
+            if constexpr (DMA) asm volatile("s_waitcnt vmcnt(0)" ::: "memory");
+            __syncthreads();
+            if constexpr (DMA) {
+                if (it + 1 < k_steps) { dma_stage = (it + 1) & 1; load_next(); }
+            } else {
+                if (it + 1 < k_steps) park((it + 1) & 1);
+                if (it + 2 < k_steps) load_next();
+            }
+            mma_step(smem + (it & 1) * STAGE);
+        }
+    }
+    if constexpr (DMA) asm volatile("s_waitcnt vmcnt(0)" ::: "memory");
+    __syncthreads();
+    if constexpr (DMA) {
+        if (p.k_slices > 1) {
+            ksplit_store(acc, reinterpret_cast<f32x4*>(p.ws) + ksplit_slab(p, L, bz, (int)blockIdx.y), p, m0);
+            return;
+        }
+    }
+
+    conv_tile_epilogue<T>(acc, smem, y, bias, p, m0, n0, bz);
+}
+
 static ConvPlan conv_generic_select(const ConvProblem& q) {
     const int n_iters = q.kh * q.kw * (q.Ck / (ROWB / q.esz()));
     static const int variant = msg_tunable("MSG_CONV_VARIANT", 0);
@@ -426,8 +523,39 @@
     return plan;
 }
 
+static int conv_generic_ksplit(const ConvProblem& q, const ConvPlan& plan, int requested) {
+    if (plan.kernel != CONV_DMA) return 1;
+    const int n_iters = q.kh * q.kw * (q.Ck / (ROWB / q.esz()));
+    if (requested == MSG_FPROP_K_AUTO) requested = msg_tunable("MSG_CONV_KSLICES", MSG_FPROP_K_AUTO);
+    if (requested > 0) return std::min(requested, n_iters);
+    const long long n_tiles = (q.N + BN - 1) / BN, wgs = ((q.mtot() + BM - 1) / BM) * n_tiles * q.samples();
+    if (wgs >= KSPLIT_ROUND_WGS) return 1;
+    const long long slabs100 = q.mtot() * n_tiles * q.samples() * 100 / BM;
+    long long best = -1;
+    int slices = 1;
+    for (int s = 1; s <= n_iters / KSPLIT_MIN_STEPS; ++s) {
+        const long long rounds = (wgs * s + KSPLIT_ROUND_WGS - 1) / KSPLIT_ROUND_WGS;
+        const long long cost = rounds * ((n_iters + s - 1) / s * 100 + KSPLIT_FIXED) +
+                               (s > 1 ? KSPLIT_SLAB + s * (KSPLIT_PER_SLICE + KSPLIT_TRAFFIC * slabs100 / 100) : 0);
+        if (best < 0 || cost < best) { best = cost; slices = s; }
+        if (wgs * s > KSPLIT_ROUND_WGS) break;
+    }
+    return slices;
+}
+static long long conv_generic_ksplit_floats(const ConvProblem& q, int k_slices) {
+    if (k_slices <= 1) return 0;
+    return ((q.mtot() + BM - 1) / BM) * ((q.N + BN - 1) / BN) * q.samples() * (long long)k_slices * (BM * BN);
+}
+
+static thread_local int g_ksplit_phases = 3;
+extern "C" int msg_conv2d_fprop_ksplit_phases(int phases) {
+    const int before = g_ksplit_phases;
+    g_ksplit_phases = phases & 3 ? phases & 3 : 3;
+    return before;
+}
+
 static void conv_generic_launch(const ConvProblem& q, const ConvPlan& plan, const void* x, const void* w, const float* bias, void* y,
-                                const ActEpilogue* act, void* stream) {
+                                const ActEpilogue* act, void* stream, int k_slices, float* ws) {
     ConvParams p{};
     conv_fill_common(p, q, act);
     conv_fill_taps(p, q);
@@ -435,17 +563,25 @@
     p.n_iters = q.kh * q.kw * p.n_chunks;
     p.m_tiles = (int)((q.mtot() + BM - 1) / BM);
     p.n_tiles = (q.N + BN - 1) / BN;
-    dim3 grid((unsigned)((long long)p.m_tiles * p.n_tiles), 1, q.samples());
+    p.k_slices = k_slices;
+    p.ws = ws;
+    dim3 grid((unsigned)((long long)p.m_tiles * p.n_tiles), (unsigned)k_slices, q.samples());
 #define GENERIC(T, ...) hipLaunchKernelGGL((conv_fprop_kernel<T, __VA_ARGS__>), grid, dim3(256), 0, (hipStream_t)stream, \
                                            (const T*)x, (const T*)w, (T*)y, bias, p)
     const bool bf16 = q.dtype == MSG_BF16;
-    if (bf16 && plan.kernel == CONV_REG_LEAN) GENERIC(bf16_t, false, 3);
+    if (k_slices > 1 && !(g_ksplit_phases & 1)) ;
+    else if (bf16 && plan.kernel == CONV_REG_LEAN) GENERIC(bf16_t, false, 3);
     else if (bf16 && plan.kernel == CONV_DMA) GENERIC(bf16_t, true);
     else if (bf16) GENERIC(bf16_t, false);
     else if (plan.kernel == CONV_REG_SPLIT) GENERIC(float, false, 0, 3);
     else if (plan.kernel == CONV_DMA) GENERIC(float, true);
     else GENERIC(float, false);
 #undef GENERIC
+    if (k_slices > 1 && (g_ksplit_phases & 2)) {
+        grid.y = 1;
+        if (bf16) hipLaunchKernelGGL(conv_fprop_finish_kernel<bf16_t>, grid, dim3(256), 0, (hipStream_t)stream, ws, (bf16_t*)y, bias, p);
+        else hipLaunchKernelGGL(conv_fprop_finish_kernel<float>, grid, dim3(256), 0, (hipStream_t)stream, ws, (float*)y, bias, p);
+    }
 }
 
 ConvPlan conv_fprop_select(const ConvProblem& q, const ActEpilogue* act, bool has_bias) {
@@ -529,6 +665,24 @@
     return MSG_OK;
 }
 
+extern "C" int msg_conv2d_fprop_ksplit_plan(int dtype, int B, int IH, int IW, int Cx, int Ck, int OH, int OW, int N, int ldy,
+                                            int kh, int kw, int stride, int pad, int in_up, int pixel_shuffle,
+                                            long long w_batch_stride, int has_bias, int epilogue, int k_slices,
+                                            long long* out, int n_out_fields) {
+    if (k_slices < 0 || epilogue < 0 || epilogue > 2 || (epilogue && (has_bias || in_up != 1 || pixel_shuffle))) return MSG_EINVAL;
+    const ConvProblem q = conv_problem(dtype, B, IH, IW, Cx, Ck, OH, OW, N, ldy, kh, kw, stride, pad, in_up, pixel_shuffle, w_batch_stride);
+    ConvPlan plan;
+    const int rc = fprop_plan_for(q, epilogue, has_bias != 0, nullptr, &plan);
+    if (rc != MSG_OK) return rc;
+    long long fields[MSG_FKSPLIT_FIELDS] = {};
+    if (q.B) {
+        fields[0] = conv_generic_ksplit(q, plan, k_slices);
+        fields[1] = conv_generic_ksplit_floats(q, (int)fields[0]);
+    }
+    for (int k = 0; k < MSG_FKSPLIT_FIELDS && k < n_out_fields; ++k) out[k] = fields[k];
+    return MSG_OK;
+}
+
 static ConvProblem conv_query_problem(int dtype, int B, int IH, int IW, int Cx, int Ck, int OH, int OW, int N, int kh, int kw,
                                       long long w_batch_stride) {
     return conv_problem(dtype, B, IH, IW, Cx, Ck, OH, OW, N, N <= 8 ? 8 : (N + 7) / 8 * 8, kh, kw, 1, kh / 2, 1, 0, w_batch_stride);
@@ -558,11 +712,14 @@
 }
 
 static int conv2d_fprop_impl(const void* x, const void* w, const float* bias, void* y, const ConvProblem& q,
-                             const ActEpilogue& act, void* stream) {
+                             const ActEpilogue& act, void* stream, int k_slices = 1, float* ws = nullptr, long long ws_floats = 0) {
     const void* const io[3] = {x, w, y};
     ConvPlan plan;
+    if (k_slices < 0 || ws_floats < 0) return MSG_EINVAL;
     const int rc = fprop_plan_for(q, act.enabled, bias != nullptr, io, &plan);
     if (rc != MSG_OK || q.B == 0) return rc;
+    k_slices = conv_generic_ksplit(q, plan, k_slices);
+    if (k_slices > 1 && (!ws || (((uintptr_t)ws) & 15u) || ws_floats < conv_generic_ksplit_floats(q, k_slices))) return MSG_EINVAL;
     if (act.mask && !is_row3(plan)) return MSG_EUNSUPPORTED;
     switch (plan.kernel) {
         case CONV_THIN_N: case CONV_THIN_K: conv_thin_launch(q, plan, x, w, bias, y, &act, stream); break;
@@ -570,29 +727,54 @@
         case CONV_ROW3: case CONV_ROW3N: conv_row3_launch(q, plan, x, w, bias, y, &act, stream); break;
         case CONV_PP: conv_pp_launch(q, plan, x, w, bias, y, &act, stream); break;
         case CONV_DMA: case CONV_REG: case CONV_REG_LEAN: case CONV_REG_SPLIT:
-            conv_generic_launch(q, plan, x, w, bias, y, &act, stream); break;
+            conv_generic_launch(q, plan, x, w, bias, y, &act, stream, k_slices, ws); break;
     }
     return MSG_CHECK_LAUNCH();
 }
 
+extern "C" int msg_conv2d_fprop_ws(const void* x, const void* w, const float* bias, void* y, int dtype,
+                                   int B, int IH, int IW, int Cx, int Ck, int OH, int OW, int N, int ldy,
+                                   int kh, int kw, int stride, int pad, int in_up, int pixel_shuffle,
+                                   long long w_batch_stride, float* ws, long long ws_floats, int k_slices, void* stream) {
+    ActEpilogue act{};
+    return conv2d_fprop_impl(x, w, bias, y, conv_problem(dtype, B, IH, IW, Cx, Ck, OH, OW, N, ldy, kh, kw, stride, pad, in_up,
+                                                         pixel_shuffle, w_batch_stride), act, stream, k_slices, ws, ws_floats);
+}
 extern "C" int msg_conv2d_fprop(const void* x, const void* w, const float* bias, void* y, int dtype,
                                 int B, int IH, int IW, int Cx, int Ck, int OH, int OW, int N, int ldy,
                                 int kh, int kw, int stride, int pad, int in_up, int pixel_shuffle,
                                 long long w_batch_stride, void* stream) {
-    ActEpilogue act{};
-    return conv2d_fprop_impl(x, w, bias, y, conv_problem(dtype, B, IH, IW, Cx, Ck, OH, OW, N, ldy, kh, kw, stride, pad, in_up,
-                                                         pixel_shuffle, w_batch_stride), act, stream);
-}
-
+    return msg_conv2d_fprop_ws(x, w, bias, y, dtype, B, IH, IW, Cx, Ck, OH, OW, N, ldy, kh, kw, stride, pad, in_up, pixel_shuffle,
+                               w_batch_stride, nullptr, 0, 1, stream);
+}
+
+extern "C" int msg_conv2d_fprop_act_mask_ws(const void* x, const void* w, void* y, int dtype,
+                                            int B, int IH, int IW, int Cx, int Ck, int OH, int OW, int N, int ldy,
+                                            int kh, int kw, int stride, int pad, long long w_batch_stride,
+                                            const float* act_bias, const float* noise, const float* noise_weight,
+                                            int noise_batch, float alpha, float scale, unsigned char* mask,
+                                            float* ws, long long ws_floats, int k_slices, void* stream) {
+    if (noise && (!noise_weight || (noise_batch != 1 && noise_batch != B))) return MSG_EINVAL;
+    ActEpilogue act{act_bias, noise, noise_weight, noise_batch, 1, alpha, scale, nullptr, 0, 0.f, mask};
+    return conv2d_fprop_impl(x, w, nullptr, y, conv_problem(dtype, B, IH, IW, Cx, Ck, OH, OW, N, ldy, kh, kw, stride, pad, 1, 0,
+                                                            w_batch_stride), act, stream, k_slices, ws, ws_floats);
+}
 extern "C" int msg_conv2d_fprop_act_mask(const void* x, const void* w, void* y, int dtype,
                                          int B, int IH, int IW, int Cx, int Ck, int OH, int OW, int N, int ldy,
                                          int kh, int kw, int stride, int pad, long long w_batch_stride,
                                          const float* act_bias, const float* noise, const float* noise_weight,
                                          int noise_batch, float alpha, float scale, unsigned char* mask, void* stream) {
-    if (noise && (!noise_weight || (noise_batch != 1 && noise_batch != B))) return MSG_EINVAL;
-    ActEpilogue act{act_bias, noise, noise_weight, noise_batch, 1, alpha, scale, nullptr, 0, 0.f, mask};
-    return conv2d_fprop_impl(x, w, nullptr, y, conv_problem(dtype, B, IH, IW, Cx, Ck, OH, OW, N, ldy, kh, kw, stride, pad, 1, 0,
-                                                            w_batch_stride), act, stream);
+    return msg_conv2d_fprop_act_mask_ws(x, w, y, dtype, B, IH, IW, Cx, Ck, OH, OW, N, ldy, kh, kw, stride, pad, w_batch_stride,
+                                        act_bias, noise, noise_weight, noise_batch, alpha, scale, mask, nullptr, 0, 1, stream);
+}
+extern "C" int msg_conv2d_fprop_act_ws(const void* x, const void* w, void* y, int dtype,
+                                       int B, int IH, int IW, int Cx, int Ck, int OH, int OW, int N, int ldy,
+                                       int kh, int kw, int stride, int pad, long long w_batch_stride,
+                                       const float* act_bias, const float* noise, const float* noise_weight,
+                                       int noise_batch, float alpha, float scale,
+                                       float* ws, long long ws_floats, int k_slices, void* stream) {
+    return msg_conv2d_fprop_act_mask_ws(x, w, y, dtype, B, IH, IW, Cx, Ck, OH, OW, N, ldy, kh, kw, stride, pad, w_batch_stride,
+                                        act_bias, noise, noise_weight, noise_batch, alpha, scale, nullptr, ws, ws_floats, k_slices, stream);
 }
 
 extern "C" int msg_conv2d_fprop_act(const void* x, const void* w, void* y, int dtype,
@@ -608,11 +790,19 @@
                                          int B, int IH, int IW, int Cx, int Ck, int OH, int OW, int N, int ldy,
                                          int kh, int kw, int stride, int pad, long long w_batch_stride,
                                          const void* residual, int res_ld, float gain, void* stream) {
+    return msg_conv2d_fprop_residual_ws(x, w, y, dtype, B, IH, IW, Cx, Ck, OH, OW, N, ldy, kh, kw, stride, pad, w_batch_stride,
+                                        residual, res_ld, gain, nullptr, 0, 1, stream);
+}
+extern "C" int msg_conv2d_fprop_residual_ws(const void* x, const void* w, void* y, int dtype,
+                                            int B, int IH, int IW, int Cx, int Ck, int OH, int OW, int N, int ldy,
+                                            int kh, int kw, int stride, int pad, long long w_batch_stride,
+                                            const void* residual, int res_ld, float gain,
+                                            float* ws, long long ws_floats, int k_slices, void* stream) {
     if (!residual || res_ld < N || (((uintptr_t)residual) & 15u) || res_ld % (dtype == MSG_BF16 ? 8 : 4)) return MSG_EINVAL;
     ActEpilogue act{};
     act.enabled = 2; act.residual = residual; act.res_ld = res_ld; act.res_gain = gain;
     return conv2d_fprop_impl(x, w, nullptr, y, conv_problem(dtype, B, IH, IW, Cx, Ck, OH, OW, N, ldy, kh, kw, stride, pad, 1, 0,
-                                                            w_batch_stride), act, stream);
+                                                            w_batch_stride), act, stream, k_slices, ws, ws_floats);
 }
 
 extern "C" int msg_conv2d_fprop_act_backward(const void* x, const void* w, void* y, int dtype,
```

Result: no change. 157.8 (median of 6 runs) (+0.8%).
